# syzhang092218-source/dgppo

Hardware: AMD Instinct MI355X
Metric: env-steps/sec whole node, LidarSpread n=8 4096 envs, 1/2/4/8 GPUs (higher is better)
Workload: dtype f32

## Files before the change

dgppo_amd/_native.py:

```python
from __future__ import annotations

import ctypes as C
import os
from typing import Optional

import numpy as np
import torch

_HERE = os.path.dirname(os.path.abspath(__file__))
LIB_PATH = os.environ.get("DGPPO_HIP_LIB") or os.path.join(_HERE, "csrc", "libdgppo_hip.so")

ABI_VERSION = 3
OPT_STATE_FLOATS = 8 + 2 * 256

ENV_KINDS = {"LidarSpread": 0, "LidarTarget": 1, "LidarBicycleTarget": 2, "MPESpread": 3, "MPETarget": 4,
             "LidarLine": 5, "MPELine": 6, "MPEFormation": 7, "MPECorridor": 8, "MPEConnectSpread": 9,
             "VMASReverseTransport": 10}
VMAS_REVERSE_TRANSPORT = 10
GOALS_NODES, GOALS_LINE, GOALS_LINE_INTERIOR, GOALS_CIRCLE = range(4)
RECT_STRIDE = 16


class EnvCfg(C.Structure):
    _fields_ = [
        ("kind", C.c_int32), ("n_agents", C.c_int32), ("n_goals", C.c_int32), ("n_obs", C.c_int32),
        ("n_rays", C.c_int32), ("top_k", C.c_int32), ("state_dim", C.c_int32), ("node_dim", C.c_int32),
        ("area_size", C.c_float), ("dt", C.c_float), ("car_radius", C.c_float), ("comm_radius", C.c_float),
        ("obs_radius", C.c_float), ("dist2goal", C.c_float), ("two_car_radius", C.c_float),
        ("lidar_mask_radius", C.c_float), ("eye_offset", C.c_float), ("car_plus_obs", C.c_float),
        ("vel_limit", C.c_float), ("reset_min_dist", C.c_float),
        ("reward_goals", C.c_int32), ("n_cost", C.c_int32), ("obs_mask_radius", C.c_float), ("y_limit", C.c_float),
        ("connect_radius", C.c_float), ("reset_side_y", C.c_float), ("goal_shift_y", C.c_float), ("line_min_dist", C.c_float),
    ]

    @property
    def is_vmas(self):
        return self.kind == VMAS_REVERSE_TRANSPORT

    @property
    def is_lidar(self):
        return self.kind <= 2 or self.kind == 5

    @property
    def is_spread(self):
        return self.kind not in (1, 2, 4)

    @property
    def obs_nodes(self):
        if self.is_lidar:
            return self.n_agents * self.top_k if self.n_obs > 0 else 0
        return self.n_obs

    @property
    def obs_slots(self):
        if self.is_lidar:
            return self.top_k if self.n_obs > 0 else 0
        return self.n_obs

    @property
    def goal_slots(self):
        return self.n_goals if self.is_spread else 1

    @property
    def num_nodes(self):
        return self.n_agents + self.n_goals + self.obs_nodes + 1

    @property
    def num_edges(self):
        return self.n_agents * (self.n_agents + self.goal_slots + self.obs_slots)

    @property
    def fan_in(self):
        return self.n_agents + self.goal_slots + self.obs_slots

    @property
    def obst_stride(self):
        return RECT_STRIDE if self.is_lidar else self.state_dim


def make_env_cfg(kind: int, n_agents: int, n_obs: int, n_rays: int = 32, top_k: int = 8, area_size: float = None,
                 dt: float = 0.03, car_radius: float = 0.05, comm_radius: float = 0.5, obs_radius: float = None,
                 dist2goal: float = 0.01, connect_radius: float = 0.45, corridor_width: float = 0.2) -> EnvCfg:
    if kind == VMAS_REVERSE_TRANSPORT:
        return make_vmas_cfg(n_agents, dt)
    is_lidar = kind <= 2 or kind == 5
    corridor, connect = kind == 8, kind == 9
    if area_size is None:
        area_size = 1.0 if (corridor or connect) else 1.5
    if corridor:
        n_obs = 2
        obs_radius = (area_size - corridor_width) / 4
    elif connect:
        n_obs = 1
        obs_radius = 0.25 if obs_radius is None else obs_radius
    elif obs_radius is None:
        obs_radius = 0.05
    sd = 5 if kind == 2 else 4
    c = EnvCfg()
    c.kind, c.n_agents, c.n_obs = kind, n_agents, n_obs
    c.n_goals = 2 if kind in (5, 6) else (1 if kind == 7 else n_agents)
    c.n_rays, c.top_k = (n_rays, top_k) if is_lidar else (0, 0)
    c.state_dim, c.node_dim = sd, sd + 3
    c.area_size, c.dt, c.car_radius, c.comm_radius = area_size, dt, car_radius, comm_radius
    c.obs_radius, c.dist2goal = obs_radius, dist2goal
    c.two_car_radius = car_radius * 2
    c.lidar_mask_radius = comm_radius - 1e-1
    c.eye_offset = comm_radius + 1
    c.car_plus_obs = car_radius + obs_radius
    c.vel_limit = 0.5 if is_lidar else 1.0
    c.reset_min_dist = (2.2 * car_radius) if (is_lidar and kind != 5) else ((2.3 if connect else 2) * car_radius)
    c.reward_goals = {5: GOALS_LINE, 6: GOALS_LINE if n_agents > 3 else GOALS_LINE_INTERIOR, 7: GOALS_CIRCLE}.get(kind, GOALS_NODES)
    c.n_cost = 3 if connect else 2
    c.obs_mask_radius = comm_radius * 100 if (corridor or connect) else comm_radius
    c.y_limit = area_size * 2 if (corridor or connect) else area_size
    c.connect_radius = connect_radius
    c.reset_side_y = ((area_size - obs_radius * 2) / 2 - 1.5 * car_radius) if (corridor or connect) else area_size
    c.goal_shift_y = (area_size - (area_size - obs_radius * 2) / 2 + 1.5 * car_radius) if (corridor or connect) else 0.0
    if kind in (5, 6):
        c.line_min_dist = n_agents * 5 * car_radius if (kind == 6 and n_agents <= 3) else (n_agents - 2) * 6 * car_radius
    else:
        c.line_min_dist = 0.0
    return c


def make_vmas_cfg(n_agents: int, dt: float = 0.03) -> EnvCfg:
    c = EnvCfg()
    c.kind, c.n_agents, c.n_goals, c.n_obs, c.n_rays, c.top_k = VMAS_REVERSE_TRANSPORT, n_agents, 0, 0, 0, 0
    c.state_dim, c.node_dim = 4, 20
    c.area_size, c.dt, c.car_radius, c.comm_radius, c.obs_radius, c.dist2goal = 1.6, dt, 0.03, 0.4, 0.15, 0.01
    c.two_car_radius = 0.03 * 2
    c.vel_limit, c.reset_min_dist = 1.0, 0.03 * 2
    c.reward_goals, c.n_cost = GOALS_NODES, 2
    c.obs_mask_radius, c.y_limit = 0.4, 1.6
    return c


class GraphOut(C.Structure):
    _fields_ = [(k, C.c_void_p) for k in
                ("nodes", "edges", "states", "receivers", "senders", "node_type", "n_node", "n_edge")]


_lib: Optional[C.CDLL] = None


def lib() -> C.CDLL:
    global _lib
    if _lib is not None:
        return _lib
    if not os.path.exists(LIB_PATH):
        raise RuntimeError(
            f"dgppo_amd: HIP library not built: {LIB_PATH} is missing. "
            "Run `python -c 'import __graft_entry__ as g; g.build()'` (or `make -C dgppo_amd/csrc`). "
            "There is no CPU fallback.")
    l = C.CDLL(LIB_PATH)
    l.dgppo_abi_version.restype = C.c_int32
    l.dgppo_last_error.restype = C.c_char_p
    v = l.dgppo_abi_version()
    if v != ABI_VERSION:
        raise RuntimeError(f"dgppo_amd: ABI mismatch: library {v}, python {ABI_VERSION}")
    _lib = l
    return l


def check(rc: int, what: str):
    if rc != 0:
        msg = lib().dgppo_last_error().decode("utf-8", "replace")
        if rc > 0:
            raise RuntimeError(f"{what}: hipError {rc}: {msg}")
        raise ValueError(f"{what}: {msg}")


def ptr(t: Optional[torch.Tensor], dtype=torch.float32, name: str = "tensor") -> C.c_void_p:
    if t is None:
        return C.c_void_p(0)
    if not t.is_cuda:
        raise RuntimeError(f"{name} must live on the GPU (the HIP path has no CPU fallback)")
    if t.dtype != dtype:
        raise TypeError(f"{name} must be {dtype}, got {t.dtype}")
    if not t.is_contiguous():
        raise ValueError(f"{name} must be contiguous")
    return C.c_void_p(t.data_ptr())


_raw_stream = getattr(torch._C, "_cuda_getCurrentRawStream", None)
_raw_device = getattr(torch._C, "_cuda_getDevice", None)


def stream_ptr() -> C.c_void_p:
    if _raw_stream is not None and _raw_device is not None:
        return C.c_void_p(_raw_stream(_raw_device()))
    return C.c_void_p(torch.cuda.current_stream().cuda_stream)


def expect_shape(t: torch.Tensor, shape, name: str):
    if tuple(t.shape) != tuple(shape):
        raise ValueError(f"{name}: expected shape {tuple(shape)}, got {tuple(t.shape)}")
```

dgppo_amd/csrc/nn_elem.hip:

```cpp
#include "common.h"

using f32x4 = __attribute__((ext_vector_type(4))) float;

__device__ inline float wave_sum(float v) {
#pragma unroll
  for (int o = 32; o >= 1; o >>= 1) v += __shfl_xor(v, o);
  return v;
}
template <int NV>
__device__ inline void block_atomic_sums(const float (&v)[NV], float* dst) {
  __shared__ float s_red[4][NV];
  const int lane = threadIdx.x & 63, wave = threadIdx.x >> 6;
#pragma unroll
  for (int k = 0; k < NV; ++k) {
    const float w = wave_sum(v[k]);
    if (lane == 0) s_red[wave][k] = w;
  }
  __syncthreads();
  if (threadIdx.x < NV) {
    float t = 0.0f;
    for (int w = 0; w < (int)(blockDim.x >> 6); ++w) t += s_red[w][threadIdx.x];
    atomicAdd(dst + threadIdx.x, t);
  }
}

__device__ inline float row16_sum(float v) {
  v += __int_as_float(__builtin_amdgcn_update_dpp(0, __float_as_int(v), 0xB1, 0xf, 0xf, false));
  v += __int_as_float(__builtin_amdgcn_update_dpp(0, __float_as_int(v), 0x4E, 0xf, 0xf, false));
  v += __int_as_float(__builtin_amdgcn_update_dpp(0, __float_as_int(v), 0x141, 0xf, 0xf, false));
  v += __int_as_float(__builtin_amdgcn_update_dpp(0, __float_as_int(v), 0x140, 0xf, 0xf, false));
  return v;
}

__global__ void __launch_bounds__(256) ln_relu_fwd_kernel(const float* __restrict__ x, const float* __restrict__ gamma,
                                                          const float* __restrict__ beta, float* __restrict__ y,
                                                          float* __restrict__ stats, int M) {
  const int lane = threadIdx.x & 63, li = lane & 15, lq = lane >> 4;
  const int wave = (blockIdx.x * blockDim.x + threadIdx.x) >> 6;
  const int nw = (gridDim.x * blockDim.x) >> 6;
  const float4 g = reinterpret_cast<const float4*>(gamma)[li], b = reinterpret_cast<const float4*>(beta)[li];
  for (int row0 = wave * 4; row0 < M; row0 += nw * 4) {
    const int row = row0 + lq;
    const bool ok = row < M;
    const float4 v = reinterpret_cast<const float4*>(x)[(size_t)(ok ? row : M - 1) * 16 + li];
    const float mean = row16_sum((v.x + v.y) + (v.z + v.w)) * (1.0f / 64.0f);
    const float mean2 = row16_sum((v.x * v.x + v.y * v.y) + (v.z * v.z + v.w * v.w)) * (1.0f / 64.0f);
    const float var = fmaxf(mean2 - mean * mean, 0.0f);
    const float rstd = rsqrtf(var + 1e-6f);
    float4 o;
    o.x = fmaxf((v.x - mean) * rstd * g.x + b.x, 0.0f);
    o.y = fmaxf((v.y - mean) * rstd * g.y + b.y, 0.0f);
    o.z = fmaxf((v.z - mean) * rstd * g.z + b.z, 0.0f);
    o.w = fmaxf((v.w - mean) * rstd * g.w + b.w, 0.0f);
    if (ok) {
      reinterpret_cast<float4*>(y)[(size_t)row * 16 + li] = o;
      if (stats != nullptr && li == 0) reinterpret_cast<float2*>(stats)[row] = make_float2(mean, rstd);
    }
  }
}

__global__ void __launch_bounds__(256) ln_relu_bwd_kernel(const float* __restrict__ x, const float* __restrict__ y,
                                                          const float* __restrict__ stats, const float* __restrict__ gamma,
                                                          const float* __restrict__ dy, float* __restrict__ dx,
                                                          float* __restrict__ dgamma, float* __restrict__ dbeta, int M) {
  const int lane = threadIdx.x & 63, li = lane & 15, lq = lane >> 4;
  const int wave = (blockIdx.x * blockDim.x + threadIdx.x) >> 6;
  const int nw = (gridDim.x * blockDim.x) >> 6;
  const float4 g = reinterpret_cast<const float4*>(gamma)[li];
  float dg[4] = {0.f, 0.f, 0.f, 0.f}, db[4] = {0.f, 0.f, 0.f, 0.f};
  for (int row0 = wave * 4; row0 < M; row0 += nw * 4) {
    const int row = row0 + lq;
    const bool ok = row < M;
    const size_t o = (size_t)(ok ? row : M - 1) * 16 + li;
    const float4 xv = reinterpret_cast<const float4*>(x)[o], yv = reinterpret_cast<const float4*>(y)[o];
    const float4 dv = reinterpret_cast<const float4*>(dy)[o];
    const float2 st = reinterpret_cast<const float2*>(stats)[ok ? row : M - 1];
    const float mean = st.x, rstd = st.y;
    const float xh[4] = {(xv.x - mean) * rstd, (xv.y - mean) * rstd, (xv.z - mean) * rstd, (xv.w - mean) * rstd};
    const float dl[4] = {(ok && yv.x > 0.0f) ? dv.x : 0.0f, (ok && yv.y > 0.0f) ? dv.y : 0.0f,
                         (ok && yv.z > 0.0f) ? dv.z : 0.0f, (ok && yv.w > 0.0f) ? dv.w : 0.0f};
    const float gg[4] = {g.x, g.y, g.z, g.w};
    float dxh[4], s1 = 0.0f, s2 = 0.0f;
#pragma unroll
    for (int q = 0; q < 4; ++q) {
      dg[q] += dl[q] * xh[q];
      db[q] += dl[q];
      dxh[q] = dl[q] * gg[q];
      s1 += dxh[q];
      s2 += dxh[q] * xh[q];
    }
    const float m1 = row16_sum(s1) * (1.0f / 64.0f), m2 = row16_sum(s2) * (1.0f / 64.0f);
    if (ok)
      reinterpret_cast<float4*>(dx)[o] = make_float4(rstd * (dxh[0] - m1 - xh[0] * m2), rstd * (dxh[1] - m1 - xh[1] * m2),
                                                     rstd * (dxh[2] - m1 - xh[2] * m2), rstd * (dxh[3] - m1 - xh[3] * m2));
  }
  __shared__ float red[2][16][64];
  const int slot = (threadIdx.x >> 6) * 4 + lq;
#pragma unroll
  for (int q = 0; q < 4; ++q) { red[0][slot][li * 4 + q] = dg[q]; red[1][slot][li * 4 + q] = db[q]; }
  __syncthreads();
  if (threadIdx.x < 128) {
    const int which = threadIdx.x >> 6;
    float v = 0.0f;
#pragma unroll
    for (int sidx = 0; sidx < 16; ++sidx) v += red[which][sidx][lane];
    atomicAdd((which ? dbeta : dgamma) + lane, v);
  }
}

extern "C" int32_t dgppo_ln_relu_fwd(const float* x, const float* gamma, const float* beta, float* y, float* stats,
                                     int32_t M, void* stream) {
  DGPPO_REQUIRE(M >= 0, "ln_relu_fwd: M < 0");
  if (M == 0) return 0;
  DGPPO_REQUIRE(x && gamma && beta && y, "ln_relu_fwd: NULL operand");
  const int grid = min(cdiv(M, 16), 2048);
  hipLaunchKernelGGL(ln_relu_fwd_kernel, dim3(grid), dim3(256), 0, (hipStream_t)stream, x, gamma, beta, y, stats, M);
  DGPPO_LAUNCH_CHECK();
  return 0;
}

extern "C" int32_t dgppo_ln_relu_bwd(const float* x, const float* y, const float* stats, const float* gamma,
                                     const float* dy, float* dx, float* dgamma, float* dbeta, int32_t M, void* stream) {
  DGPPO_REQUIRE(M >= 0, "ln_relu_bwd: M < 0");
  if (M == 0) return 0;
  DGPPO_REQUIRE(x && y && stats && gamma && dy && dx && dgamma && dbeta, "ln_relu_bwd: NULL operand");
  const int grid = min(cdiv(M, 16), 256);
  hipLaunchKernelGGL(ln_relu_bwd_kernel, dim3(grid), dim3(256), 0, (hipStream_t)stream, x, y, stats, gamma, dy, dx, dgamma,
                     dbeta, M);
  DGPPO_LAUNCH_CHECK();
  return 0;
}

#define GRU_H 64
#define GRU_WL 194
#define GRU_HL 66

struct GruArgs {
  const float* gi;
  const float* Wh;
  const float* bhn;
  const float* h0;
  float* hs;
  float* hprev;
  float* gates;
  const float* dhs;
  float* dgi;
  float* dgh;
  float* dhn;
  int n_seq, T, n_inner;
};

__device__ inline size_t gru_row(const GruArgs& a, int s, int tau) {
  const int grp = s / a.n_inner, i = s - grp * a.n_inner;
  return ((size_t)grp * a.T + tau) * a.n_inner + i;
}
__device__ inline float sigmoidf_(float x) { return 1.0f / (1.0f + expf(-x)); }
__device__ inline float gate_sigmoid(float x) { return __builtin_amdgcn_rcpf(1.0f + __expf(-x)); }
__device__ inline float gate_tanh(float x) { return fmaf(2.0f, __builtin_amdgcn_rcpf(1.0f + __expf(-2.0f * x)), -1.0f); }


#define GRU_LDS_BARRIER() asm volatile("s_waitcnt lgkmcnt(0)\n\ts_barrier" ::: "memory")

template <int RTW>
__global__ void __launch_bounds__(256) gru_fwd_kernel(GruArgs a) {
  extern __shared__ float sm[];
  constexpr int RB = 16 * RTW;
  constexpr int HSLOT = RB * 16 / 256 > 0 ? RB * 16 / 256 : 1;
  const int tid = threadIdx.x, lane = tid & 63, w = tid >> 6, li = lane & 15, lq = lane >> 4;
  const int c = w * 16 + li;
  float breg[16][3];
#pragma unroll
  for (int kk = 0; kk < 16; ++kk)
#pragma unroll
    for (int t = 0; t < 3; ++t) breg[kk][t] = a.Wh[(size_t)(kk * 4 + lq) * 192 + t * 64 + c];
  const float bn = a.bhn[c];
  const int n_tiles = (a.n_seq + RB - 1) / RB;
  const float4 z4 = make_float4(0.f, 0.f, 0.f, 0.f);
  float hpf[HSLOT][4];
  auto fetch_h0 = [&](int tile) {
#pragma unroll
    for (int u = 0; u < HSLOT; ++u) {
      int idx = u * 256 + tid;
      idx = idx < RB * 16 ? idx : RB * 16 - 1;
      const int r = idx >> 4, q = idx & 15;
      int s = tile * RB + r;
      s = s < a.n_seq ? s : a.n_seq - 1;
      float4 v = z4;
      if (a.h0 != nullptr) v = reinterpret_cast<const float4*>(a.h0 + (size_t)s * GRU_H)[q];
      hpf[u][0] = v.x; hpf[u][1] = v.y; hpf[u][2] = v.z; hpf[u][3] = v.w;
    }
  };
  auto commit_h0 = [&](float* dst) {
#pragma unroll
    for (int u = 0; u < HSLOT; ++u) {
      const int idx = u * 256 + tid, r = idx >> 4, q = idx & 15;
      if (idx < RB * 16) { float* d = dst + r * GRU_HL + 4 * q; d[0] = hpf[u][0]; d[1] = hpf[u][1]; d[2] = hpf[u][2]; d[3] = hpf[u][3]; }
    }
  };
  int tile = blockIdx.x;
  if (tile < n_tiles) { fetch_h0(tile); commit_h0(sm); }
  __syncthreads();
  int cur = 0;
  for (; tile < n_tiles; tile += gridDim.x) {
    const int s0 = tile * RB;
    const int nxt = tile + gridDim.x;
    if (nxt < n_tiles) fetch_h0(nxt);
    int row0[RTW][4];
    bool ok[RTW][4];
#pragma unroll
    for (int rt = 0; rt < RTW; ++rt)
#pragma unroll
      for (int r = 0; r < 4; ++r) {
        int s = s0 + rt * 16 + lq * 4 + r;
        ok[rt][r] = s < a.n_seq;
        s = ok[rt][r] ? s : a.n_seq - 1;
        int rw = s;
        if (a.T != 1 && a.n_inner != 1) { const int grp = s / a.n_inner; rw = grp * a.T * a.n_inner + (s - grp * a.n_inner); }
        else if (a.T != 1) rw = s * a.T;
        row0[rt][r] = rw;
      }
    float gn[RTW][4][3];
    auto fetch_gi = [&](int tau) {
#pragma unroll
      for (int rt = 0; rt < RTW; ++rt)
#pragma unroll
        for (int r = 0; r < 4; ++r) {
          const float* gp = a.gi + (size_t)(row0[rt][r] + tau * a.n_inner) * 192 + c;
          gn[rt][r][0] = gp[0]; gn[rt][r][1] = gp[64]; gn[rt][r][2] = gp[128];
        }
    };
    fetch_gi(0);
    for (int tau = 0; tau < a.T; ++tau) {
      const float* hs_cur = sm + cur * (RB * GRU_HL);
      float* hs_nxt = sm + (cur ^ 1) * (RB * GRU_HL);
      float g[RTW][4][3];
#pragma unroll
      for (int rt = 0; rt < RTW; ++rt)
#pragma unroll
        for (int r = 0; r < 4; ++r) { g[rt][r][0] = gn[rt][r][0]; g[rt][r][1] = gn[rt][r][1]; g[rt][r][2] = gn[rt][r][2]; }
      if (tau + 1 < a.T) fetch_gi(tau + 1);
      __builtin_amdgcn_sched_barrier(0);
      float areg[RTW][16];
#pragma unroll
      for (int rt = 0; rt < RTW; ++rt)
#pragma unroll
        for (int kk = 0; kk < 16; ++kk) areg[rt][kk] = hs_cur[(rt * 16 + li) * GRU_HL + kk * 4 + lq];
      __builtin_amdgcn_sched_barrier(0);
      f32x4 acc[RTW][3];
#pragma unroll
      for (int rt = 0; rt < RTW; ++rt)
#pragma unroll
        for (int t = 0; t < 3; ++t) acc[rt][t] = f32x4{0.f, 0.f, 0.f, 0.f};
#pragma unroll
      for (int kk = 0; kk < 16; ++kk)
#pragma unroll
        for (int rt = 0; rt < RTW; ++rt)
#pragma unroll
          for (int t = 0; t < 3; ++t) acc[rt][t] = __builtin_amdgcn_mfma_f32_16x16x4f32(areg[rt][kk], breg[kk][t], acc[rt][t], 0, 0, 0);
#pragma unroll
      for (int rt = 0; rt < RTW; ++rt)
#pragma unroll
        for (int r = 0; r < 4; ++r) {
          const int rl = rt * 16 + lq * 4 + r;
          const float hp = hs_cur[rl * GRU_HL + c];
          const float rg = gate_sigmoid(g[rt][r][0] + acc[rt][0][r]);
          const float zg = gate_sigmoid(g[rt][r][1] + acc[rt][1][r]);
          const float hn = acc[rt][2][r] + bn;
          const float ng = gate_tanh(g[rt][r][2] + rg * hn);
          const float hnew = (1.0f - zg) * ng + zg * hp;
          hs_nxt[rl * GRU_HL + c] = hnew;
          if (ok[rt][r]) {
            const size_t row = (size_t)(row0[rt][r] + tau * a.n_inner);
            a.hs[row * GRU_H + c] = hnew;
            if (a.hprev != nullptr) a.hprev[row * GRU_H + c] = hp;
            if (a.gates != nullptr) {
              float* gs = a.gates + row * 256;
              gs[c] = rg; gs[64 + c] = zg; gs[128 + c] = ng; gs[192 + c] = hn;
            }
          }
        }
      GRU_LDS_BARRIER();
      cur ^= 1;
    }
    if (nxt < n_tiles) {
      commit_h0(sm + cur * (RB * GRU_HL));
      GRU_LDS_BARRIER();
    }
  }
}

template <int RTW, bool DHN_ONLY>
__global__ void __launch_bounds__(256) gru_bwd_kernel(GruArgs a) {
  extern __shared__ float sm[];
  constexpr int RB = 16 * RTW;
  const int tid = threadIdx.x, lane = tid & 63, w = tid >> 6, li = lane & 15, lq = lane >> 4;
  const int c = w * 16 + li;
  float breg[48];
#pragma unroll
  for (int kk = 0; kk < 48; ++kk) breg[kk] = a.Wh[(size_t)c * 192 + kk * 4 + lq];
  const int n_tiles = (a.n_seq + RB - 1) / RB;
  int cur = 0;
  for (int tile = blockIdx.x; tile < n_tiles; tile += gridDim.x) {
    const int s0 = tile * RB;
    int row0[RTW][4];
    bool ok[RTW][4];
#pragma unroll
    for (int rt = 0; rt < RTW; ++rt)
#pragma unroll
      for (int r = 0; r < 4; ++r) {
        int s = s0 + rt * 16 + lq * 4 + r;
        ok[rt][r] = s < a.n_seq;
        s = ok[rt][r] ? s : a.n_seq - 1;
        int rw = s;
        if (a.T != 1 && a.n_inner != 1) { const int grp = s / a.n_inner; rw = grp * a.T * a.n_inner + (s - grp * a.n_inner); }
        else if (a.T != 1) rw = s * a.T;
        row0[rt][r] = rw;
      }
    float rg[RTW][4], zg[RTW][4], ng[RTW][4], hn[RTW][4], hp[RTW][4], du[RTW][4], dh[RTW][4];
    auto fetch = [&](int tau) {
#pragma unroll
      for (int rt = 0; rt < RTW; ++rt)
#pragma unroll
        for (int r = 0; r < 4; ++r) {
          const size_t row = (size_t)(row0[rt][r] + tau * a.n_inner);
          const float* gs = a.gates + row * 256 + c;
          rg[rt][r] = gs[0]; zg[rt][r] = gs[64]; ng[rt][r] = gs[128]; hn[rt][r] = gs[192];
          hp[rt][r] = a.hprev[row * GRU_H + c];
          du[rt][r] = a.dhs[row * GRU_H + c];
        }
    };
#pragma unroll
    for (int rt = 0; rt < RTW; ++rt)
#pragma unroll
      for (int r = 0; r < 4; ++r) dh[rt][r] = 0.0f;
    fetch(a.T - 1);
    for (int tau = a.T - 1; tau >= 0; --tau) {
      float* s_g = sm + cur * (RB * GRU_WL);
#pragma unroll
      for (int rt = 0; rt < RTW; ++rt)
#pragma unroll
        for (int r = 0; r < 4; ++r) {
          const int rl = rt * 16 + lq * 4 + r;
          const float d = ok[rt][r] ? dh[rt][r] + du[rt][r] : 0.0f;
          const float dz = d * (hp[rt][r] - ng[rt][r]);
          const float dn = d * (1.0f - zg[rt][r]);
          const float dan = dn * (1.0f - ng[rt][r] * ng[rt][r]);
          const float dhn = dan * rg[rt][r];
          const float dar = dan * hn[rt][r] * rg[rt][r] * (1.0f - rg[rt][r]);
          const float daz = dz * zg[rt][r] * (1.0f - zg[rt][r]);
          dh[rt][r] = d * zg[rt][r];
          s_g[rl * GRU_WL + c] = dar;
          s_g[rl * GRU_WL + 64 + c] = daz;
          s_g[rl * GRU_WL + 128 + c] = dhn;
          if (ok[rt][r]) {
            const size_t row = (size_t)(row0[rt][r] + tau * a.n_inner);
            float* o = a.dgi + row * 192 + c;
            o[0] = dar; o[64] = daz; o[128] = dan;
            if (DHN_ONLY) {
              a.dhn[row * GRU_H + c] = dhn;
            } else {
              float* p = a.dgh + row * 192 + c;
              p[0] = dar; p[64] = daz; p[128] = dhn;
            }
          }
        }
      GRU_LDS_BARRIER();
      if (tau > 0) fetch(tau - 1);
      __builtin_amdgcn_sched_barrier(0);
      f32x4 acc[RTW];
#pragma unroll
      for (int rt = 0; rt < RTW; ++rt) acc[rt] = f32x4{0.f, 0.f, 0.f, 0.f};
#pragma unroll
      for (int k0 = 0; k0 < 48; k0 += 16) {
        float areg[RTW][16];
#pragma unroll
        for (int rt = 0; rt < RTW; ++rt)
#pragma unroll
          for (int u = 0; u < 16; ++u) areg[rt][u] = s_g[(rt * 16 + li) * GRU_WL + (k0 + u) * 4 + lq];
        __builtin_amdgcn_sched_barrier(0);
#pragma unroll
        for (int u = 0; u < 16; ++u)
#pragma unroll
          for (int rt = 0; rt < RTW; ++rt) acc[rt] = __builtin_amdgcn_mfma_f32_16x16x4f32(areg[rt][u], breg[k0 + u], acc[rt], 0, 0, 0);
      }
#pragma unroll
      for (int rt = 0; rt < RTW; ++rt)
#pragma unroll
        for (int r = 0; r < 4; ++r) dh[rt][r] += acc[rt][r];
      cur ^= 1;
    }
    GRU_LDS_BARRIER();
  }
}

static int gru_resident(const void* fn, size_t smem) {
  int per_cu = 0, dev = 0, cus = 256;
  if (hipOccupancyMaxActiveBlocksPerMultiprocessor(&per_cu, fn, 256, smem) != hipSuccess || per_cu < 1) per_cu = 1;
  if (hipGetDevice(&dev) != hipSuccess ||
      hipDeviceGetAttribute(&cus, hipDeviceAttributeMultiprocessorCount, dev) != hipSuccess || cus < 1) cus = 256;
  return per_cu * cus;
}

static int32_t gru_check(const GruArgs& a) {
  DGPPO_REQUIRE(a.n_seq >= 0 && a.T >= 1 && a.n_inner >= 1, "gru: bad sizes n_seq=%d T=%d n_inner=%d", a.n_seq, a.T, a.n_inner);
  DGPPO_REQUIRE(a.n_seq % a.n_inner == 0, "gru: n_seq must be a multiple of n_inner");
  return 0;
}

extern "C" int32_t dgppo_gru_fwd(const float* gi, const float* Wh, const float* bhn, const float* h0, float* hs,
                                 float* hprev, float* gates, int32_t n_seq, int32_t T, int32_t n_inner, void* stream) {
  GruArgs a{};
  a.gi = gi; a.Wh = Wh; a.bhn = bhn; a.h0 = h0; a.hs = hs; a.hprev = hprev; a.gates = gates;
  a.n_seq = n_seq; a.T = T; a.n_inner = n_inner;
  int32_t rc = gru_check(a);
  if (rc) return rc;
  if (n_seq == 0) return 0;
  DGPPO_REQUIRE(gi && Wh && bhn && hs, "gru_fwd: NULL operand");
  if (cdiv(n_seq, 32) >= 512) {
    const size_t smem = sizeof(float) * 2 * 32 * GRU_HL;
    static thread_local int cap = 0;
    if (cap == 0) cap = gru_resident(reinterpret_cast<const void*>(&gru_fwd_kernel<2>), smem);
    const int tiles = cdiv(n_seq, 32);
    hipLaunchKernelGGL(gru_fwd_kernel<2>, dim3(tiles < cap ? tiles : cap), dim3(256), smem, (hipStream_t)stream, a);
  } else {
    const size_t smem = sizeof(float) * 2 * 16 * GRU_HL;
    static thread_local int cap = 0;
    if (cap == 0) cap = gru_resident(reinterpret_cast<const void*>(&gru_fwd_kernel<1>), smem);
    const int tiles = cdiv(n_seq, 16);
    hipLaunchKernelGGL(gru_fwd_kernel<1>, dim3(tiles < cap ? tiles : cap), dim3(256), smem, (hipStream_t)stream, a);
  }
  DGPPO_LAUNCH_CHECK();
  return 0;
}

template <bool DHN_ONLY>
static int32_t gru_bwd_launch(GruArgs a, hipStream_t stream) {
  int32_t rc = gru_check(a);
  if (rc) return rc;
  if (a.n_seq == 0) return 0;
  DGPPO_REQUIRE(a.dhs && a.Wh && a.hprev && a.gates && a.dgi && (DHN_ONLY ? a.dhn : a.dgh), "gru_bwd: NULL operand");
  if (cdiv(a.n_seq, 32) >= 512) {
    const size_t smem = sizeof(float) * 2 * 32 * GRU_WL;
    static thread_local int cap = 0;
    if (cap == 0) cap = gru_resident(reinterpret_cast<const void*>(&gru_bwd_kernel<2, DHN_ONLY>), smem);
    const int tiles = cdiv(a.n_seq, 32);
    hipLaunchKernelGGL((gru_bwd_kernel<2, DHN_ONLY>), dim3(tiles < cap ? tiles : cap), dim3(256), smem, stream, a);
  } else {
    const size_t smem = sizeof(float) * 2 * 16 * GRU_WL;
    static thread_local int cap = 0;
    if (cap == 0) cap = gru_resident(reinterpret_cast<const void*>(&gru_bwd_kernel<1, DHN_ONLY>), smem);
    const int tiles = cdiv(a.n_seq, 16);
    hipLaunchKernelGGL((gru_bwd_kernel<1, DHN_ONLY>), dim3(tiles < cap ? tiles : cap), dim3(256), smem, stream, a);
  }
  DGPPO_LAUNCH_CHECK();
  return 0;
}

extern "C" int32_t dgppo_gru_bwd(const float* dhs, const float* Wh, const float* hprev, const float* gates, float* dgi,
                                 float* dgh, int32_t n_seq, int32_t T, int32_t n_inner, void* stream) {
  GruArgs a{};
  a.dhs = dhs; a.Wh = Wh; a.hprev = (float*)hprev; a.gates = (float*)gates; a.dgi = dgi; a.dgh = dgh;
  a.n_seq = n_seq; a.T = T; a.n_inner = n_inner;
  return gru_bwd_launch<false>(a, (hipStream_t)stream);
}

extern "C" int32_t dgppo_gru_bwd_dhn(const float* dhs, const float* Wh, const float* hprev, const float* gates, float* dgi,
                                     float* dhn, int32_t n_seq, int32_t T, int32_t n_inner, void* stream) {
  GruArgs a{};
  a.dhs = dhs; a.Wh = Wh; a.hprev = (float*)hprev; a.gates = (float*)gates; a.dgi = dgi; a.dhn = dhn;
  a.n_seq = n_seq; a.T = T; a.n_inner = n_inner;
  return gru_bwd_launch<true>(a, (hipStream_t)stream);
}

#define STD_INIT_INV (-0.43275212956718856f)
#define STD_MIN 1e-5f
#define THRESH 0.999f
#define INV_THRESH 3.8002011672502f
#define LOG_EPS (-6.907755278982137f)
#define HALF_LOG_2PI 0.9189385332046727f
#define LOG2_F 0.6931471805599453f

__device__ inline float softplusf_(float x) { return (x > 20.0f) ? x : log1pf(expf(x)); }
#define NDTR_SERIES_BELOW (-10.0f)
__device__ inline float ndtr_tail_series(float z2) { return 1.0f - 1.0f / z2 + 3.0f / (z2 * z2) - 15.0f / (z2 * z2 * z2); }
__device__ inline float log_ndtrf_(float z) {
  if (z > NDTR_SERIES_BELOW) return logf(0.5f * erfcf(-z * 0.70710678118654752f));
  const float z2 = z * z;
  return -0.5f * z2 - logf(-z) - HALF_LOG_2PI + logf(ndtr_tail_series(z2));
}
__device__ inline float dlog_ndtrf_(float z) {
  if (z > NDTR_SERIES_BELOW) return 0.3989422804014327f * expf(-0.5f * z * z) / (0.5f * erfcf(-z * 0.70710678118654752f));
  return -z / ndtr_tail_series(z * z);
}
__device__ inline float tanh_fldj(float x) { return 2.0f * (LOG2_F - x - softplusf_(-2.0f * x)); }

struct HeadArgs {
  const float* ms;
  const float* eps;
  const float* action_in;
  float* action;
  float* log_pi;
  float* entropy;
  int rows, n_agents, mode;
  const float* log_pi_old;
  const float* adv;
  float* dms;
  float* stats;
  float clip_eps, coef_ent, inv_count;
};

__device__ inline float tn_log_prob_dim(float act, float mu, float sd) {
  const float ac = fminf(fmaxf(act, -THRESH), THRESH);
  if (ac <= -THRESH) return log_ndtrf_((-INV_THRESH - mu) / sd) - LOG_EPS;
  if (ac >= THRESH) return log_ndtrf_(-(INV_THRESH - mu) / sd) - LOG_EPS;
  const float x = atanhf(ac);
  const float z = (x - mu) / sd;
  return -0.5f * z * z - logf(sd) - HALF_LOG_2PI - tanh_fldj(x);
}

__global__ void __launch_bounds__(256) policy_head_kernel(HeadArgs a) {
  float acc[4] = {0.0f, 0.0f, 0.0f, 0.0f};
  const int rows_pad = (a.rows + 255) & ~255;
  for (int row_raw = blockIdx.x * blockDim.x + threadIdx.x; row_raw < rows_pad; row_raw += gridDim.x * blockDim.x) {
  const bool valid = row_raw < a.rows;
  const int row = valid ? row_raw : a.rows - 1;
  const float4 m = reinterpret_cast<const float4*>(a.ms)[row];
  const float mu[2] = {m.x, m.y};
  const float st[2] = {m.z, m.w};
  float sd[2];
  for (int d = 0; d < 2; ++d) sd[d] = softplusf_(st[d] + STD_INIT_INV) + STD_MIN;
  if (a.mode == 1) {
    if (valid) {
      a.action[row * 2] = tanhf(mu[0]);
      a.action[row * 2 + 1] = tanhf(mu[1]);
    }
    continue;
  }
  float act[2];
  if (a.mode == 0) {
    for (int d = 0; d < 2; ++d) act[d] = tanhf(mu[d] + sd[d] * a.eps[row * 2 + d]);
    if (valid) {
      a.action[row * 2] = act[0];
      a.action[row * 2 + 1] = act[1];
      a.log_pi[row] = tn_log_prob_dim(act[0], mu[0], sd[0]) + tn_log_prob_dim(act[1], mu[1], sd[1]);
    }
    continue;
  }
  act[0] = a.action_in[row * 2];
  act[1] = a.action_in[row * 2 + 1];
  const int ag = row % a.n_agents;
  float lp = 0.0f, ent = 0.0f;
  float dlp_dmu[2], dlp_dsd[2], dent_dmu[2], dent_dsd[2];
  for (int d = 0; d < 2; ++d) {
    const float ac = fminf(fmaxf(act[d], -THRESH), THRESH);
    if (ac <= -THRESH) {
      const float u = (-INV_THRESH - mu[d]) / sd[d];
      lp += log_ndtrf_(u) - LOG_EPS;
      const float r = dlog_ndtrf_(u);
      dlp_dmu[d] = -r / sd[d];
      dlp_dsd[d] = -r * u / sd[d];
    } else if (ac >= THRESH) {
      const float u = (mu[d] - INV_THRESH) / sd[d];
      lp += log_ndtrf_(u) - LOG_EPS;
      const float r = dlog_ndtrf_(u);
      dlp_dmu[d] = r / sd[d];
      dlp_dsd[d] = -r * u / sd[d];
    } else {
      const float x = atanhf(ac);
      const float z = (x - mu[d]) / sd[d];
      lp += -0.5f * z * z - logf(sd[d]) - HALF_LOG_2PI - tanh_fldj(x);
      dlp_dmu[d] = z / sd[d];
      dlp_dsd[d] = (z * z - 1.0f) / sd[d];
    }
    const float eh = a.eps[ag * 2 + d];
    const float y = mu[d] + sd[d] * eh;
    ent += 0.5f + HALF_LOG_2PI + logf(sd[d]) + tanh_fldj(y);
    const float th = tanhf(y);
    dent_dmu[d] = -2.0f * th;
    dent_dsd[d] = 1.0f / sd[d] - 2.0f * th * eh;
  }
  if (valid) {
    a.log_pi[row] = lp;
    a.entropy[row] = ent;
  }
  if (a.dms == nullptr) continue;
  const float A = a.adv[row];
  const float rho = expf(lp - a.log_pi_old[row]);
  const float l1 = -rho * A;
  const float l2 = -fminf(fmaxf(rho, 1.0f - a.clip_eps), 1.0f + a.clip_eps) * A;
  const float lsel = fmaxf(l1, l2);
  const float dl_dlp = ((l2 > l1) ? 0.0f : -rho * A) * a.inv_count;
  const float dl_dent = -a.coef_ent * a.inv_count;
  if (valid) {
    float4 o;
    const float dsd0 = dl_dlp * dlp_dsd[0] + dl_dent * dent_dsd[0];
    const float dsd1 = dl_dlp * dlp_dsd[1] + dl_dent * dent_dsd[1];
    o.x = dl_dlp * dlp_dmu[0] + dl_dent * dent_dmu[0];
    o.y = dl_dlp * dlp_dmu[1] + dl_dent * dent_dmu[1];
    o.z = dsd0 * sigmoidf_(st[0] + STD_INIT_INV);
    o.w = dsd1 * sigmoidf_(st[1] + STD_INIT_INV);
    reinterpret_cast<float4*>(a.dms)[row] = o;
  }
  if (valid) {
    acc[0] += lsel; acc[1] += ent; acc[2] += (l2 > l1) ? 1.0f : 0.0f; acc[3] += fabsf(rho - 1.0f);
  }
  }
  if (a.mode == 2 && a.dms != nullptr) block_atomic_sums<4>(acc, a.stats);
}

extern "C" int32_t dgppo_policy_head(const float* ms, const float* eps, const float* action_in, float* action,
                                     float* log_pi, float* entropy, int32_t rows, int32_t n_agents, int32_t mode,
                                     const float* log_pi_old, const float* adv, float* dms, float* stats, float clip_eps,
                                     float coef_ent, void* stream) {
  DGPPO_REQUIRE(rows >= 0 && n_agents >= 1 && mode >= 0 && mode <= 2, "policy_head: bad arguments");
  if (rows == 0) return 0;
  DGPPO_REQUIRE(ms, "policy_head: ms is NULL");
  DGPPO_REQUIRE(((uintptr_t)ms & 15) == 0, "policy_head: ms must be 16-byte aligned");
  if (mode == 0) DGPPO_REQUIRE(eps && action && log_pi, "policy_head(sample): NULL operand");
  if (mode == 1) DGPPO_REQUIRE(action, "policy_head(mode): NULL operand");
  if (mode == 2) {
    DGPPO_REQUIRE(eps && action_in && log_pi && entropy, "policy_head(eval): NULL operand");
    if (dms) DGPPO_REQUIRE(log_pi_old && adv && stats && ((uintptr_t)dms & 15) == 0, "policy_head(eval+loss): NULL operand");
  }
  HeadArgs a{};
  a.ms = ms; a.eps = eps; a.action_in = action_in; a.action = action; a.log_pi = log_pi; a.entropy = entropy;
  a.rows = rows; a.n_agents = n_agents; a.mode = mode; a.log_pi_old = log_pi_old; a.adv = adv; a.dms = dms; a.stats = stats;
  a.clip_eps = clip_eps; a.coef_ent = coef_ent; a.inv_count = 1.0f / (float)rows;
  const int blocks = cdiv(rows, 256);
  hipLaunchKernelGGL(policy_head_kernel, dim3(blocks < 512 ? blocks : 512), dim3(256), 0, (hipStream_t)stream, a);
  DGPPO_LAUNCH_CHECK();
  return 0;
}

__global__ void __launch_bounds__(256) value_loss_kernel(const float* __restrict__ v, const float* __restrict__ target,
                                                         float* __restrict__ dv, float* __restrict__ stats, int count,
                                                         float count_f) {
  float l[1] = {0.0f};
  for (int i = blockIdx.x * blockDim.x + threadIdx.x; i < count; i += gridDim.x * blockDim.x) {
    const float d = v[i] - target[i];
    dv[i] = d / count_f;
    l[0] += 0.5f * d * d;
  }
  block_atomic_sums<1>(l, stats);
}

extern "C" int32_t dgppo_value_loss(const float* v, const float* target, float* dv, float* stats, int32_t count,
                                    void* stream) {
  DGPPO_REQUIRE(count >= 0, "value_loss: count < 0");
  if (count == 0) return 0;
  DGPPO_REQUIRE(v && target && dv && stats, "value_loss: NULL operand");
  const int blocks = cdiv(count, 256);
  hipLaunchKernelGGL(value_loss_kernel, dim3(blocks < 256 ? blocks : 256), dim3(256), 0, (hipStream_t)stream, v, target, dv,
                     stats, count, (float)count);
  DGPPO_LAUNCH_CHECK();
  return 0;
}

__global__ void mean_agents_kernel(const float* __restrict__ x, float* __restrict__ y, int G, int n, int D, int backward,
                                   const float* __restrict__ relu_mask) {
  const int idx = blockIdx.x * blockDim.x + threadIdx.x;
  if (backward) {
    if (idx >= G * n * D) return;
    const int d = idx % D, g = idx / (n * D);
    const float v = (backward == 2) ? y[idx] + x[(size_t)g * D + d] : x[(size_t)g * D + d] / (float)n;
    y[idx] = (relu_mask == nullptr || relu_mask[idx] > 0.0f) ? v : 0.0f;
  } else {
    if (idx >= G * D) return;
    const int d = idx % D, g = idx / D;
    float acc = 0.0f;
    for (int i = 0; i < n; ++i) acc += x[((size_t)g * n + i) * D + d];
    y[idx] = acc / (float)n;
  }
}

extern "C" int32_t dgppo_mean_agents(const float* x, float* y, int32_t G, int32_t n, int32_t D, int32_t backward,
                                     const float* relu_mask, void* stream) {
  DGPPO_REQUIRE(G >= 0 && n >= 1 && D >= 1, "mean_agents: bad sizes");
  DGPPO_REQUIRE(backward >= 0 && backward <= 2, "mean_agents: backward must be 0, 1 or 2");
  if (G == 0) return 0;
  DGPPO_REQUIRE(x && y, "mean_agents: NULL operand");
  const long total = backward ? (long)G * n * D : (long)G * D;
  hipLaunchKernelGGL(mean_agents_kernel, dim3(cdiv(total, 256)), dim3(256), 0, (hipStream_t)stream, x, y, G, n, D, backward,
                     backward ? relu_mask : nullptr);
  DGPPO_LAUNCH_CHECK();
  return 0;
}

__global__ void relu_bwd_kernel(float* __restrict__ dy, const float* __restrict__ y, long count) {
  const long i = (long)blockIdx.x * blockDim.x + threadIdx.x;
  if (i < count && !(y[i] > 0.0f)) dy[i] = 0.0f;
}

extern "C" int32_t dgppo_relu_bwd(float* dy, const float* y, int64_t count, void* stream) {
  DGPPO_REQUIRE(count >= 0, "relu_bwd: count < 0");
  if (count == 0) return 0;
  DGPPO_REQUIRE(dy && y, "relu_bwd: NULL operand");
  hipLaunchKernelGGL(relu_bwd_kernel, dim3(cdiv(count, 256)), dim3(256), 0, (hipStream_t)stream, dy, y, (long)count);
  DGPPO_LAUNCH_CHECK();
  return 0;
}
```

dgppo_amd/csrc/nn_fused.hip:

```cpp
#include "common.h"

using f32x4 = __attribute__((ext_vector_type(4))) float;
#define FZ_H 64
#define FZ_HL 66
#define FZ_RB 32
#define FZ_LDS_BARRIER() asm volatile("s_waitcnt lgkmcnt(0)\n\ts_barrier" ::: "memory")

__device__ inline float row16_sum(float v) {
  v += __int_as_float(__builtin_amdgcn_update_dpp(0, __float_as_int(v), 0xB1, 0xf, 0xf, false));
  v += __int_as_float(__builtin_amdgcn_update_dpp(0, __float_as_int(v), 0x4E, 0xf, 0xf, false));
  v += __int_as_float(__builtin_amdgcn_update_dpp(0, __float_as_int(v), 0x141, 0xf, 0xf, false));
  v += __int_as_float(__builtin_amdgcn_update_dpp(0, __float_as_int(v), 0x140, 0xf, 0xf, false));
  return v;
}

struct MlpGiArgs {
  const float* X; int ldx; int M;
  const float *W1, *b1, *g1, *be1, *W2, *b2, *g2, *be2, *Wi, *bi;
  float *p1, *y1, *st1, *p2, *y2, *st2;
  float* gi;
};

__global__ void __launch_bounds__(256) __attribute__((amdgpu_waves_per_eu(2, 8))) mlp_gi_fwd_kernel(MlpGiArgs a) {
  extern __shared__ float sm[];
  float* s_x = sm;
  float* s_y1 = s_x + FZ_RB * FZ_HL;
  float* s_y2 = s_y1 + FZ_RB * FZ_HL;
  float* s_red = s_y2 + FZ_RB * FZ_HL;
  const int tid = threadIdx.x, lane = tid & 63, w = tid >> 6, li = lane & 15, lq = lane >> 4;
  const int c = w * 16 + li;
  float w1[16], w2[16], wi[16][3];
#pragma unroll
  for (int kk = 0; kk < 16; ++kk) {
    const int k = kk * 4 + lq;
    w1[kk] = a.W1[k * FZ_H + c];
    w2[kk] = a.W2[k * FZ_H + c];
#pragma unroll
    for (int t = 0; t < 3; ++t) wi[kk][t] = a.Wi[k * 192 + t * 64 + c];
  }
  const float b1 = a.b1[c], g1 = a.g1[c], e1 = a.be1[c], b2 = a.b2[c], g2 = a.g2[c], e2 = a.be2[c];
  const float bi0 = a.bi[c], bi1 = a.bi[64 + c], bi2 = a.bi[128 + c];
  const int n_tiles = (a.M + FZ_RB - 1) / FZ_RB;
  const bool vec = ((a.ldx & 3) == 0) && ((reinterpret_cast<uintptr_t>(a.X) & 15) == 0);
  float xpf[2][4];
  auto fetch = [&](int tile) {
#pragma unroll
    for (int u = 0; u < 2; ++u) {
      const int idx = u * 256 + tid, r = idx >> 4, q = idx & 15;
      int row = tile * FZ_RB + r;
      row = row < a.M ? row : a.M - 1;
      const float* p = a.X + (size_t)row * a.ldx + 4 * q;
      if (vec) { const float4 v = *reinterpret_cast<const float4*>(p); xpf[u][0] = v.x; xpf[u][1] = v.y; xpf[u][2] = v.z; xpf[u][3] = v.w; }
      else { xpf[u][0] = p[0]; xpf[u][1] = p[1]; xpf[u][2] = p[2]; xpf[u][3] = p[3]; }
    }
  };
  auto commit = [&]() {
#pragma unroll
    for (int u = 0; u < 2; ++u) {
      const int idx = u * 256 + tid, r = idx >> 4, q = idx & 15;
      float* d = s_x + r * FZ_HL + 4 * q;
      d[0] = xpf[u][0]; d[1] = xpf[u][1]; d[2] = xpf[u][2]; d[3] = xpf[u][3];
    }
  };
  auto ln_relu = [&](float (&v)[2][4], float g, float e, float* s_out, float* y_out, float* st_out, int row0) {
#pragma unroll
    for (int rt = 0; rt < 2; ++rt)
#pragma unroll
      for (int r = 0; r < 4; ++r) {
        const float s = row16_sum(v[rt][r]), q = row16_sum(v[rt][r] * v[rt][r]);
        if (li == 0) { float* d = s_red + (rt * 16 + lq * 4 + r) * 8 + 2 * w; d[0] = s; d[1] = q; }
      }
    FZ_LDS_BARRIER();
    float4 pa[2][4], pb[2][4];
#pragma unroll
    for (int rt = 0; rt < 2; ++rt)
#pragma unroll
      for (int r = 0; r < 4; ++r) {
        const int rl = rt * 16 + lq * 4 + r;
        pa[rt][r] = *reinterpret_cast<const float4*>(s_red + rl * 8);
        pb[rt][r] = *reinterpret_cast<const float4*>(s_red + rl * 8 + 4);
      }
    __builtin_amdgcn_sched_barrier(0);
#pragma unroll
    for (int rt = 0; rt < 2; ++rt)
#pragma unroll
      for (int r = 0; r < 4; ++r) {
        const int rl = rt * 16 + lq * 4 + r;
        const float4 p0 = pa[rt][r], p1 = pb[rt][r];
        const float mean = ((p0.x + p0.z) + (p1.x + p1.z)) * (1.0f / 64.0f);
        const float mean2 = ((p0.y + p0.w) + (p1.y + p1.w)) * (1.0f / 64.0f);
        const float var = fmaxf(mean2 - mean * mean, 0.0f);
        const float rstd = rsqrtf(var + 1e-6f);
        const float y = fmaxf((v[rt][r] - mean) * rstd * g + e, 0.0f);
        s_out[rl * FZ_HL + c] = y;
        const int row = row0 + rl;
        if (y_out != nullptr && row < a.M) {
          y_out[(size_t)row * FZ_H + c] = y;
          if (c == 0) { st_out[(size_t)row * 2] = mean; st_out[(size_t)row * 2 + 1] = rstd; }
        }
      }
    FZ_LDS_BARRIER();
  };
  int tile = blockIdx.x;
  if (tile < n_tiles) { fetch(tile); commit(); }
  __syncthreads();
  for (; tile < n_tiles; tile += gridDim.x) {
    const int row0 = tile * FZ_RB;
    const int nxt = tile + gridDim.x;
    const bool more = nxt < n_tiles;
    if (more) fetch(nxt);
    __builtin_amdgcn_sched_barrier(0);
    float areg[2][16];
    f32x4 acc[2];
    float v[2][4];
#pragma unroll
    for (int rt = 0; rt < 2; ++rt)
#pragma unroll
      for (int kk = 0; kk < 16; ++kk) areg[rt][kk] = s_x[(rt * 16 + li) * FZ_HL + kk * 4 + lq];
    __builtin_amdgcn_sched_barrier(0);
    acc[0] = acc[1] = f32x4{0.f, 0.f, 0.f, 0.f};
#pragma unroll
    for (int kk = 0; kk < 16; ++kk)
#pragma unroll
      for (int rt = 0; rt < 2; ++rt) acc[rt] = __builtin_amdgcn_mfma_f32_16x16x4f32(areg[rt][kk], w1[kk], acc[rt], 0, 0, 0);
#pragma unroll
    for (int rt = 0; rt < 2; ++rt)
#pragma unroll
      for (int r = 0; r < 4; ++r) {
        v[rt][r] = acc[rt][r] + b1;
        const int row = row0 + rt * 16 + lq * 4 + r;
        if (a.p1 != nullptr && row < a.M) a.p1[(size_t)row * FZ_H + c] = v[rt][r];
      }
    ln_relu(v, g1, e1, s_y1, a.y1, a.st1, row0);
    if (more) commit();
#pragma unroll
    for (int rt = 0; rt < 2; ++rt)
#pragma unroll
      for (int kk = 0; kk < 16; ++kk) areg[rt][kk] = s_y1[(rt * 16 + li) * FZ_HL + kk * 4 + lq];
    __builtin_amdgcn_sched_barrier(0);
    acc[0] = acc[1] = f32x4{0.f, 0.f, 0.f, 0.f};
#pragma unroll
    for (int kk = 0; kk < 16; ++kk)
#pragma unroll
      for (int rt = 0; rt < 2; ++rt) acc[rt] = __builtin_amdgcn_mfma_f32_16x16x4f32(areg[rt][kk], w2[kk], acc[rt], 0, 0, 0);
#pragma unroll
    for (int rt = 0; rt < 2; ++rt)
#pragma unroll
      for (int r = 0; r < 4; ++r) {
        v[rt][r] = acc[rt][r] + b2;
        const int row = row0 + rt * 16 + lq * 4 + r;
        if (a.p2 != nullptr && row < a.M) a.p2[(size_t)row * FZ_H + c] = v[rt][r];
      }
    ln_relu(v, g2, e2, s_y2, a.y2, a.st2, row0);
#pragma unroll
    for (int rt = 0; rt < 2; ++rt)
#pragma unroll
      for (int kk = 0; kk < 16; ++kk) areg[rt][kk] = s_y2[(rt * 16 + li) * FZ_HL + kk * 4 + lq];
    __builtin_amdgcn_sched_barrier(0);
    f32x4 ag[2][3];
#pragma unroll
    for (int rt = 0; rt < 2; ++rt)
#pragma unroll
      for (int t = 0; t < 3; ++t) ag[rt][t] = f32x4{0.f, 0.f, 0.f, 0.f};
#pragma unroll
    for (int kk = 0; kk < 16; ++kk)
#pragma unroll
      for (int rt = 0; rt < 2; ++rt)
#pragma unroll
        for (int t = 0; t < 3; ++t) ag[rt][t] = __builtin_amdgcn_mfma_f32_16x16x4f32(areg[rt][kk], wi[kk][t], ag[rt][t], 0, 0, 0);
#pragma unroll
    for (int rt = 0; rt < 2; ++rt)
#pragma unroll
      for (int r = 0; r < 4; ++r) {
        const int row = row0 + rt * 16 + lq * 4 + r;
        if (row < a.M) {
          float* o = a.gi + (size_t)row * 192 + c;
          o[0] = ag[rt][0][r] + bi0; o[64] = ag[rt][1][r] + bi1; o[128] = ag[rt][2][r] + bi2;
        }
      }
  }
}

#define RW_WL 65
#define RW_WIL 193
#define RW_YL 68
#define RW_WAVES 16
__global__ void __launch_bounds__(64 * RW_WAVES) mlp_gi_fwd_rw_kernel(MlpGiArgs a) {
  extern __shared__ float sm[];
  float* sW1 = sm;
  float* sW2 = sW1 + 64 * RW_WL;
  float* sWi = sW2 + 64 * RW_WL;
  float* sP = sWi + 64 * RW_WIL;
  const int tid = threadIdx.x, lane = tid & 63, w = tid >> 6, li = lane & 15, lq = lane >> 4;
  float* sY = sP + 576 + w * (16 * RW_YL);
  {
    static_assert(RW_WAVES == 16, "the staging below assumes 1024 threads");
    const float4 v1 = reinterpret_cast<const float4*>(a.W1)[tid], v2 = reinterpret_cast<const float4*>(a.W2)[tid];
    float4 vi[3];
#pragma unroll
    for (int j = 0; j < 3; ++j) vi[j] = reinterpret_cast<const float4*>(a.Wi)[j * 1024 + tid];
    {
      const int k = tid >> 4, c = (tid & 15) * 4;
      float* d1 = sW1 + k * RW_WL + c; float* d2 = sW2 + k * RW_WL + c;
      d1[0] = v1.x; d1[1] = v1.y; d1[2] = v1.z; d1[3] = v1.w;
      d2[0] = v2.x; d2[1] = v2.y; d2[2] = v2.z; d2[3] = v2.w;
    }
#pragma unroll
    for (int j = 0; j < 3; ++j) {
      const int q = j * 1024 + tid, k = q / 48, c = (q - k * 48) * 4;
      float* d = sWi + k * RW_WIL + c;
      d[0] = vi[j].x; d[1] = vi[j].y; d[2] = vi[j].z; d[3] = vi[j].w;
    }
  }
  if (tid < 64) {
    sP[tid] = a.b1[tid]; sP[64 + tid] = a.g1[tid]; sP[128 + tid] = a.be1[tid];
    sP[192 + tid] = a.b2[tid]; sP[256 + tid] = a.g2[tid]; sP[320 + tid] = a.be2[tid];
  }
  if (tid < 192) sP[384 + tid] = a.bi[tid];
  __syncthreads();
  const int n_tiles = (a.M + 15) >> 4;
  const bool save = a.p1 != nullptr;
  float A[16];
  auto fetch = [&](int tile) {
    int row = tile * 16 + li;
    row = row < a.M ? row : a.M - 1;
    const float4* p = reinterpret_cast<const float4*>(a.X + (size_t)row * a.ldx + lq * 16);
#pragma unroll
    for (int j = 0; j < 4; ++j) { const float4 v = p[j]; A[4 * j] = v.x; A[4 * j + 1] = v.y; A[4 * j + 2] = v.z; A[4 * j + 3] = v.w; }
  };
  auto layer = [&](const float* sW, const float* par, float* p_out, float* y_out, float* st_out, int row0) {
    f32x4 acc[4];
#pragma unroll
    for (int ct = 0; ct < 4; ++ct) acc[ct] = f32x4{0.f, 0.f, 0.f, 0.f};
    float bw[2][4][4];
    auto ldw = [&](int buf, int g) {
#pragma unroll
      for (int kk = 0; kk < 4; ++kk) {
        const float* wr = sW + (lq * 16 + g * 4 + kk) * RW_WL + li;
#pragma unroll
        for (int ct = 0; ct < 4; ++ct) bw[buf][kk][ct] = wr[ct * 16];
      }
    };
    ldw(0, 0);
#pragma unroll
    for (int g = 0; g < 4; ++g) {
      if (g + 1 < 4) ldw((g + 1) & 1, g + 1);
      __builtin_amdgcn_sched_barrier(0);
#pragma unroll
      for (int kk = 0; kk < 4; ++kk)
#pragma unroll
        for (int ct = 0; ct < 4; ++ct) acc[ct] = __builtin_amdgcn_mfma_f32_16x16x4f32(A[g * 4 + kk], bw[g & 1][kk][ct], acc[ct], 0, 0, 0);
      __builtin_amdgcn_sched_barrier(0);
    }
    float s[4] = {0.f, 0.f, 0.f, 0.f}, q[4] = {0.f, 0.f, 0.f, 0.f};
#pragma unroll
    for (int ct = 0; ct < 4; ++ct) {
      const float b = par[ct * 16 + li];
#pragma unroll
      for (int r = 0; r < 4; ++r) {
        acc[ct][r] += b;
        s[r] += acc[ct][r];
        q[r] = fmaf(acc[ct][r], acc[ct][r], q[r]);
        const int row = row0 + lq * 4 + r;
        if (save && row < a.M) p_out[(size_t)row * FZ_H + ct * 16 + li] = acc[ct][r];
      }
    }
    float mean[4], rstd[4];
#pragma unroll
    for (int r = 0; r < 4; ++r) {
      mean[r] = row16_sum(s[r]) * (1.0f / 64.0f);
      const float m2 = row16_sum(q[r]) * (1.0f / 64.0f);
      rstd[r] = rsqrtf(fmaxf(m2 - mean[r] * mean[r], 0.0f) + 1e-6f);
      const int row = row0 + lq * 4 + r;
      if (save && li == 0 && row < a.M) { st_out[(size_t)row * 2] = mean[r]; st_out[(size_t)row * 2 + 1] = rstd[r]; }
    }
#pragma unroll
    for (int ct = 0; ct < 4; ++ct) {
      const float g = par[64 + ct * 16 + li], e = par[128 + ct * 16 + li];
#pragma unroll
      for (int r = 0; r < 4; ++r) {
        const float y = fmaxf((acc[ct][r] - mean[r]) * rstd[r] * g + e, 0.0f);
        sY[(lq * 4 + r) * RW_YL + ct * 16 + li] = y;
        const int row = row0 + lq * 4 + r;
        if (save && row < a.M) y_out[(size_t)row * FZ_H + ct * 16 + li] = y;
      }
    }
#pragma unroll
    for (int j = 0; j < 4; ++j) {
      const float4 v = *reinterpret_cast<const float4*>(sY + li * RW_YL + lq * 16 + 4 * j);
      A[4 * j] = v.x; A[4 * j + 1] = v.y; A[4 * j + 2] = v.z; A[4 * j + 3] = v.w;
    }
  };
  for (int tile = w * gridDim.x + blockIdx.x; tile < n_tiles; tile += gridDim.x * RW_WAVES) {
    const int row0 = tile * 16;
    fetch(tile);
    layer(sW1, sP, a.p1, a.y1, a.st1, row0);
    layer(sW2, sP + 192, a.p2, a.y2, a.st2, row0);
#pragma unroll
    for (int half = 0; half < 2; ++half) {
      f32x4 ag[6];
#pragma unroll
      for (int t = 0; t < 6; ++t) ag[t] = f32x4{0.f, 0.f, 0.f, 0.f};
      float bg[2][2][6];
      auto ldg = [&](int buf, int g) {
#pragma unroll
        for (int kk = 0; kk < 2; ++kk) {
          const float* wr = sWi + (lq * 16 + g * 2 + kk) * RW_WIL + half * 96 + li;
#pragma unroll
          for (int t = 0; t < 6; ++t) bg[buf][kk][t] = wr[t * 16];
        }
      };
      ldg(0, 0);
#pragma unroll
      for (int g = 0; g < 8; ++g) {
        if (g + 1 < 8) ldg((g + 1) & 1, g + 1);
        __builtin_amdgcn_sched_barrier(0);
#pragma unroll
        for (int kk = 0; kk < 2; ++kk)
#pragma unroll
          for (int t = 0; t < 6; ++t) ag[t] = __builtin_amdgcn_mfma_f32_16x16x4f32(A[g * 2 + kk], bg[g & 1][kk][t], ag[t], 0, 0, 0);
        __builtin_amdgcn_sched_barrier(0);
      }
#pragma unroll
      for (int t = 0; t < 6; ++t) {
        const int col = half * 96 + t * 16 + li;
        const float b = sP[384 + col];
#pragma unroll
        for (int r = 0; r < 4; ++r) {
          const int row = row0 + lq * 4 + r;
          if (row < a.M) a.gi[(size_t)row * 192 + col] = ag[t][r] + b;
        }
      }
    }
  }
}

struct MlpGiBwdArgs {
  const float* dgi; int M;
  const float *Wi, *W2, *W1, *g2, *g1;
  const float *p2, *y2, *st2, *p1, *y1, *st1;
  const float* mask; int ldm;
  float *dpre2, *dpre1, *dx; int lddx;
  float *dg2, *db2, *dg1, *db1;
};
#define FZ_GL 194
#ifndef FZ_BWD_RT
#define FZ_BWD_RT 1
#endif
#ifndef FZ_BWD_WPE
#define FZ_BWD_WPE 2
#endif

__global__ void __launch_bounds__(256) __attribute__((amdgpu_waves_per_eu(FZ_BWD_WPE, 8))) mlp_gi_bwd_kernel(MlpGiBwdArgs a) {
  constexpr int BRT = FZ_BWD_RT, BRB = 16 * BRT;
  extern __shared__ float sm[];
  float* s_g = sm;
  float* s_d2 = s_g + BRB * FZ_GL;
  float* s_d1 = s_d2 + BRB * FZ_HL;
  float* s_red = s_d1 + BRB * FZ_HL;
  const int tid = threadIdx.x, lane = tid & 63, w = tid >> 6, li = lane & 15, lq = lane >> 4;
  const int c = w * 16 + li;
  float wi[48], w2[16], w1[16];
#pragma unroll
  for (int kk = 0; kk < 48; ++kk) wi[kk] = a.Wi[c * 192 + kk * 4 + lq];
#pragma unroll
  for (int kk = 0; kk < 16; ++kk) { w2[kk] = a.W2[c * FZ_H + kk * 4 + lq]; w1[kk] = a.W1[c * FZ_H + kk * 4 + lq]; }
  const float g2 = a.g2[c], g1 = a.g1[c];
  float dgs[2] = {0.f, 0.f}, dbs[2] = {0.f, 0.f};
  const int n_tiles = (a.M + BRB - 1) / BRB;
  constexpr int GSL = BRB * 48 / 256;
  float4 gpf[GSL];
  auto fetch = [&](int tile) {
#pragma unroll
    for (int u = 0; u < GSL; ++u) {
      const int idx = u * 256 + tid, r = idx / 48, q = idx - r * 48;
      int row = tile * BRB + r;
      row = row < a.M ? row : a.M - 1;
      gpf[u] = *reinterpret_cast<const float4*>(a.dgi + (size_t)row * 192 + 4 * q);
    }
  };
  auto commit = [&]() {
#pragma unroll
    for (int u = 0; u < GSL; ++u) {
      const int idx = u * 256 + tid, r = idx / 48, q = idx - r * 48;
      float2* d = reinterpret_cast<float2*>(s_g + r * FZ_GL + 4 * q);
      d[0] = make_float2(gpf[u].x, gpf[u].y); d[1] = make_float2(gpf[u].z, gpf[u].w);
    }
  };
  auto ln_relu_bwd = [&](float (&v)[BRT][4], const float (&pv)[BRT][4], const float (&yv)[BRT][4], const float2 (&st)[BRT][4], float g,
                         float& dg_acc, float& db_acc, float* s_out, float* d_out, int row0) {
    float xh[BRT][4], dxh[BRT][4];
#pragma unroll
    for (int rt = 0; rt < BRT; ++rt)
#pragma unroll
      for (int r = 0; r < 4; ++r) {
        const int rl = rt * 16 + lq * 4 + r;
        int row = row0 + rl;
        const bool ok = row < a.M;
        row = ok ? row : a.M - 1;
        const float2 ms = st[rt][r];
        xh[rt][r] = (pv[rt][r] - ms.x) * ms.y;
        const float dl = (ok && yv[rt][r] > 0.0f) ? v[rt][r] : 0.0f;
        dg_acc += dl * xh[rt][r];
        db_acc += dl;
        dxh[rt][r] = dl * g;
        const float s1 = row16_sum(dxh[rt][r]), s2 = row16_sum(dxh[rt][r] * xh[rt][r]);
        if (li == 0) { float* d = s_red + rl * 8 + 2 * w; d[0] = s1; d[1] = s2; }
        v[rt][r] = ms.y;
      }
    FZ_LDS_BARRIER();
#pragma unroll
    for (int rt = 0; rt < BRT; ++rt)
#pragma unroll
      for (int r = 0; r < 4; ++r) {
        const int rl = rt * 16 + lq * 4 + r;
        const float4 p0 = *reinterpret_cast<const float4*>(s_red + rl * 8), p1 = *reinterpret_cast<const float4*>(s_red + rl * 8 + 4);
        const float m1 = ((p0.x + p0.z) + (p1.x + p1.z)) * (1.0f / 64.0f);
        const float m2 = ((p0.y + p0.w) + (p1.y + p1.w)) * (1.0f / 64.0f);
        const float dp = v[rt][r] * (dxh[rt][r] - m1 - xh[rt][r] * m2);
        v[rt][r] = dp;
        s_out[rl * FZ_HL + c] = dp;
        const int row = row0 + rl;
        if (row < a.M) d_out[(size_t)row * FZ_H + c] = dp;
      }
    FZ_LDS_BARRIER();
  };
  auto load_st = [&](const float* src, int row0, float2 (&o)[BRT][4]) {
#pragma unroll
    for (int rt = 0; rt < BRT; ++rt)
#pragma unroll
      for (int r = 0; r < 4; ++r) {
        int row = row0 + rt * 16 + lq * 4 + r;
        row = row < a.M ? row : a.M - 1;
        o[rt][r] = reinterpret_cast<const float2*>(src)[row];
      }
  };
  auto load8 = [&](const float* src, int ld, int row0, float (&o)[BRT][4]) {
#pragma unroll
    for (int rt = 0; rt < BRT; ++rt)
#pragma unroll
      for (int r = 0; r < 4; ++r) {
        int row = row0 + rt * 16 + lq * 4 + r;
        row = row < a.M ? row : a.M - 1;
        o[rt][r] = src[(size_t)row * ld + c];
      }
  };
  int tile = blockIdx.x;
  if (tile < n_tiles) { fetch(tile); commit(); }
  __syncthreads();
  for (; tile < n_tiles; tile += gridDim.x) {
    const int row0 = tile * BRB;
    const int nxt = tile + gridDim.x;
    const bool more = nxt < n_tiles;
    if (more) fetch(nxt);
    float pv2[BRT][4], yv2[BRT][4], pv1[BRT][4], yv1[BRT][4], mk[BRT][4];
    float2 sv2[BRT][4], sv1[BRT][4];
    load8(a.p2, FZ_H, row0, pv2); load8(a.y2, FZ_H, row0, yv2); load_st(a.st2, row0, sv2);
    load8(a.p1, FZ_H, row0, pv1); load8(a.y1, FZ_H, row0, yv1); load_st(a.st1, row0, sv1);
    if (a.mask != nullptr) load8(a.mask, a.ldm, row0, mk);
    __builtin_amdgcn_sched_barrier(0);
    f32x4 acc[BRT];
    float v[BRT][4];
    for (int rt = 0; rt < BRT; ++rt) acc[rt] = f32x4{0.f, 0.f, 0.f, 0.f};
#pragma unroll
    for (int c0 = 0; c0 < 48; c0 += 8) {
      float areg[BRT][8];
#pragma unroll
      for (int rt = 0; rt < BRT; ++rt)
#pragma unroll
        for (int kk = 0; kk < 8; ++kk) areg[rt][kk] = s_g[(rt * 16 + li) * FZ_GL + (c0 + kk) * 4 + lq];
      __builtin_amdgcn_sched_barrier(0);
#pragma unroll
      for (int kk = 0; kk < 8; ++kk)
#pragma unroll
        for (int rt = 0; rt < BRT; ++rt) acc[rt] = __builtin_amdgcn_mfma_f32_16x16x4f32(areg[rt][kk], wi[c0 + kk], acc[rt], 0, 0, 0);
      __builtin_amdgcn_sched_barrier(0);
    }
#pragma unroll
    for (int rt = 0; rt < BRT; ++rt)
#pragma unroll
      for (int r = 0; r < 4; ++r) v[rt][r] = acc[rt][r];
    ln_relu_bwd(v, pv2, yv2, sv2, g2, dgs[0], dbs[0], s_d2, a.dpre2, row0);
    if (more) commit();
    {
      float areg[BRT][16];
#pragma unroll
      for (int rt = 0; rt < BRT; ++rt)
#pragma unroll
        for (int kk = 0; kk < 16; ++kk) areg[rt][kk] = s_d2[(rt * 16 + li) * FZ_HL + kk * 4 + lq];
      __builtin_amdgcn_sched_barrier(0);
      for (int rt = 0; rt < BRT; ++rt) acc[rt] = f32x4{0.f, 0.f, 0.f, 0.f};
#pragma unroll
      for (int kk = 0; kk < 16; ++kk)
#pragma unroll
        for (int rt = 0; rt < BRT; ++rt) acc[rt] = __builtin_amdgcn_mfma_f32_16x16x4f32(areg[rt][kk], w2[kk], acc[rt], 0, 0, 0);
    }
#pragma unroll
    for (int rt = 0; rt < BRT; ++rt)
#pragma unroll
      for (int r = 0; r < 4; ++r) v[rt][r] = acc[rt][r];
    ln_relu_bwd(v, pv1, yv1, sv1, g1, dgs[1], dbs[1], s_d1, a.dpre1, row0);
    {
      float areg[BRT][16];
#pragma unroll
      for (int rt = 0; rt < BRT; ++rt)
#pragma unroll
        for (int kk = 0; kk < 16; ++kk) areg[rt][kk] = s_d1[(rt * 16 + li) * FZ_HL + kk * 4 + lq];
      __builtin_amdgcn_sched_barrier(0);
      for (int rt = 0; rt < BRT; ++rt) acc[rt] = f32x4{0.f, 0.f, 0.f, 0.f};
#pragma unroll
      for (int kk = 0; kk < 16; ++kk)
#pragma unroll
        for (int rt = 0; rt < BRT; ++rt) acc[rt] = __builtin_amdgcn_mfma_f32_16x16x4f32(areg[rt][kk], w1[kk], acc[rt], 0, 0, 0);
    }
#pragma unroll
    for (int rt = 0; rt < BRT; ++rt)
#pragma unroll
      for (int r = 0; r < 4; ++r) {
        const int row = row0 + rt * 16 + lq * 4 + r;
        float o = acc[rt][r];
        if (a.mask != nullptr) o = (mk[rt][r] > 0.0f) ? o : 0.0f;
        if (row < a.M) a.dx[(size_t)row * a.lddx + c] = o;
      }
  }
  __syncthreads();
  float* red = sm;
  red[(0 * 4 + lq) * 64 + c] = dgs[0]; red[(1 * 4 + lq) * 64 + c] = dbs[0];
  red[(2 * 4 + lq) * 64 + c] = dgs[1]; red[(3 * 4 + lq) * 64 + c] = dbs[1];
  __syncthreads();
  {
    const int which = tid >> 6, col = tid & 63;
    const float tot = (red[(which * 4 + 0) * 64 + col] + red[(which * 4 + 1) * 64 + col]) +
                      (red[(which * 4 + 2) * 64 + col] + red[(which * 4 + 3) * 64 + col]);
    float* dst = which == 0 ? a.dg2 : (which == 1 ? a.db2 : (which == 2 ? a.dg1 : a.db1));
    atomicAdd(dst + col, tot);
  }
}

extern "C" int32_t dgppo_mlp_gi_bwd(const float* dgi, const float* Wi, const float* W2, const float* W1, const float* g2,
                                    const float* g1, const float* p2, const float* y2, const float* st2, const float* p1,
                                    const float* y1, const float* st1, const float* relu_mask, int32_t ldm, float* dpre2,
                                    float* dpre1, float* dx, int32_t lddx, float* dg2, float* db2, float* dg1, float* db1,
                                    int32_t M, void* stream) {
  DGPPO_REQUIRE(M >= 0 && lddx >= FZ_H && (relu_mask == nullptr || ldm >= FZ_H), "mlp_gi_bwd: bad shape M=%d lddx=%d ldm=%d", M, lddx, ldm);
  DGPPO_REQUIRE(dgi && Wi && W2 && W1 && g2 && g1 && p2 && y2 && st2 && p1 && y1 && st1 && dpre2 && dpre1 && dx && dg2 && db2 &&
                dg1 && db1, "mlp_gi_bwd: NULL operand");
  DGPPO_REQUIRE((reinterpret_cast<uintptr_t>(dgi) & 15) == 0, "mlp_gi_bwd: dgi must be 16-byte aligned");
  if (M == 0) return 0;
  MlpGiBwdArgs a{dgi, M, Wi, W2, W1, g2, g1, p2, y2, st2, p1, y1, st1, relu_mask, ldm, dpre2, dpre1, dx, lddx, dg2, db2, dg1, db1};
  constexpr int BRB = 16 * FZ_BWD_RT;
  const size_t smem_t = sizeof(float) * (BRB * FZ_GL + 2 * BRB * FZ_HL + BRB * 8), smem_r = sizeof(float) * 16 * 64;
  const size_t smem = smem_t > smem_r ? smem_t : smem_r;
  static thread_local int cap = 0;
  if (cap == 0) {
    int per_cu = 0, dev = 0, cus = 256;
    if (hipOccupancyMaxActiveBlocksPerMultiprocessor(&per_cu, reinterpret_cast<const void*>(&mlp_gi_bwd_kernel), 256, smem) !=
            hipSuccess || per_cu < 1) per_cu = 1;
    if (hipGetDevice(&dev) != hipSuccess ||
        hipDeviceGetAttribute(&cus, hipDeviceAttributeMultiprocessorCount, dev) != hipSuccess || cus < 1) cus = 256;
    cap = per_cu * cus;
  }
  const int tiles = (M + BRB - 1) / BRB;
  hipLaunchKernelGGL(mlp_gi_bwd_kernel, dim3(tiles < cap ? tiles : cap), dim3(256), smem, (hipStream_t)stream, a);
  DGPPO_LAUNCH_CHECK();
  return 0;
}

extern "C" int32_t dgppo_mlp_gi_fwd(const float* X, int32_t ldx, const float* W1, const float* b1, const float* g1,
                                    const float* be1, const float* W2, const float* b2, const float* g2, const float* be2,
                                    const float* Wi, const float* bi, float* p1, float* y1, float* st1, float* p2, float* y2,
                                    float* st2, float* gi, int32_t M, void* stream) {
  DGPPO_REQUIRE(M >= 0 && ldx >= FZ_H, "mlp_gi_fwd: bad shape M=%d ldx=%d", M, ldx);
  DGPPO_REQUIRE(X && W1 && b1 && g1 && be1 && W2 && b2 && g2 && be2 && Wi && bi && gi, "mlp_gi_fwd: NULL operand");
  const bool save = p1 || y1 || st1 || p2 || y2 || st2;
  DGPPO_REQUIRE(!save || (p1 && y1 && st1 && p2 && y2 && st2), "mlp_gi_fwd: the saved activations are all-or-none");
  if (M == 0) return 0;
  MlpGiArgs a{X, ldx, M, W1, b1, g1, be1, W2, b2, g2, be2, Wi, bi, p1, y1, st1, p2, y2, st2, gi};
  if ((ldx & 3) == 0 && ((reinterpret_cast<uintptr_t>(X) | reinterpret_cast<uintptr_t>(W1) | reinterpret_cast<uintptr_t>(W2) |
                          reinterpret_cast<uintptr_t>(Wi)) & 15) == 0) {
    static thread_local int cus = 0;
    if (cus == 0) {
      int dev = 0;
      if (hipGetDevice(&dev) != hipSuccess ||
          hipDeviceGetAttribute(&cus, hipDeviceAttributeMultiprocessorCount, dev) != hipSuccess || cus < 1) cus = 256;
    }
    const size_t smem_rw = sizeof(float) * (2 * 64 * RW_WL + 64 * RW_WIL + 576 + RW_WAVES * 16 * RW_YL);
    static thread_local bool attr = false;
    if (!attr) {
      const hipError_t e = hipFuncSetAttribute(reinterpret_cast<const void*>(&mlp_gi_fwd_rw_kernel),
                                               hipFuncAttributeMaxDynamicSharedMemorySize, (int)smem_rw);
      DGPPO_REQUIRE(e == hipSuccess, "mlp_gi_fwd: cannot reserve %zu bytes of LDS per workgroup: %s", smem_rw, hipGetErrorString(e));
      attr = true;
    }
    const int tiles16 = (M + 15) / 16;
    hipLaunchKernelGGL(mlp_gi_fwd_rw_kernel, dim3(tiles16 < cus ? tiles16 : cus), dim3(64 * RW_WAVES), smem_rw, (hipStream_t)stream, a);
    DGPPO_LAUNCH_CHECK();
    return 0;
  }
  const size_t smem = sizeof(float) * (3 * FZ_RB * FZ_HL + FZ_RB * 8);
  static thread_local int cap = 0;
  if (cap == 0) {
    int per_cu = 0, dev = 0, cus = 256;
    if (hipOccupancyMaxActiveBlocksPerMultiprocessor(&per_cu, reinterpret_cast<const void*>(&mlp_gi_fwd_kernel), 256, smem) !=
            hipSuccess || per_cu < 1) per_cu = 1;
    if (hipGetDevice(&dev) != hipSuccess ||
        hipDeviceGetAttribute(&cus, hipDeviceAttributeMultiprocessorCount, dev) != hipSuccess || cus < 1) cus = 256;
    cap = per_cu * cus;
  }
  const int tiles = (M + FZ_RB - 1) / FZ_RB;
  hipLaunchKernelGGL(mlp_gi_fwd_kernel, dim3(tiles < cap ? tiles : cap), dim3(256), smem, (hipStream_t)stream, a);
  DGPPO_LAUNCH_CHECK();
  return 0;
}

struct GruHeadArgs {
  const float *gi, *Wh, *bhn, *h0;
  const float *W1, *b1, *W2, *b2;
  float *hs, *hprev, *gates, *u, *out;
  int M, n_out;
};
__device__ inline float gate_sigmoid(float x) { return __builtin_amdgcn_rcpf(1.0f + __expf(-x)); }
__device__ inline float gate_tanh(float x) { return fmaf(2.0f, __builtin_amdgcn_rcpf(1.0f + __expf(-2.0f * x)), -1.0f); }


template <bool TWO>
__global__ void __launch_bounds__(256) __attribute__((amdgpu_waves_per_eu(2, 8))) gru1_head_fwd_kernel(GruHeadArgs a) {
  extern __shared__ float sm[];
  float* s_h = sm;
  float* s_n = s_h + FZ_RB * FZ_HL;
  float* s_u = s_n + FZ_RB * FZ_HL;
  const int tid = threadIdx.x, lane = tid & 63, w = tid >> 6, li = lane & 15, lq = lane >> 4;
  const int c = w * 16 + li;
  float wh[16][3], w1[16], w2[16];
#pragma unroll
  for (int kk = 0; kk < 16; ++kk) {
    const int k = kk * 4 + lq;
#pragma unroll
    for (int t = 0; t < 3; ++t) wh[kk][t] = a.Wh[k * 192 + t * 64 + c];
    if (TWO) {
      w1[kk] = a.W1[k * FZ_H + c];
      w2[kk] = (li < a.n_out) ? a.W2[k * a.n_out + li] : 0.0f;
    } else {
      w1[kk] = (li < a.n_out) ? a.W1[k * a.n_out + li] : 0.0f;
      w2[kk] = 0.0f;
    }
  }
  const float bn = a.bhn[c];
  const float b1 = TWO ? a.b1[c] : ((li < a.n_out) ? a.b1[li] : 0.0f);
  const float b2 = (TWO && li < a.n_out) ? a.b2[li] : 0.0f;
  const int n_tiles = (a.M + FZ_RB - 1) / FZ_RB;
  float hpf[2][4];
  auto fetch_h0 = [&](int tile) {
#pragma unroll
    for (int u = 0; u < 2; ++u) {
      const int idx = u * 256 + tid, r = idx >> 4, q = idx & 15;
      int row = tile * FZ_RB + r;
      row = row < a.M ? row : a.M - 1;
      float4 v = make_float4(0.f, 0.f, 0.f, 0.f);
      if (a.h0 != nullptr) v = reinterpret_cast<const float4*>(a.h0 + (size_t)row * FZ_H)[q];
      hpf[u][0] = v.x; hpf[u][1] = v.y; hpf[u][2] = v.z; hpf[u][3] = v.w;
    }
  };
  auto commit_h0 = [&]() {
#pragma unroll
    for (int u = 0; u < 2; ++u) {
      const int idx = u * 256 + tid, r = idx >> 4, q = idx & 15;
      float* d = s_h + r * FZ_HL + 4 * q;
      d[0] = hpf[u][0]; d[1] = hpf[u][1]; d[2] = hpf[u][2]; d[3] = hpf[u][3];
    }
  };
  int tile = blockIdx.x;
  if (tile < n_tiles) { fetch_h0(tile); commit_h0(); }
  __syncthreads();
  for (; tile < n_tiles; tile += gridDim.x) {
    const int row0 = tile * FZ_RB;
    const int nxt = tile + gridDim.x;
    const bool more = nxt < n_tiles;
    float g[2][4][3];
#pragma unroll
    for (int rt = 0; rt < 2; ++rt)
#pragma unroll
      for (int r = 0; r < 4; ++r) {
        int row = row0 + rt * 16 + lq * 4 + r;
        row = row < a.M ? row : a.M - 1;
        const float* gp = a.gi + (size_t)row * 192 + c;
        g[rt][r][0] = gp[0]; g[rt][r][1] = gp[64]; g[rt][r][2] = gp[128];
      }
    if (more) fetch_h0(nxt);
    __builtin_amdgcn_sched_barrier(0);
    float areg[2][16];
#pragma unroll
    for (int rt = 0; rt < 2; ++rt)
#pragma unroll
      for (int kk = 0; kk < 16; ++kk) areg[rt][kk] = s_h[(rt * 16 + li) * FZ_HL + kk * 4 + lq];
    __builtin_amdgcn_sched_barrier(0);
    f32x4 acc[2][3];
#pragma unroll
    for (int rt = 0; rt < 2; ++rt)
#pragma unroll
      for (int t = 0; t < 3; ++t) acc[rt][t] = f32x4{0.f, 0.f, 0.f, 0.f};
#pragma unroll
    for (int kk = 0; kk < 16; ++kk)
#pragma unroll
      for (int rt = 0; rt < 2; ++rt)
#pragma unroll
        for (int t = 0; t < 3; ++t) acc[rt][t] = __builtin_amdgcn_mfma_f32_16x16x4f32(areg[rt][kk], wh[kk][t], acc[rt][t], 0, 0, 0);
#pragma unroll
    for (int rt = 0; rt < 2; ++rt)
#pragma unroll
      for (int r = 0; r < 4; ++r) {
        const int rl = rt * 16 + lq * 4 + r, row = row0 + rl;
        const float hp = s_h[rl * FZ_HL + c];
        const float rg = gate_sigmoid(g[rt][r][0] + acc[rt][0][r]);
        const float zg = gate_sigmoid(g[rt][r][1] + acc[rt][1][r]);
        const float hn = acc[rt][2][r] + bn;
        const float ng = gate_tanh(g[rt][r][2] + rg * hn);
        const float hnew = (1.0f - zg) * ng + zg * hp;
        s_n[rl * FZ_HL + c] = hnew;
        if (row < a.M) {
          a.hs[(size_t)row * FZ_H + c] = hnew;
          if (a.hprev != nullptr) a.hprev[(size_t)row * FZ_H + c] = hp;
          if (a.gates != nullptr) {
            float* gs = a.gates + (size_t)row * 256;
            gs[c] = rg; gs[64 + c] = zg; gs[128 + c] = ng; gs[192 + c] = hn;
          }
        }
      }
    FZ_LDS_BARRIER();
    if (more) commit_h0();
#pragma unroll
    for (int rt = 0; rt < 2; ++rt)
#pragma unroll
      for (int kk = 0; kk < 16; ++kk) areg[rt][kk] = s_n[(rt * 16 + li) * FZ_HL + kk * 4 + lq];
    __builtin_amdgcn_sched_barrier(0);
    if (TWO) {
      f32x4 au[2] = {f32x4{0.f, 0.f, 0.f, 0.f}, f32x4{0.f, 0.f, 0.f, 0.f}};
#pragma unroll
      for (int kk = 0; kk < 16; ++kk)
#pragma unroll
        for (int rt = 0; rt < 2; ++rt) au[rt] = __builtin_amdgcn_mfma_f32_16x16x4f32(areg[rt][kk], w1[kk], au[rt], 0, 0, 0);
#pragma unroll
      for (int rt = 0; rt < 2; ++rt)
#pragma unroll
        for (int r = 0; r < 4; ++r) {
          const int rl = rt * 16 + lq * 4 + r, row = row0 + rl;
          const float uv = au[rt][r] + b1;
          s_u[rl * FZ_HL + c] = uv;
          if (a.u != nullptr && row < a.M) a.u[(size_t)row * FZ_H + c] = uv;
        }
      FZ_LDS_BARRIER();
      if (w < 2) {
        float ar[16];
#pragma unroll
        for (int kk = 0; kk < 16; ++kk) ar[kk] = s_u[(w * 16 + li) * FZ_HL + kk * 4 + lq];
        f32x4 ao = f32x4{0.f, 0.f, 0.f, 0.f};
#pragma unroll
        for (int kk = 0; kk < 16; ++kk) ao = __builtin_amdgcn_mfma_f32_16x16x4f32(ar[kk], w2[kk], ao, 0, 0, 0);
#pragma unroll
        for (int r = 0; r < 4; ++r) {
          const int row = row0 + w * 16 + lq * 4 + r;
          if (row < a.M && li < a.n_out) a.out[(size_t)row * a.n_out + li] = ao[r] + b2;
        }
      }
    } else if (w < 2) {
      f32x4 ao = f32x4{0.f, 0.f, 0.f, 0.f};
#pragma unroll
      for (int kk = 0; kk < 16; ++kk) ao = __builtin_amdgcn_mfma_f32_16x16x4f32(areg[w][kk], w1[kk], ao, 0, 0, 0);
#pragma unroll
      for (int r = 0; r < 4; ++r) {
        const int row = row0 + w * 16 + lq * 4 + r;
        if (row < a.M && li < a.n_out) a.out[(size_t)row * a.n_out + li] = ao[r] + b1;
      }
    }
    FZ_LDS_BARRIER();
  }
}

#define RWH_W1L 65
template <bool TWO>
__global__ void __launch_bounds__(64 * RW_WAVES) gru1_head_fwd_rw_kernel(GruHeadArgs a) {
  extern __shared__ float sm[];
  float* sWh = sm;
  float* sW1 = sWh + 64 * RW_WIL;
  float* sW2 = sW1 + 64 * RWH_W1L;
  float* sB = sW2 + 64 * 17;
  const int tid = threadIdx.x, lane = tid & 63, w = tid >> 6, li = lane & 15, lq = lane >> 4;
  float* sY = sB + 144 + w * (16 * RW_YL);
  {
    static_assert(RW_WAVES == 16, "the staging below assumes 1024 threads");
    float4 vh[3];
#pragma unroll
    for (int j = 0; j < 3; ++j) vh[j] = reinterpret_cast<const float4*>(a.Wh)[j * 1024 + tid];
    float w1v[4] = {0.f, 0.f, 0.f, 0.f};
    float w2v = 0.0f;
    if (TWO) {
      const float4 v = reinterpret_cast<const float4*>(a.W1)[tid];
      w1v[0] = v.x; w1v[1] = v.y; w1v[2] = v.z; w1v[3] = v.w;
      { const int k = tid >> 4, c = tid & 15; w2v = (c < a.n_out) ? a.W2[k * a.n_out + c] : 0.0f; }
    } else {
      const int k = tid >> 4, c = tid & 15;
      w1v[0] = (c < a.n_out) ? a.W1[k * a.n_out + c] : 0.0f;
    }
#pragma unroll
    for (int j = 0; j < 3; ++j) {
      const int q = j * 1024 + tid, k = q / 48, c = (q - k * 48) * 4;
      float* d = sWh + k * RW_WIL + c;
      d[0] = vh[j].x; d[1] = vh[j].y; d[2] = vh[j].z; d[3] = vh[j].w;
    }
    if (TWO) {
      const int k = tid >> 4, c = (tid & 15) * 4;
      float* d = sW1 + k * RWH_W1L + c;
      d[0] = w1v[0]; d[1] = w1v[1]; d[2] = w1v[2]; d[3] = w1v[3];
      sW2[(tid >> 4) * 17 + (tid & 15)] = w2v;
    } else {
      sW1[(tid >> 4) * RWH_W1L + (tid & 15)] = w1v[0];
    }
    if (tid < 64) { sB[tid] = a.bhn[tid]; sB[64 + tid] = TWO ? a.b1[tid] : ((tid < a.n_out) ? a.b1[tid] : 0.0f); }
    if (tid < 16) sB[128 + tid] = (TWO && tid < a.n_out) ? a.b2[tid] : 0.0f;
  }
  __syncthreads();
  const int n_tiles = (a.M + 15) >> 4;
  for (int tile = w * gridDim.x + blockIdx.x; tile < n_tiles; tile += gridDim.x * RW_WAVES) {
    const int row0 = tile * 16;
    float A[16];
    {
      int row = row0 + li;
      row = row < a.M ? row : a.M - 1;
      if (a.h0 != nullptr) {
        const float4* p = reinterpret_cast<const float4*>(a.h0 + (size_t)row * FZ_H + lq * 16);
#pragma unroll
        for (int j = 0; j < 4; ++j) { const float4 v = p[j]; A[4 * j] = v.x; A[4 * j + 1] = v.y; A[4 * j + 2] = v.z; A[4 * j + 3] = v.w; }
      } else {
#pragma unroll
        for (int j = 0; j < 16; ++j) A[j] = 0.0f;
      }
    }
    float hp[4][4];
#pragma unroll
    for (int ct = 0; ct < 4; ++ct)
#pragma unroll
      for (int r = 0; r < 4; ++r) {
        int row = row0 + lq * 4 + r;
        row = row < a.M ? row : a.M - 1;
        hp[ct][r] = (a.h0 != nullptr) ? a.h0[(size_t)row * FZ_H + ct * 16 + li] : 0.0f;
      }
#pragma unroll
    for (int ct = 0; ct < 4; ++ct) {
      f32x4 ar, az, an = f32x4{0.f, 0.f, 0.f, 0.f};
      float gn[4];
#pragma unroll
      for (int r = 0; r < 4; ++r) {
        int row = row0 + lq * 4 + r;
        row = row < a.M ? row : a.M - 1;
        const float* gp = a.gi + (size_t)row * 192 + ct * 16 + li;
        ar[r] = gp[0]; az[r] = gp[64]; gn[r] = gp[128];
      }
#pragma unroll
      for (int kk = 0; kk < 16; ++kk) {
        const float* wr = sWh + (lq * 16 + kk) * RW_WIL + ct * 16 + li;
        ar = __builtin_amdgcn_mfma_f32_16x16x4f32(A[kk], wr[0], ar, 0, 0, 0);
        az = __builtin_amdgcn_mfma_f32_16x16x4f32(A[kk], wr[64], az, 0, 0, 0);
        an = __builtin_amdgcn_mfma_f32_16x16x4f32(A[kk], wr[128], an, 0, 0, 0);
      }
      const float bn = sB[ct * 16 + li];
#pragma unroll
      for (int r = 0; r < 4; ++r) {
        const float rg = gate_sigmoid(ar[r]);
        const float zg = gate_sigmoid(az[r]);
        const float ng = gate_tanh(gn[r] + rg * (an[r] + bn));
        const float hnew = (1.0f - zg) * ng + zg * hp[ct][r];
        sY[(lq * 4 + r) * RW_YL + ct * 16 + li] = hnew;
        const int row = row0 + lq * 4 + r;
        if (row < a.M) a.hs[(size_t)row * FZ_H + ct * 16 + li] = hnew;
      }
    }
#pragma unroll
    for (int j = 0; j < 4; ++j) {
      const float4 v = *reinterpret_cast<const float4*>(sY + li * RW_YL + lq * 16 + 4 * j);
      A[4 * j] = v.x; A[4 * j + 1] = v.y; A[4 * j + 2] = v.z; A[4 * j + 3] = v.w;
    }
    if (TWO) {
      f32x4 au[4];
#pragma unroll
      for (int ct = 0; ct < 4; ++ct) au[ct] = f32x4{0.f, 0.f, 0.f, 0.f};
#pragma unroll
      for (int kk = 0; kk < 16; ++kk) {
        const float* wr = sW1 + (lq * 16 + kk) * RWH_W1L + li;
#pragma unroll
        for (int ct = 0; ct < 4; ++ct) au[ct] = __builtin_amdgcn_mfma_f32_16x16x4f32(A[kk], wr[ct * 16], au[ct], 0, 0, 0);
      }
#pragma unroll
      for (int ct = 0; ct < 4; ++ct) {
        const float b = sB[64 + ct * 16 + li];
#pragma unroll
        for (int r = 0; r < 4; ++r) sY[(lq * 4 + r) * RW_YL + ct * 16 + li] = au[ct][r] + b;
      }
#pragma unroll
      for (int j = 0; j < 4; ++j) {
        const float4 v = *reinterpret_cast<const float4*>(sY + li * RW_YL + lq * 16 + 4 * j);
        A[4 * j] = v.x; A[4 * j + 1] = v.y; A[4 * j + 2] = v.z; A[4 * j + 3] = v.w;
      }
    }
    {
      f32x4 ao = f32x4{0.f, 0.f, 0.f, 0.f};
      const float* sWo = TWO ? sW2 : sW1;
      const int ld = TWO ? 17 : RWH_W1L;
#pragma unroll
      for (int kk = 0; kk < 16; ++kk) ao = __builtin_amdgcn_mfma_f32_16x16x4f32(A[kk], sWo[(lq * 16 + kk) * ld + li], ao, 0, 0, 0);
      const float b = TWO ? sB[128 + li] : sB[64 + li];
#pragma unroll
      for (int r = 0; r < 4; ++r) {
        const int row = row0 + lq * 4 + r;
        if (row < a.M && li < a.n_out) a.out[(size_t)row * a.n_out + li] = ao[r] + b;
      }
    }
  }
}

extern "C" int32_t dgppo_gru1_head_fwd(const float* gi, const float* Wh, const float* bhn, const float* h0, const float* W1,
                                       const float* b1, const float* W2, const float* b2, float* hs, float* hprev,
                                       float* gates, float* u, float* out, int32_t M, int32_t n_out, void* stream) {
  DGPPO_REQUIRE(M >= 0 && n_out >= 1 && n_out <= 16, "gru1_head_fwd: bad shape M=%d n_out=%d", M, n_out);
  DGPPO_REQUIRE(gi && Wh && bhn && W1 && b1 && hs && out, "gru1_head_fwd: NULL operand");
  const bool two = W2 != nullptr;
  DGPPO_REQUIRE(!two || b2, "gru1_head_fwd: W2 without b2");
  DGPPO_REQUIRE(two || !u, "gru1_head_fwd: u is only produced by the two-layer head");
  if (M == 0) return 0;
  GruHeadArgs a{gi, Wh, bhn, h0, W1, b1, W2, b2, hs, hprev, gates, u, out, M, n_out};
  if (!hprev && !gates && !u && ((reinterpret_cast<uintptr_t>(Wh) | reinterpret_cast<uintptr_t>(W1) | reinterpret_cast<uintptr_t>(h0)) & 15) == 0) {
    static thread_local int cus = 0;
    if (cus == 0) {
      int dev = 0;
      if (hipGetDevice(&dev) != hipSuccess ||
          hipDeviceGetAttribute(&cus, hipDeviceAttributeMultiprocessorCount, dev) != hipSuccess || cus < 1) cus = 256;
    }
    const size_t smem_rw = sizeof(float) * (64 * RW_WIL + 64 * RWH_W1L + 64 * 17 + 144 + RW_WAVES * 16 * RW_YL);
    static thread_local bool attr[2] = {false, false};
    if (!attr[two]) {
      const void* f = two ? reinterpret_cast<const void*>(&gru1_head_fwd_rw_kernel<true>)
                          : reinterpret_cast<const void*>(&gru1_head_fwd_rw_kernel<false>);
      const hipError_t e = hipFuncSetAttribute(f, hipFuncAttributeMaxDynamicSharedMemorySize, (int)smem_rw);
      DGPPO_REQUIRE(e == hipSuccess, "gru1_head_fwd: cannot reserve %zu bytes of LDS per workgroup: %s", smem_rw, hipGetErrorString(e));
      attr[two] = true;
    }
    const int tiles16 = (M + 15) / 16, grid_rw = tiles16 < cus ? tiles16 : cus;
    if (two) hipLaunchKernelGGL(gru1_head_fwd_rw_kernel<true>, dim3(grid_rw), dim3(64 * RW_WAVES), smem_rw, (hipStream_t)stream, a);
    else hipLaunchKernelGGL(gru1_head_fwd_rw_kernel<false>, dim3(grid_rw), dim3(64 * RW_WAVES), smem_rw, (hipStream_t)stream, a);
    DGPPO_LAUNCH_CHECK();
    return 0;
  }
  const size_t smem = sizeof(float) * 3 * FZ_RB * FZ_HL;
  const void* fn = two ? reinterpret_cast<const void*>(&gru1_head_fwd_kernel<true>)
                       : reinterpret_cast<const void*>(&gru1_head_fwd_kernel<false>);
  static thread_local int cap[2] = {0, 0};
  if (cap[two] == 0) {
    int per_cu = 0, dev = 0, cus = 256;
    if (hipOccupancyMaxActiveBlocksPerMultiprocessor(&per_cu, fn, 256, smem) != hipSuccess || per_cu < 1) per_cu = 1;
    if (hipGetDevice(&dev) != hipSuccess ||
        hipDeviceGetAttribute(&cus, hipDeviceAttributeMultiprocessorCount, dev) != hipSuccess || cus < 1) cus = 256;
    cap[two] = per_cu * cus;
  }
  const int tiles = (M + FZ_RB - 1) / FZ_RB;
  const int grid = tiles < cap[two] ? tiles : cap[two];
  if (two) hipLaunchKernelGGL(gru1_head_fwd_kernel<true>, dim3(grid), dim3(256), smem, (hipStream_t)stream, a);
  else hipLaunchKernelGGL(gru1_head_fwd_kernel<false>, dim3(grid), dim3(256), smem, (hipStream_t)stream, a);
  DGPPO_LAUNCH_CHECK();
  return 0;
}
```

dgppo_amd/nets.py:

```python
from __future__ import annotations

import math
from typing import Dict, List, Optional, Tuple

import numpy as np
import torch

from . import _native as N
from . import ops_nn as K

H_HEADS = 3
MSG_DIM = 32
OUT_DIM = 64
HID = 64


def _ceil4(x):
    return (x + 3) // 4 * 4


class Layout:
    def __init__(self):
        self.entries: Dict[str, Tuple[int, Tuple[int, ...]]] = {}
        self.size = 0

    def add(self, name, *shape):
        n = int(np.prod(shape))
        self.size = (self.size + 3) // 4 * 4
        self.entries[name] = (self.size, tuple(shape))
        self.size += n

    def view(self, flat: torch.Tensor, name: str) -> torch.Tensor:
        off, shape = self.entries[name]
        return flat[off:off + math.prod(shape)].view(shape)


def make_layout(kind: str, node_dim: int, gnn_layers: int, n_out: int, rnn: str = "gru", rnn_layers: int = 1) -> Layout:
    L = Layout()
    f = node_dim
    for l in range(gnn_layers):
        d = OUT_DIM if l == gnn_layers - 1 else MSG_DIM
        hd = H_HEADS * d
        for nm, shp in (("Wq", (f, hd)), ("bq", (hd,)), ("Wk", (f, hd)), ("bk", (hd,)), ("Wv", (f, hd)), ("bv", (hd,)),
                        ("We", (4, hd)), ("Wu", (f, d)), ("bu", (d,))):
            L.add(f"gnn{l}.{nm}", *shp)
        f = d
    for i in (1, 2):
        L.add(f"mlp.W{i}", 2 * HID if (kind == "Vhg" and i == 1) else HID, HID)
        L.add(f"mlp.b{i}", HID)
        L.add(f"mlp.g{i}", HID)
        L.add(f"mlp.be{i}", HID)
    assert rnn in ("gru", "lstm", "none"), rnn
    for l in range(rnn_layers if rnn == "lstm" else 0):
        L.add(f"lstm{l}.Wi", HID, 4 * HID)
        L.add(f"lstm{l}.Wh", HID, 4 * HID)
        L.add(f"lstm{l}.bh", 4 * HID)
    for l in range(rnn_layers if rnn == "gru" else 0):
        pre = "gru" if l == 0 else f"gru{l}"
        L.add(f"{pre}.Wi", HID, 3 * HID)
        L.add(f"{pre}.bi", 3 * HID)
        L.add(f"{pre}.Wh", HID, 3 * HID)
        L.add(f"{pre}.bhn", HID)
    if kind == "policy":
        L.add("head.Ws", HID, HID)
        L.add("head.bs", HID)
        L.add("head.Wms", HID, 2 * n_out)
        L.add("head.bms", 2 * n_out)
    else:
        L.add("head.Wo", HID, n_out)
        L.add("head.bo", n_out)
    return L


class Arena:

    def __init__(self, device):
        self.device = device
        self.bufs: Dict[str, torch.Tensor] = {}
        self.generation = 0

    def get(self, name: str, *shape, dtype=torch.float32, zero=False) -> torch.Tensor:
        n = math.prod(shape)
        b = self.bufs.get(name)
        if b is None or b.numel() < n or b.dtype != dtype:
            if b is not None:
                self.generation += 1
            b = torch.empty(max(n, 1), dtype=dtype, device=self.device)
            self.bufs[name] = b
        v = b[:n].view(shape)
        if zero:
            v.zero_()
        return v


class GraphFeats:

    def __init__(self, cfg: N.EnvCfg, G: int, arena: Arena, tag: str):
        self.cfg, self.G = cfg, G
        n, S = cfg.n_agents, cfg.fan_in
        self.n_other = cfg.num_nodes - 1 - n
        self.Fp = input_width(cfg)
        self.Xa = arena.get(f"{tag}.Xa0", G * n, self.Fp)
        self.Xo = arena.get(f"{tag}.Xo0", max(G * self.n_other, 1), self.Fp)[:G * self.n_other]
        self.efeat = arena.get(f"{tag}.efeat", G * n, S, 4)
        self.emask = arena.get(f"{tag}.emask", G * n, S)

    def compute(self, agent, agent_se, agent_st, goal, obst, hits, hits_se, hits_st, env_ids, n_env, n_time):
        assert n_env * n_time == self.G
        K.graph_feats(self.cfg, agent, agent_se, agent_st, goal, obst, hits, hits_se, hits_st, env_ids, n_env, n_time,
                      self.Xa, self.Xo if self.n_other > 0 else None, self.efeat, self.emask, self.Fp)
        return self

    def compute_record(self, step, slots: int, env, env_ids, n_env, n_time):
        cfg, n = self.cfg, self.cfg.n_agents
        se, st = slots, int(slots > 1)
        if cfg.is_vmas:
            return self.compute_vmas(step["agent"], se * n * 4, st * n * 4, step["body"], se * 4, st * 4, env["scene"], env_ids,
                                     n_env, n_time)
        ia, ih = n * cfg.state_dim, n * cfg.top_k * 2
        return self.compute(step["agent"], se * ia, st * ia, env["goal"], env.get("obst"), step.get("hits"), se * ih, st * ih,
                            env_ids, n_env, n_time)

    def compute_vmas(self, agent, agent_se, agent_st, body, body_se, body_st, scene, env_ids, n_env, n_time):
        assert n_env * n_time == self.G
        K.vmas_graph_feats(self.cfg, agent, agent_se, agent_st, body, body_se, body_st, scene, env_ids, n_env, n_time,
                           self.Xa, self.efeat, self.emask, self.Fp)
        return self


def input_width(cfg: N.EnvCfg) -> int:
    return _ceil4(cfg.node_dim) if cfg.is_vmas else 8


class Net:

    def __init__(self, kind: str, cfg: N.EnvCfg, gnn_layers: int, n_out: int, device, grads: Optional[torch.Tensor] = None,
                 rnn: str = "gru", rnn_layers: int = 1):
        assert kind in ("policy", "Vl", "Vh", "Vhg")
        self.kind, self.cfg, self.gnn_layers, self.n_out, self.device = kind, cfg, gnn_layers, n_out, device
        self.rnn, self.rnn_layers = rnn, (rnn_layers if rnn != "none" else 0)
        self.carry_dim = HID * max(self.rnn_layers, 1) * (2 if rnn == "lstm" else 1)
        self.layout = make_layout(kind, cfg.node_dim, gnn_layers, n_out, rnn, rnn_layers)
        self.params = torch.zeros(self.layout.size, device=device)
        if grads is None:
            grads = torch.zeros(self.layout.size, device=device)
        assert grads.shape == (self.layout.size,) and grads.is_contiguous() and grads.data_ptr() % 16 == 0
        self.grads = grads
        self.arena = Arena(device)
        self.ws_arena = Arena(device)
        self._views: Dict[tuple, torch.Tensor] = {}
        self.dims = []
        f = cfg.node_dim
        for l in range(gnn_layers):
            d = OUT_DIM if l == gnn_layers - 1 else MSG_DIM
            fp = input_width(cfg) if l == 0 else f
            kp = _ceil4(fp + H_HEADS * (fp + 4) + 1)
            self.dims.append((f, fp, d, kp))
            f = d
        self.prep_layout = Layout()
        for l, (f, fp, d, kp) in enumerate(self.dims):
            self.prep_layout.add(f"gnn{l}.Mcat", fp, H_HEADS * fp)
            self.prep_layout.add(f"gnn{l}.cvec", H_HEADS * fp)
            self.prep_layout.add(f"gnn{l}.Wout", kp, d)
        self.prep = torch.zeros(self.prep_layout.size, device=device)
        self.prep_grads = torch.zeros(self.prep_layout.size, device=device)

    def _cached(self, kind: str, layout, flat, name):
        key = (kind, name)
        v = self._views.get(key)
        if v is None:
            v = self._views[key] = layout.view(flat, name)
        return v

    def p(self, name):
        return self._cached("p", self.layout, self.params, name)

    def g(self, name):
        return self._cached("g", self.layout, self.grads, name)

    def pp(self, name):
        return self._cached("pp", self.prep_layout, self.prep, name)

    def pg(self, name):
        return self._cached("pg", self.prep_layout, self.prep_grads, name)

    def prepare(self):
        for l, (f, fp, d, kp) in enumerate(self.dims):
            q = lambda nm: self.p(f"gnn{l}.{nm}")
            K.gnn_prep(q("Wq"), q("bq"), q("Wk"), q("Wv"), q("bv"), q("We"), q("Wu"), self.pp(f"gnn{l}.Mcat"),
                       self.pp(f"gnn{l}.cvec"), self.pp(f"gnn{l}.Wout"), f, fp, d, H_HEADS, kp)

    def _xo_fusable(self, l: int) -> bool:
        if l != 0 or self.gnn_layers != 2:
            return False
        key = "_xo_ok"
        if not hasattr(self, key):
            f1, fp1, d1, kp1 = self.dims[1]
            setattr(self, key, self.dims[0][1] == 8 and self.dims[0][2] == 32 and fp1 == 32 and
                    K.attn_xo_supported(self.cfg, fp1, H_HEADS, kp1))
        return getattr(self, key)

    def zero_grads(self):
        self.grads.zero_()

    def forward(self, feats: GraphFeats, n_seq: int, T: int, h0: Optional[torch.Tensor], tag: str = "f",
                hs_out: Optional[torch.Tensor] = None, train: bool = True):
        cfg, G, A = self.cfg, feats.G, self.arena
        n = cfg.n_agents
        R = G * n
        Ro = G * feats.n_other
        act = {"feats": feats, "G": G, "n_seq": n_seq, "T": T}
        Xa, Xo = feats.Xa, feats.Xo
        xo_fused = None
        for l, (f, fp, d, kp) in enumerate(self.dims):
            qt = A.get(f"{tag}.qt{l}", R, H_HEADS * fp)
            K.dense_fwd(Xa, self.pp(f"gnn{l}.Mcat"), self.pp(f"gnn{l}.cvec"), qt)
            zcat = A.get(f"{tag}.zcat{l}", R, kp)
            attn = A.get(f"{tag}.attn{l}", R, cfg.fan_in, H_HEADS) if train else None
            if xo_fused is not None:
                K.attn_fwd_xo(cfg, fp, H_HEADS, kp, qt, Xa, xo_fused[0], xo_fused[1], xo_fused[2], feats.efeat, feats.emask, zcat, attn, G)
            else:
                K.attn_fwd(cfg, fp, H_HEADS, kp, qt, Xa, Xo if Ro > 0 else None, feats.efeat, feats.emask, zcat, attn, G)
            act[f"xo_fused{l}"] = xo_fused
            xo_fused = None
            Xa_n = A.get(f"{tag}.Xa{l + 1}", R, d)
            K.dense_fwd(zcat, self.pp(f"gnn{l}.Wout"), self.p(f"gnn{l}.bu"), Xa_n, act=1)
            act[f"Xa{l}"], act[f"Xo{l}"], act[f"qt{l}"], act[f"zcat{l}"], act[f"attn{l}"] = Xa, Xo, qt, zcat, attn
            if l < self.gnn_layers - 1 and Ro > 0:
                if self._xo_fusable(l):
                    xo_fused = (Xo, self.pp(f"gnn{l}.Wout")[:fp], self.p(f"gnn{l}.bu"))
                    Xo = None
                else:
                    Xo_n = A.get(f"{tag}.Xo{l + 1}", Ro, d)
                    K.dense_fwd(Xo, self.pp(f"gnn{l}.Wout")[:fp], self.p(f"gnn{l}.bu"), Xo_n, act=1)
                    Xo = Xo_n
            Xa = Xa_n
        act[f"Xa{self.gnn_layers}"] = Xa
        if self.kind == "Vl":
            pooled = A.get(f"{tag}.pool", G, OUT_DIM)
            K.mean_agents(Xa, pooled, G, n, OUT_DIM)
            x, Rh, n_inner = pooled, G, 1
        else:
            x, Rh, n_inner = Xa, R, n
        if self.kind == "Vhg":
            pooled = A.get(f"{tag}.pool", G, OUT_DIM)
            K.mean_agents(Xa, pooled, G, n, OUT_DIM)
            xcat = A.get(f"{tag}.xcat", R, 2 * OUT_DIM)
            xcat[:, :OUT_DIM].copy_(Xa)
            xcat.view(G, n, 2 * OUT_DIM)[:, :, OUT_DIM:].copy_(pooled.view(G, 1, OUT_DIM).expand(G, n, OUT_DIM))
            x = xcat
        act["Rh"], act["n_inner"], act["mlp_in"] = Rh, n_inner, x
        gi = A.get(f"{tag}.gi", Rh, 3 * HID)
        if self.kind == "Vhg" or self.rnn != "gru":
            sv = {nm: A.get(f"{tag}.{nm}", Rh, w) for nm, w in (("p1", HID), ("y1", HID), ("st1", 2), ("p2", HID), ("y2", HID), ("st2", 2))}
            K.dense_fwd(x, self.p("mlp.W1"), self.p("mlp.b1"), sv["p1"])
            K.ln_relu_fwd(sv["p1"], self.p("mlp.g1"), self.p("mlp.be1"), sv["y1"], sv["st1"])
            K.dense_fwd(sv["y1"], self.p("mlp.W2"), self.p("mlp.b2"), sv["p2"])
            K.ln_relu_fwd(sv["p2"], self.p("mlp.g2"), self.p("mlp.be2"), sv["y2"], sv["st2"])
            if self.rnn == "gru":
                K.dense_fwd(sv["y2"], self.p("gru.Wi"), self.p("gru.bi"), gi)
            act.update(sv)
        else:
            saves = None
            if train:
                saves = tuple(A.get(f"{tag}.{nm}{i}", Rh, w) for i in (1, 2) for nm, w in (("p", HID), ("y", HID), ("st", 2)))
                for i in (1, 2):
                    act[f"p{i}"], act[f"y{i}"], act[f"st{i}"] = saves[3 * (i - 1):3 * i]
            K.mlp_gi_fwd(x, self.p("mlp.W1"), self.p("mlp.b1"), self.p("mlp.g1"), self.p("mlp.be1"), self.p("mlp.W2"),
                         self.p("mlp.b2"), self.p("mlp.g2"), self.p("mlp.be2"), self.p("gru.Wi"), self.p("gru.bi"), gi, saves)
        assert n_seq * T == Rh, (n_seq, T, Rh)
        L, CD = self.rnn_layers, self.carry_dim
        if h0 is not None:
            assert tuple(h0.shape) == (n_seq, CD), (tuple(h0.shape), n_seq, CD)
        if hs_out is not None:
            assert tuple(hs_out.shape) == (Rh, CD), (tuple(hs_out.shape), Rh, CD)
        act["gi"] = gi
        simple = (self.rnn == "gru" and L == 1)
        if simple:
            hs = hs_out if hs_out is not None else A.get(f"{tag}.hs", Rh, HID)
            hprev_is_h0 = train and T == 1 and h0 is not None and self.kind != "policy"
            hprev = A.get(f"{tag}.hprev", Rh, HID) if (train and not hprev_is_h0) else None
            gates = A.get(f"{tag}.gates", Rh, 4 * HID) if train else None
            feat = hs
            act["hs"], act["hprev"], act["gates"] = hs, hprev, gates
        fused_tail = (simple and T == 1 and self.kind == "policy")
        if simple and not fused_tail:
            K.gru_fwd(gi, self.p("gru.Wh"), self.p("gru.bhn"), h0, hs, hprev, gates, n_seq, T, n_inner)
            if hprev_is_h0:
                act["hprev"] = h0
        if self.rnn == "none":
            feat = act["y2"]
            if hs_out is not None:
                if h0 is not None and T == 1:
                    hs_out.copy_(h0)
                else:
                    hs_out.zero_()
        elif self.rnn == "lstm":
            x_l = act["y2"]
            act["stack"] = []
            for l in range(L):
                zi = A.get(f"{tag}.zi{l}", Rh, 4 * HID)
                for half in (slice(0, 2 * HID), slice(2 * HID, 4 * HID)):
                    K.dense_fwd(x_l, self.p(f"lstm{l}.Wi")[:, half], None, zi[:, half])
                c0_l = h0_l = None
                if h0 is not None:
                    c0_l, h0_l = A.get(f"{tag}.c0_{l}", n_seq, HID), A.get(f"{tag}.h0_{l}", n_seq, HID)
                    c0_l.copy_(h0[:, (2 * l) * HID:(2 * l + 1) * HID])
                    h0_l.copy_(h0[:, (2 * l + 1) * HID:(2 * l + 2) * HID])
                cs_l, hs_l = A.get(f"{tag}.cs{l}", Rh, HID), A.get(f"{tag}.hs{l}", Rh, HID)
                cprev_l = A.get(f"{tag}.cprev{l}", Rh, HID) if train else None
                hprev_l = A.get(f"{tag}.hprev{l}", Rh, HID) if train else None
                gates_l = A.get(f"{tag}.gates{l}", Rh, 4 * HID) if train else None
                K.lstm_fwd(zi, self.p(f"lstm{l}.Wh"), self.p(f"lstm{l}.bh"), c0_l, h0_l, cs_l, hs_l, cprev_l, hprev_l, gates_l,
                           n_seq, T, n_inner)
                if hs_out is not None:
                    hs_out[:, (2 * l) * HID:(2 * l + 1) * HID].copy_(cs_l)
                    hs_out[:, (2 * l + 1) * HID:(2 * l + 2) * HID].copy_(hs_l)
                act["stack"].append(dict(x=x_l, hs=hs_l, cprev=cprev_l, hprev=hprev_l, gates=gates_l))
                x_l = hs_l
            feat = x_l
        elif not simple:
            x_l = None
            act["stack"] = []
            for l in range(L):
                pre = "gru" if l == 0 else f"gru{l}"
                gi_l = gi if l == 0 else A.get(f"{tag}.gi{l}", Rh, 3 * HID)
                if l > 0:
                    K.dense_fwd(x_l, self.p(f"{pre}.Wi"), self.p(f"{pre}.bi"), gi_l)
                h0_l = None
                if h0 is not None:
                    h0_l = A.get(f"{tag}.h0_{l}", n_seq, HID)
                    h0_l.copy_(h0[:, l * HID:(l + 1) * HID])
                hs_l = A.get(f"{tag}.hs{l}", Rh, HID)
                hprev_l = A.get(f"{tag}.hprev{l}", Rh, HID) if train else None
                gates_l = A.get(f"{tag}.gates{l}", Rh, 4 * HID) if train else None
                K.gru_fwd(gi_l, self.p(f"{pre}.Wh"), self.p(f"{pre}.bhn"), h0_l, hs_l, hprev_l, gates_l, n_seq, T, n_inner)
                if hs_out is not None:
                    hs_out[:, l * HID:(l + 1) * HID].copy_(hs_l)
                act["stack"].append(dict(x=x_l, gi=gi_l, hs=hs_l, hprev=hprev_l, gates=gates_l))
                x_l = hs_l
            feat = x_l
        act["feat"] = feat
        if self.kind == "policy":
            u = A.get(f"{tag}.u", Rh, HID) if (train or not fused_tail) else None
            ms = A.get(f"{tag}.ms", Rh, 4)
            if fused_tail:
                K.gru1_head_fwd(gi, self.p("gru.Wh"), self.p("gru.bhn"), h0, self.p("head.Ws"), self.p("head.bs"),
                                self.p("head.Wms"), self.p("head.bms"), hs, hprev, gates, u, ms)
            else:
                K.dense_fwd(feat, self.p("head.Ws"), self.p("head.bs"), u)
                K.dense_fwd(u, self.p("head.Wms"), self.p("head.bms"), ms)
            act["u"], act["ms"] = u, ms
        else:
            v = A.get(f"{tag}.v", Rh, self.n_out)
            K.dense_fwd(feat, self.p("head.Wo"), self.p("head.bo"), v)
            act["v"] = v
        return act

    def backward(self, act, dout: torch.Tensor, tag: str = "b"):
        A = self.arena
        ws_floats = getattr(self, "_bwdw_floats", 16 << 20)

        def _alloc(n_floats):
            self._bwdw_floats = max(ws_floats, n_floats)
            return self.ws_arena.get(f"{tag}.bwdw_ws", self._bwdw_floats)
        batch = K.BwdWBatch(self.device, _alloc) if dout.is_cuda else None
        if batch is not None:
            batch.__enter__()
        try:
            self._backward_body(act, dout, tag)
        except BaseException:
            if batch is not None:
                batch.__exit__(RuntimeError, None, None)
            raise
        if batch is not None:
            batch.__exit__(None, None, None)
        for l, (f, fp, d, kp) in enumerate(self.dims):
            q = lambda nm: self.p(f"gnn{l}.{nm}")
            gq = lambda nm: self.g(f"gnn{l}.{nm}")
            K.gnn_unprep(self.pg(f"gnn{l}.Mcat"), self.pg(f"gnn{l}.cvec"), self.pg(f"gnn{l}.Wout"), q("Wq"), q("bq"), q("Wk"),
                         gq("Wq"), gq("bq"), gq("Wk"), gq("Wv"), gq("bv"), gq("We"), gq("Wu"), f, fp, d, H_HEADS, kp)
        self.prep_grads.zero_()

    def _backward_body(self, act, dout: torch.Tensor, tag: str):
        cfg, A = self.cfg, self.arena
        G, Rh, n_inner, n_seq, T = act["G"], act["Rh"], act["n_inner"], act["n_seq"], act["T"]
        n = cfg.n_agents
        R = G * n
        feats: GraphFeats = act["feats"]
        Ro = G * feats.n_other
        feat = act["feat"]
        fused_trunk = self.rnn == "gru" and self.rnn_layers == 1 and self.kind != "Vhg" and dout.is_cuda
        dgi0 = None
        dhs = A.get(f"{tag}.dhs", Rh, HID)
        if self.kind == "policy":
            K.dense_bwd_w(act["u"], dout, self.g("head.Wms"), self.g("head.bms"))
            du = A.get(f"{tag}.du", Rh, HID)
            K.dense_fwd(dout, self.p("head.Wms"), None, du, trans_w=True)
            K.dense_bwd_w(feat, du, self.g("head.Ws"), self.g("head.bs"))
            K.dense_fwd(du, self.p("head.Ws"), None, dhs, trans_w=True)
        else:
            K.dense_bwd_w(feat, dout, self.g("head.Wo"), self.g("head.bo"))
            K.dense_fwd(dout, self.p("head.Wo"), None, dhs, trans_w=True)
        if self.rnn == "none":
            dy = dhs
        elif self.rnn == "lstm":
            stack = act["stack"]
            for l in range(len(stack) - 1, -1, -1):
                st = stack[l]
                dz = A.get(f"{tag}.dz_lstm{l}", Rh, 4 * HID)
                K.lstm_bwd(dhs, self.p(f"lstm{l}.Wh"), st["cprev"], st["gates"], dz, n_seq, T, n_inner)
                for half in (slice(0, 2 * HID), slice(2 * HID, 4 * HID)):
                    K.dense_bwd_w(st["hprev"], dz[:, half], self.g(f"lstm{l}.Wh")[:, half], self.g(f"lstm{l}.bh")[half])
                    K.dense_bwd_w(st["x"], dz[:, half], self.g(f"lstm{l}.Wi")[:, half], None)
                dx = A.get(f"{tag}.dy" if l == 0 else f"{tag}.dx{l}", Rh, HID)
                K.dense_fwd(dz, self.p(f"lstm{l}.Wi"), None, dx, trans_w=True)
                dhs = dx
            dy = dhs
        else:
            stack = act.get("stack") or [dict(x=None, gi=act["gi"], hs=act["hs"], hprev=act["hprev"], gates=act["gates"])]
            if act.get("stack") is None and dout.is_cuda:
                st = stack[0]
                dgi = A.get(f"{tag}.dgi0", Rh, 3 * HID)
                dhn = A.get(f"{tag}.dhn0", Rh, HID)
                K.gru_bwd_dhn(dhs, self.p("gru.Wh"), st["hprev"], st["gates"], dgi, dhn, n_seq, T, n_inner)
                K.gru_bwd_w(act["y2"], st["hprev"], dgi, dhn, self.g("gru.Wi"), self.g("gru.bi"), self.g("gru.Wh"), self.g("gru.bhn"))
                if fused_trunk:
                    dgi0 = dgi
                else:
                    dhs = A.get(f"{tag}.dy", Rh, HID)
                    K.dense_fwd(dgi, self.p("gru.Wi"), None, dhs, trans_w=True)
                stack = []
            for l in range(len(stack) - 1, -1, -1):
                st = stack[l]
                pre = "gru" if l == 0 else f"gru{l}"
                dgi = A.get(f"{tag}.dgi{l}", Rh, 3 * HID)
                dgh = A.get(f"{tag}.dgh{l}", Rh, 3 * HID)
                K.gru_bwd(dhs, self.p(f"{pre}.Wh"), st["hprev"], st["gates"], dgi, dgh, n_seq, T, n_inner)
                K.dense_bwd_w(st["hprev"], dgh[:, :2 * HID], self.g(f"{pre}.Wh")[:, :2 * HID], None)
                K.dense_bwd_w(st["hprev"], dgh[:, 2 * HID:], self.g(f"{pre}.Wh")[:, 2 * HID:], self.g(f"{pre}.bhn"))
                x_l = act["y2"] if l == 0 else st["x"]
                K.dense_bwd_w(x_l, dgi, self.g(f"{pre}.Wi"), self.g(f"{pre}.bi"))
                if l == 0 and fused_trunk:
                    dgi0 = dgi
                    break
                dx = A.get(f"{tag}.dy" if l == 0 else f"{tag}.dx{l}", Rh, HID)
                K.dense_fwd(dgi, self.p(f"{pre}.Wi"), None, dx, trans_w=True)
                dhs = dx
            dy = dhs
        x_in = {1: act["mlp_in"], 2: act["y1"]}
        top = act[f"Xa{self.gnn_layers}"]
        if fused_trunk:
            dpre2, dpre1 = A.get(f"{tag}.dpre2", Rh, HID), A.get(f"{tag}.dpre1", Rh, HID)
            dy = A.get(f"{tag}.dyy1", Rh, HID)
            K.mlp_gi_bwd(dgi0, self.p("gru.Wi"), self.p("mlp.W2"), self.p("mlp.W1"), self.p("mlp.g2"), self.p("mlp.g1"),
                         act["p2"], act["y2"], act["st2"], act["p1"], act["y1"], act["st1"],
                         top if self.kind in ("policy", "Vh") else None, dpre2, dpre1, dy,
                         self.g("mlp.g2"), self.g("mlp.be2"), self.g("mlp.g1"), self.g("mlp.be1"))
            K.dense_bwd_w(x_in[2], dpre2, self.g("mlp.W2"), self.g("mlp.b2"))
            K.dense_bwd_w(x_in[1], dpre1, self.g("mlp.W1"), self.g("mlp.b1"))
        for i in (() if fused_trunk else (2, 1)):
            dpre = A.get(f"{tag}.dpre{i}", Rh, HID)
            K.ln_relu_bwd(act[f"p{i}"], act[f"y{i}"], act[f"st{i}"], self.p(f"mlp.g{i}"), dy, dpre, self.g(f"mlp.g{i}"),
                          self.g(f"mlp.be{i}"))
            K.dense_bwd_w(x_in[i], dpre, self.g(f"mlp.W{i}"), self.g(f"mlp.b{i}"))
            dy = A.get(f"{tag}.dyy{i}", Rh, HID if not (self.kind == "Vhg" and i == 1) else 2 * HID)
            K.dense_fwd(dpre, self.p(f"mlp.W{i}"), None, dy, trans_w=True,
                        relu_mask=top if (i == 1 and self.kind in ("policy", "Vh")) else None)
        if self.kind == "Vl":
            dXa = A.get(f"{tag}.dXaL", R, OUT_DIM)
            K.mean_agents(dy, dXa, G, n, OUT_DIM, backward=True, relu_mask=top)
        elif self.kind == "Vhg":
            dXa = A.get(f"{tag}.dXaL", R, OUT_DIM)
            dXa.copy_(dy[:, :OUT_DIM])
            dglob = A.get(f"{tag}.dglob", R, OUT_DIM)
            dglob.copy_(dy[:, OUT_DIM:])
            dpool = A.get(f"{tag}.dpool", G, OUT_DIM)
            K.mean_agents(dglob, dpool, G, n, OUT_DIM)
            K.mean_agents(dpool, dXa, G, n, OUT_DIM, backward=2, relu_mask=top)
        else:
            dXa = dy
        dXo = None
        for l in range(self.gnn_layers - 1, -1, -1):
            f, fp, d, kp = self.dims[l]
            K.dense_bwd_w(act[f"zcat{l}"], dXa, self.pg(f"gnn{l}.Wout"), self.g(f"gnn{l}.bu"))
            dz = A.get(f"{tag}.dz{l}", R, kp)
            K.dense_fwd(dXa, self.pp(f"gnn{l}.Wout"), None, dz, trans_w=True)
            if dXo is not None:
                K.dense_bwd_w(act[f"Xo{l}"], dXo, self.pg(f"gnn{l}.Wout")[:fp], self.g(f"gnn{l}.bu"))
            dqt = A.get(f"{tag}.dqt{l}", R, H_HEADS * fp)
            need_dx = l > 0
            dXa_l = A.get(f"{tag}.dXa{l}", R, fp) if need_dx else None
            dXo_prev = dXo
            dXo_l = A.get(f"{tag}.dXo{l}", Ro, fp) if (need_dx and Ro > 0) else None
            more_dXo = dXo_prev is not None and dXo_l is not None
            xf = act.get(f"xo_fused{l}")
            if xf is not None and dXa_l is not None and not more_dXo:
                ws = A.get(f"{tag}.xo_ws", K.attn_xo_workspace_floats(G), 1).view(-1)
                K.attn_bwd_xo_dw(cfg, fp, H_HEADS, kp, dz, act[f"attn{l}"], act[f"qt{l}"], act[f"Xa{l}"], xf[0], xf[1], xf[2],
                                 feats.efeat, dqt, dXa_l, self.pg(f"gnn{l - 1}.Wout")[:self.dims[l - 1][1]], self.g(f"gnn{l - 1}.bu"), ws, G)
                dXo_l = None
            elif xf is not None:
                K.attn_bwd_xo(cfg, fp, H_HEADS, kp, dz, act[f"attn{l}"], act[f"qt{l}"], act[f"Xa{l}"], xf[0], xf[1], xf[2],
                              feats.efeat, dqt, dXa_l, dXo_l, G, relu_xo=(dXo_l is not None and not more_dXo))
            else:
                K.attn_bwd(cfg, fp, H_HEADS, kp, dz, act[f"attn{l}"], act[f"qt{l}"], act[f"Xa{l}"],
                           act[f"Xo{l}"] if Ro > 0 else None, feats.efeat, dqt, dXa_l, dXo_l, G,
                           relu_xo=(dXo_l is not None and not more_dXo))
            K.dense_bwd_w(act[f"Xa{l}"], dqt, self.pg(f"gnn{l}.Mcat"), self.pg(f"gnn{l}.cvec"))
            if need_dx:
                K.dense_fwd(dqt, self.pp(f"gnn{l}.Mcat"), None, dXa_l, accumulate=True, trans_w=True, relu_mask=act[f"Xa{l}"])
                if more_dXo:
                    K.dense_fwd(dXo_prev, self.pp(f"gnn{l}.Wout")[:fp], None, dXo_l, accumulate=True, trans_w=True,
                                relu_mask=act[f"Xo{l}"])
            dXa, dXo = dXa_l, dXo_l

    def load_tree(self, tree: dict):
        t = tree["params"]
        to = lambda x: torch.as_tensor(np.asarray(x), dtype=torch.float32).to(self.device)
        if self.kind == "policy":
            base, gnn, head_name = t["PolicyNet_0"], t["PolicyNet_0"]["GraphTransformerGNN_0"], "PolicyGNNHead"
        else:
            base, gnn, head_name = t, t["GraphTransformerGNN_0"], "ValueGNNHead"
        for l in range(self.gnn_layers):
            gl = gnn[f"GraphTransformer_{l}"]
            for nm, dn, key in (("Wq", "Dense_0", "kernel"), ("bq", "Dense_0", "bias"), ("Wk", "Dense_1", "kernel"),
                                ("bk", "Dense_1", "bias"), ("Wv", "Dense_2", "kernel"), ("bv", "Dense_2", "bias"),
                                ("We", "Dense_3", "kernel"), ("Wu", "Dense_4", "kernel"), ("bu", "Dense_4", "bias")):
                self.p(f"gnn{l}.{nm}").copy_(to(gl[dn][key]))
        hd = base[head_name]
        for i in (1, 2):
            self.p(f"mlp.W{i}").copy_(to(hd[f"Dense_{i - 1}"]["kernel"]))
            self.p(f"mlp.b{i}").copy_(to(hd[f"Dense_{i - 1}"]["bias"]))
            self.p(f"mlp.g{i}").copy_(to(hd[f"LayerNorm_{i - 1}"]["scale"]))
            self.p(f"mlp.be{i}").copy_(to(hd[f"LayerNorm_{i - 1}"]["bias"]))
        for l in range(self.rnn_layers if self.rnn == "lstm" else 0):
            lc = base["RNN_0"][f"LSTMCell_{3 * l + 2}"]
            self.p(f"lstm{l}.Wi").copy_(torch.cat([to(lc[k]["kernel"]) for k in ("ii", "if", "ig", "io")], dim=1))
            self.p(f"lstm{l}.Wh").copy_(torch.cat([to(lc[k]["kernel"]) for k in ("hi", "hf", "hg", "ho")], dim=1))
            self.p(f"lstm{l}.bh").copy_(torch.cat([to(lc[k]["bias"]) for k in ("hi", "hf", "hg", "ho")]))
        for l in range(self.rnn_layers if self.rnn == "gru" else 0):
            pre = "gru" if l == 0 else f"gru{l}"
            gr = base["RNN_0"][f"GRUCell_{2 * l + 1}"]
            self.p(f"{pre}.Wi").copy_(torch.cat([to(gr[k]["kernel"]) for k in ("ir", "iz", "in")], dim=1))
            self.p(f"{pre}.bi").copy_(torch.cat([to(gr[k]["bias"]) for k in ("ir", "iz", "in")]))
            self.p(f"{pre}.Wh").copy_(torch.cat([to(gr[k]["kernel"]) for k in ("hr", "hz", "hn")], dim=1))
            self.p(f"{pre}.bhn").copy_(to(gr["hn"]["bias"]))
        if self.kind == "policy":
            self.p("head.Ws").copy_(to(t["ScaleHid"]["kernel"]))
            self.p("head.bs").copy_(to(t["ScaleHid"]["bias"]))
            self.p("head.Wms").copy_(torch.cat([to(t["OutputDenseMean"]["kernel"]), to(t["OutputDenseStdTrans"]["kernel"])], 1))
            self.p("head.bms").copy_(torch.cat([to(t["OutputDenseMean"]["bias"]), to(t["OutputDenseStdTrans"]["bias"])]))
        else:
            self.p("head.Wo").copy_(to(t["Dense_0"]["kernel"]))
            self.p("head.bo").copy_(to(t["Dense_0"]["bias"]))
        self.prepare()

    def to_tree(self, flat: Optional[torch.Tensor] = None) -> dict:
        flat = self.params if flat is None else flat
        v = lambda nm: self.layout.view(flat, nm).detach().cpu().numpy().copy()
        gnn = {}
        for l in range(self.gnn_layers):
            gnn[f"GraphTransformer_{l}"] = {
                "Dense_0": {"kernel": v(f"gnn{l}.Wq"), "bias": v(f"gnn{l}.bq")},
                "Dense_1": {"kernel": v(f"gnn{l}.Wk"), "bias": v(f"gnn{l}.bk")},
                "Dense_2": {"kernel": v(f"gnn{l}.Wv"), "bias": v(f"gnn{l}.bv")},
                "Dense_3": {"kernel": v(f"gnn{l}.We")},
                "Dense_4": {"kernel": v(f"gnn{l}.Wu"), "bias": v(f"gnn{l}.bu")},
            }
        head = {}
        for i in (1, 2):
            head[f"Dense_{i - 1}"] = {"kernel": v(f"mlp.W{i}"), "bias": v(f"mlp.b{i}")}
            head[f"LayerNorm_{i - 1}"] = {"scale": v(f"mlp.g{i}"), "bias": v(f"mlp.be{i}")}
        rnn = {}
        for l in range(self.rnn_layers if self.rnn == "lstm" else 0):
            Wi, Wh, bh = v(f"lstm{l}.Wi"), v(f"lstm{l}.Wh"), v(f"lstm{l}.bh")
            cell = {}
            for q, g_ in enumerate("ifgo"):
                cell["i" + g_] = {"kernel": Wi[:, q * 64:(q + 1) * 64]}
                cell["h" + g_] = {"kernel": Wh[:, q * 64:(q + 1) * 64], "bias": bh[q * 64:(q + 1) * 64]}
            rnn[f"LSTMCell_{3 * l + 2}"] = cell
        for l in range(self.rnn_layers if self.rnn == "gru" else 0):
            pre = "gru" if l == 0 else f"gru{l}"
            Wi, bi, Wh = v(f"{pre}.Wi"), v(f"{pre}.bi"), v(f"{pre}.Wh")
            rnn[f"GRUCell_{2 * l + 1}"] = {
                "ir": {"kernel": Wi[:, :64], "bias": bi[:64]}, "iz": {"kernel": Wi[:, 64:128], "bias": bi[64:128]},
                "in": {"kernel": Wi[:, 128:], "bias": bi[128:]}, "hr": {"kernel": Wh[:, :64]}, "hz": {"kernel": Wh[:, 64:128]},
                "hn": {"kernel": Wh[:, 128:], "bias": v(f"{pre}.bhn")}}
        if self.kind == "policy":
            Wms, bms = v("head.Wms"), v("head.bms")
            k = self.n_out
            return {"params": {
                "PolicyNet_0": dict({"GraphTransformerGNN_0": gnn, "PolicyGNNHead": head}, **({"RNN_0": rnn} if rnn else {})),
                "ScaleHid": {"kernel": v("head.Ws"), "bias": v("head.bs")},
                "OutputDenseMean": {"kernel": Wms[:, :k], "bias": bms[:k]},
                "OutputDenseStdTrans": {"kernel": Wms[:, k:], "bias": bms[k:]}}}
        return {"params": dict({"GraphTransformerGNN_0": gnn, "ValueGNNHead": head, "Dense_0": {"kernel": v("head.Wo"), "bias": v("head.bo")}},
                               **({"RNN_0": rnn} if rnn else {}))}
```

dgppo_amd/ops_nn.py:

```python
from __future__ import annotations

import ctypes as C
from typing import Optional

import torch

from . import _native as N

FLOPS = [0.0]


def _mat(t: torch.Tensor, name: str):
    if t.dim() != 2:
        raise ValueError(f"{name} must be 2-D, got {tuple(t.shape)}")
    if not t.is_cuda:
        raise RuntimeError(f"{name} must live on the GPU (the HIP path has no CPU fallback)")
    if t.dtype != torch.float32:
        raise TypeError(f"{name} must be float32")
    if t.shape[1] > 1 and t.stride(1) != 1:
        raise ValueError(f"{name} must have unit inner stride")
    ld = t.stride(0) if t.shape[0] > 1 else max(t.shape[1], t.stride(0))
    return C.c_void_p(t.data_ptr()), int(ld), int(t.shape[0]), int(t.shape[1])


def _p(t: Optional[torch.Tensor], name="tensor", dtype=torch.float32):
    return N.ptr(t, dtype, name)


def dense_fwd(X, W, bias, Y, act: int = 0, accumulate: bool = False, trans_w: bool = False, relu_mask=None):
    xp, ldx, M, K = _mat(X, "X")
    wp, ldw, wr, wc = _mat(W, "W")
    yp, ldy, My, Ncol = _mat(Y, "Y")
    Kw, Nw = (wc, wr) if trans_w else (wr, wc)
    if Kw != K or Nw != Ncol or My != M:
        raise ValueError(f"dense_fwd: shape mismatch X{tuple(X.shape)} W{tuple(W.shape)} trans={trans_w} Y{tuple(Y.shape)}")
    if bias is not None:
        N.expect_shape(bias, (Ncol,), "bias")
    mp, ldm = C.c_void_p(0), 0
    if relu_mask is not None:
        mp, ldm, Mm, Nm = _mat(relu_mask, "relu_mask")
        if (Mm, Nm) != (M, Ncol):
            raise ValueError(f"dense_fwd: relu_mask {tuple(relu_mask.shape)} does not match Y {tuple(Y.shape)}")
    FLOPS[0] += 2.0 * M * K * Ncol
    rc = N.lib().dgppo_dense_fwd(xp, ldx, wp, ldw, _p(bias, "bias"), yp, ldy, M, K, Ncol, int(act), int(accumulate),
                                 int(trans_w), mp, ldm, N.stream_ptr())
    N.check(rc, "dgppo_dense_fwd")


def mlp_gi_fwd(X, W1, b1, g1, be1, W2, b2, g2, be2, Wi, bi, gi, saves=None):
    xp, ldx, M, K = _mat(X, "X")
    if K != 64:
        raise ValueError(f"mlp_gi_fwd: X must be [M, 64], got {tuple(X.shape)}")
    for t, shp, nm in ((W1, (64, 64), "W1"), (W2, (64, 64), "W2"), (Wi, (64, 192), "Wi"), (b1, (64,), "b1"), (g1, (64,), "g1"),
                       (be1, (64,), "be1"), (b2, (64,), "b2"), (g2, (64,), "g2"), (be2, (64,), "be2"), (bi, (192,), "bi"),
                       (gi, (M, 192), "gi")):
        N.expect_shape(t, shp, nm)
    sv = [None] * 6
    if saves is not None:
        for t, shp, nm in zip(saves, ((M, 64), (M, 64), (M, 2), (M, 64), (M, 64), (M, 2)), ("p1", "y1", "st1", "p2", "y2", "st2")):
            N.expect_shape(t, shp, nm)
        sv = list(saves)
    FLOPS[0] += 2.0 * M * (64 * 64 * 2 + 64 * 192)
    rc = N.lib().dgppo_mlp_gi_fwd(xp, ldx, _p(W1), _p(b1), _p(g1), _p(be1), _p(W2), _p(b2), _p(g2), _p(be2), _p(Wi), _p(bi),
                                  *[_p(t) for t in sv], _p(gi), M, N.stream_ptr())
    N.check(rc, "dgppo_mlp_gi_fwd")


def mlp_gi_bwd(dgi, Wi, W2, W1, g2, g1, p2, y2, st2, p1, y1, st1, relu_mask, dpre2, dpre1, dx, dg2, db2, dg1, db1):
    M = dgi.shape[0]
    N.expect_shape(dgi, (M, 192), "dgi")
    for t, shp, nm in ((Wi, (64, 192), "Wi"), (W2, (64, 64), "W2"), (W1, (64, 64), "W1"), (g2, (64,), "g2"), (g1, (64,), "g1"),
                       (p2, (M, 64), "p2"), (y2, (M, 64), "y2"), (st2, (M, 2), "st2"), (p1, (M, 64), "p1"), (y1, (M, 64), "y1"),
                       (st1, (M, 2), "st1"), (dpre2, (M, 64), "dpre2"), (dpre1, (M, 64), "dpre1"), (dx, (M, 64), "dx"),
                       (dg2, (64,), "dg2"), (db2, (64,), "db2"), (dg1, (64,), "dg1"), (db1, (64,), "db1")):
        N.expect_shape(t, shp, nm)
    mp, ldm = (None, 0)
    if relu_mask is not None:
        mp, ldm, Mm, Km = _mat(relu_mask, "relu_mask")
        if (Mm, Km) != (M, 64):
            raise ValueError(f"mlp_gi_bwd: relu_mask must be [M, 64], got {tuple(relu_mask.shape)}")
    FLOPS[0] += 2.0 * M * (64 * 64 * 2 + 64 * 192)
    rc = N.lib().dgppo_mlp_gi_bwd(_p(dgi), _p(Wi), _p(W2), _p(W1), _p(g2), _p(g1), _p(p2), _p(y2), _p(st2), _p(p1), _p(y1), _p(st1),
                                  mp if mp is not None else C.c_void_p(0), ldm, _p(dpre2), _p(dpre1), _p(dx), 64,
                                  _p(dg2), _p(db2), _p(dg1), _p(db1), M, N.stream_ptr())
    N.check(rc, "dgppo_mlp_gi_bwd")


def gru1_head_fwd(gi, Wh, bhn, h0, W1, b1, W2, b2, hs, hprev, gates, u, out):
    M = gi.shape[0]
    n_out = out.shape[1]
    N.expect_shape(gi, (M, 192), "gi"); N.expect_shape(Wh, (64, 192), "Wh"); N.expect_shape(bhn, (64,), "bhn")
    N.expect_shape(hs, (M, 64), "hs"); N.expect_shape(out, (M, n_out), "out")
    if h0 is not None:
        N.expect_shape(h0, (M, 64), "h0")
    if W2 is not None:
        N.expect_shape(W1, (64, 64), "W1"); N.expect_shape(b1, (64,), "b1")
        N.expect_shape(W2, (64, n_out), "W2"); N.expect_shape(b2, (n_out,), "b2")
    else:
        N.expect_shape(W1, (64, n_out), "W1"); N.expect_shape(b1, (n_out,), "b1")
    for t, shp, nm in ((hprev, (M, 64), "hprev"), (gates, (M, 256), "gates"), (u, (M, 64), "u")):
        if t is not None:
            N.expect_shape(t, shp, nm)
    FLOPS[0] += 2.0 * M * (64 * 192 + (64 * 64 + 64 * n_out if W2 is not None else 64 * n_out))
    rc = N.lib().dgppo_gru1_head_fwd(_p(gi), _p(Wh), _p(bhn), _p(h0), _p(W1), _p(b1), _p(W2), _p(b2), _p(hs), _p(hprev),
                                     _p(gates), _p(u), _p(out), M, n_out, N.stream_ptr())
    N.check(rc, "dgppo_gru1_head_fwd")


_WS: dict = {}


def _bwd_w_workspace(device, K: int, Ncol: int) -> torch.Tensor:
    lib = N.lib()
    lib.dgppo_dense_bwd_w_workspace_bytes.restype = C.c_int64
    need = int(lib.dgppo_dense_bwd_w_workspace_bytes(C.c_int32(K), C.c_int32(Ncol)))
    need = min(need, 64 << 20)
    key = (device.index, torch.cuda.current_stream(device).cuda_stream)
    ws = _WS.get(key)
    if ws is None or ws.numel() * 4 < need:
        ws = torch.empty(need // 4, dtype=torch.float32, device=device)
        _WS[key] = ws
    return ws


class ReduceDesc(C.Structure):
    _fields_ = [("part", C.c_void_p), ("dW", C.c_void_p), ("db", C.c_void_p), ("part_stride", C.c_int32), ("slabs", C.c_int32),
                ("ldw", C.c_int32), ("K", C.c_int32), ("N", C.c_int32), ("pending", C.c_int32)]


class BwdWBatch:
    _active = {}

    def __init__(self, device, alloc):
        self.device, self.alloc = device, alloc
        self.key = None
        self.descs = []
        self.offset = 0
        self.ws = None

    def __enter__(self):
        self.key = (self.device.index, torch.cuda.current_stream(self.device).cuda_stream)
        if self.key in BwdWBatch._active:
            raise RuntimeError("BwdWBatch: nested batches on one stream")
        BwdWBatch._active[self.key] = self
        return self

    def region(self, nbytes: int):
        nbytes = (nbytes + 255) & ~255
        if self.ws is None or self.ws.numel() * 4 < self.offset + nbytes:
            if self.descs:
                self.flush()
            self.ws = self.alloc(max(self.offset + nbytes, 2 * (self.ws.numel() * 4 if self.ws is not None else 0)) // 4)
        view = self.ws[self.offset // 4:(self.offset + nbytes) // 4]
        self.offset += nbytes
        return view

    def flush(self):
        if self.descs:
            arr = (ReduceDesc * len(self.descs))(*self.descs)
            N.check(N.lib().dgppo_dense_bwd_w_reduce_batch(arr, C.c_int32(len(self.descs)), N.stream_ptr()),
                    "dgppo_dense_bwd_w_reduce_batch")
        self.descs = []
        self.offset = 0

    def __exit__(self, *exc):
        try:
            if exc[0] is None:
                self.flush()
        finally:
            BwdWBatch._active.pop(self.key, None)
        return False


def dense_bwd_w(X, dY, dW, db=None):
    xp, ldx, M, K = _mat(X, "X")
    yp, ldy, My, Ncol = _mat(dY, "dY")
    wp, ldw, Kw, Nw = _mat(dW, "dW")
    if My != M or Kw != K or Nw != Ncol:
        raise ValueError(f"dense_bwd_w: shape mismatch X{tuple(X.shape)} dY{tuple(dY.shape)} dW{tuple(dW.shape)}")
    if db is not None:
        N.expect_shape(db, (Ncol,), "db")
    FLOPS[0] += 2.0 * M * K * Ncol
    batch = BwdWBatch._active.get((X.device.index, torch.cuda.current_stream(X.device).cuda_stream)) if X.is_cuda else None
    if batch is not None:
        lib = N.lib()
        lib.dgppo_dense_bwd_w_workspace_bytes.restype = C.c_int64
        need = min(int(lib.dgppo_dense_bwd_w_workspace_bytes(C.c_int32(K), C.c_int32(Ncol))), 64 << 20)
        ws = batch.region(need)
        d = ReduceDesc()
        rc = lib.dgppo_dense_bwd_w_deferred(xp, ldx, yp, ldy, wp, ldw, _p(db, "db"), M, K, Ncol, _p(ws, "workspace"),
                                            C.c_int64(ws.numel() * 4), C.byref(d), N.stream_ptr())
        N.check(rc, "dgppo_dense_bwd_w_deferred")
        if d.pending:
            batch.descs.append(d)
        return
    ws = _bwd_w_workspace(X.device, K, Ncol)
    rc = N.lib().dgppo_dense_bwd_w(xp, ldx, yp, ldy, wp, ldw, _p(db, "db"), M, K, Ncol, _p(ws, "workspace"),
                                   C.c_int64(ws.numel() * 4), N.stream_ptr())
    N.check(rc, "dgppo_dense_bwd_w")


def _check_strided(fn: str, name: str, t_, se: int, st: int, inner: tuple, env_ids, n_env: int, n_time: int):
    if not (t_.is_cuda and t_.dtype == torch.float32):
        raise ValueError(f"{fn}: {name} must be a float32 CUDA tensor")
    want, acc = [], 1
    for d in reversed(inner):
        want.append(acc)
        acc *= d
    if tuple(t_.shape[-len(inner):]) != tuple(inner) or list(t_.stride()[-len(inner):]) != want[::-1]:
        raise ValueError(f"{fn}: the trailing {inner} block of {name} must be dense (got shape {tuple(t_.shape)}, "
                         f"strides {t_.stride()})")
    avail = t_.untyped_storage().nbytes() // 4 - t_.storage_offset()
    if env_ids is None and (n_env - 1) * se + (n_time - 1) * st + acc > avail:
        raise ValueError(f"{fn}: {name}: the strides reach beyond its storage")


def graph_feats(cfg: N.EnvCfg, agent, agent_se, agent_st, goal, obst, hits, hits_se, hits_st, env_ids, n_env, n_time,
                Xa, Xo, efeat, emask, Fp):
    G = n_env * n_time
    n, S = cfg.n_agents, cfg.fan_in
    n_other = cfg.num_nodes - 1 - n
    N.expect_shape(Xa, (G * n, Fp), "Xa")
    if n_other > 0:
        N.expect_shape(Xo, (G * n_other, Fp), "Xo")
    N.expect_shape(efeat, (G * n, S, 4), "efeat")
    N.expect_shape(emask, (G * n, S), "emask")
    _check_strided("graph_feats", "agent", agent, agent_se, agent_st, (n, cfg.state_dim), env_ids, n_env, n_time)
    if hits is not None:
        _check_strided("graph_feats", "hits", hits, hits_se, hits_st, (n, cfg.top_k, 2), env_ids, n_env, n_time)
    rc = N.lib().dgppo_graph_feats(
        C.byref(cfg), C.c_void_p(agent.data_ptr()), C.c_int64(agent_se), C.c_int64(agent_st), _p(goal, "goal"),
        _p(obst, "obst") if (obst is not None and not cfg.is_lidar) else C.c_void_p(0),
        C.c_void_p(hits.data_ptr()) if hits is not None else C.c_void_p(0), C.c_int64(hits_se), C.c_int64(hits_st),
        _p(env_ids, "env_ids", torch.int32), C.c_int32(n_env), C.c_int32(n_time), _p(Xa, "Xa"), _p(Xo, "Xo"),
        _p(efeat, "efeat"), _p(emask, "emask"), C.c_int32(Fp), N.stream_ptr())
    N.check(rc, "dgppo_graph_feats")


def vmas_graph_feats(cfg: N.EnvCfg, agent, agent_se, agent_st, body, body_se, body_st, scene, env_ids, n_env, n_time,
                     Xa, efeat, emask, Fp):
    G = n_env * n_time
    n = cfg.n_agents
    N.expect_shape(Xa, (G * n, Fp), "Xa")
    N.expect_shape(efeat, (G * n, n, 4), "efeat")
    N.expect_shape(emask, (G * n, n), "emask")
    _check_strided("vmas_graph_feats", "agent", agent, agent_se, agent_st, (n, 4), env_ids, n_env, n_time)
    _check_strided("vmas_graph_feats", "body", body, body_se, body_st, (4,), env_ids, n_env, n_time)
    rc = N.lib().dgppo_vmas_graph_feats(
        C.byref(cfg), C.c_void_p(agent.data_ptr()), C.c_int64(agent_se), C.c_int64(agent_st), C.c_void_p(body.data_ptr()),
        C.c_int64(body_se), C.c_int64(body_st), _p(scene, "scene"), _p(env_ids, "env_ids", torch.int32), C.c_int32(n_env),
        C.c_int32(n_time), _p(Xa, "Xa"), _p(efeat, "efeat"), _p(emask, "emask"), C.c_int32(Fp), N.stream_ptr())
    N.check(rc, "dgppo_vmas_graph_feats")


def attn_fwd(cfg, F, H, Kp, qt, Xa, Xo, efeat, emask, zcat, attn, G):
    n, S = cfg.n_agents, cfg.fan_in
    N.expect_shape(qt, (G * n, H * F), "qt")
    N.expect_shape(Xa, (G * n, F), "Xa")
    N.expect_shape(zcat, (G * n, Kp), "zcat")
    if attn is not None:
        N.expect_shape(attn, (G * n, S, H), "attn")
    FLOPS[0] += 2.0 * G * n * H * S * (2 * F + 4)
    rc = N.lib().dgppo_attn_fwd(C.byref(cfg), F, H, Kp, _p(qt), _p(Xa), _p(Xo), _p(efeat), _p(emask), _p(zcat), _p(attn),
                                G, N.stream_ptr())
    N.check(rc, "dgppo_attn_fwd")


def attn_bwd(cfg, F, H, Kp, dzcat, attn, qt, Xa, Xo, efeat, dqt, dXa, dXo, G, relu_xo: bool = False):
    n = cfg.n_agents
    N.expect_shape(dzcat, (G * n, Kp), "dzcat")
    N.expect_shape(dqt, (G * n, H * F), "dqt")
    if dXa is not None:
        N.expect_shape(dXa, (G * n, F), "dXa")
    FLOPS[0] += 4.0 * G * n * H * cfg.fan_in * (2 * F + 4)
    rc = N.lib().dgppo_attn_bwd(C.byref(cfg), F, H, Kp, _p(dzcat), _p(attn), _p(qt), _p(Xa), _p(Xo), _p(efeat), _p(dqt),
                                _p(dXa), _p(dXo), int(relu_xo), G, N.stream_ptr())
    N.check(rc, "dgppo_attn_bwd")


def attn_xo_supported(cfg, F, H, Kp) -> bool:
    return bool(N.lib().dgppo_attn_xo_supported(C.byref(cfg), F, H, Kp))


def _wo_ptr(Wo):
    if not Wo.is_cuda or Wo.dtype != torch.float32:
        raise TypeError("Wo must be a float32 GPU tensor")
    return C.c_void_p(Wo.data_ptr())


def _wo_ld(Wo):
    if Wo.dim() != 2 or Wo.shape[0] != 8 or Wo.shape[1] < 32 or Wo.stride(1) != 1:
        raise ValueError(f"Wo must be [8, >= 32] with contiguous rows, got {tuple(Wo.shape)} strides {Wo.stride()}")
    return int(Wo.stride(0))


def attn_fwd_xo(cfg, F, H, Kp, qt, Xa, Xo_raw, Wo, bo, efeat, emask, zcat, attn, G):
    n, S = cfg.n_agents, cfg.fan_in
    N.expect_shape(qt, (G * n, H * F), "qt")
    N.expect_shape(Xa, (G * n, F), "Xa")
    N.expect_shape(zcat, (G * n, Kp), "zcat")
    N.expect_shape(Xo_raw, (G * (cfg.num_nodes - 1 - n), 8), "Xo_raw")
    N.expect_shape(bo, (32,), "bo")
    if attn is not None:
        N.expect_shape(attn, (G * n, S, H), "attn")
    FLOPS[0] += 2.0 * G * n * H * S * (2 * F + 4) + 2.0 * G * (cfg.num_nodes - 1 - n) * 8 * 32
    rc = N.lib().dgppo_attn_fwd_xo(C.byref(cfg), F, H, Kp, _p(qt), _p(Xa), _p(Xo_raw), _wo_ptr(Wo),
                                   _wo_ld(Wo), _p(bo), _p(efeat), _p(emask), _p(zcat), _p(attn), G, N.stream_ptr())
    N.check(rc, "dgppo_attn_fwd_xo")


def attn_bwd_xo(cfg, F, H, Kp, dzcat, attn, qt, Xa, Xo_raw, Wo, bo, efeat, dqt, dXa, dXo, G, relu_xo: bool = False):
    n = cfg.n_agents
    N.expect_shape(dzcat, (G * n, Kp), "dzcat")
    N.expect_shape(dqt, (G * n, H * F), "dqt")
    N.expect_shape(Xo_raw, (G * (cfg.num_nodes - 1 - n), 8), "Xo_raw")
    if dXa is not None:
        N.expect_shape(dXa, (G * n, F), "dXa")
    FLOPS[0] += 4.0 * G * n * H * cfg.fan_in * (2 * F + 4) + 2.0 * G * (cfg.num_nodes - 1 - n) * 8 * 32
    rc = N.lib().dgppo_attn_bwd_xo(C.byref(cfg), F, H, Kp, _p(dzcat), _p(attn), _p(qt), _p(Xa), _p(Xo_raw),
                                   _wo_ptr(Wo), _wo_ld(Wo), _p(bo), _p(efeat), _p(dqt), _p(dXa), _p(dXo),
                                   int(relu_xo), G, N.stream_ptr())
    N.check(rc, "dgppo_attn_bwd_xo")


def attn_xo_workspace_floats(G: int) -> int:
    return int(N.lib().dgppo_attn_xo_workspace_bytes(int(G))) // 4


def attn_bwd_xo_dw(cfg, F, H, Kp, dzcat, attn, qt, Xa, Xo_raw, Wo, bo, efeat, dqt, dXa, dWo, dbo, workspace, G):
    n = cfg.n_agents
    N.expect_shape(dzcat, (G * n, Kp), "dzcat")
    N.expect_shape(dqt, (G * n, H * F), "dqt")
    N.expect_shape(dXa, (G * n, F), "dXa")
    N.expect_shape(Xo_raw, (G * (cfg.num_nodes - 1 - n), 8), "Xo_raw")
    N.expect_shape(dbo, (32,), "dbo")
    FLOPS[0] += 4.0 * G * n * H * cfg.fan_in * (2 * F + 4) + 4.0 * G * (cfg.num_nodes - 1 - n) * 8 * 32
    rc = N.lib().dgppo_attn_bwd_xo_dw(C.byref(cfg), F, H, Kp, _p(dzcat), _p(attn), _p(qt), _p(Xa), _p(Xo_raw), _wo_ptr(Wo), _wo_ld(Wo),
                                      _p(bo), _p(efeat), _p(dqt), _p(dXa), _wo_ptr(dWo), _wo_ld(dWo), _p(dbo), _p(workspace),
                                      C.c_int64(workspace.numel() * 4), G, N.stream_ptr())
    N.check(rc, "dgppo_attn_bwd_xo_dw")


def gnn_prep(Wq, bq, Wk, Wv, bv, We, Wu, Mcat, cvec, Wout, F, Fp, D, H, Kp):
    rc = N.lib().dgppo_gnn_prep(_p(Wq), _p(bq), _p(Wk), _p(Wv), _p(bv), _p(We), _p(Wu), _p(Mcat), _p(cvec), _p(Wout),
                                F, Fp, D, H, Kp, N.stream_ptr())
    N.check(rc, "dgppo_gnn_prep")


def gnn_unprep(dMcat, dcvec, dWout, Wq, bq, Wk, dWq, dbq, dWk, dWv, dbv, dWe, dWu, F, Fp, D, H, Kp):
    rc = N.lib().dgppo_gnn_unprep(_p(dMcat), _p(dcvec), _p(dWout), _p(Wq), _p(bq), _p(Wk), _p(dWq), _p(dbq), _p(dWk),
                                  _p(dWv), _p(dbv), _p(dWe), _p(dWu), F, Fp, D, H, Kp, N.stream_ptr())
    N.check(rc, "dgppo_gnn_unprep")


def ln_relu_fwd(x, gamma, beta, y, stats):
    M = x.shape[0]
    N.expect_shape(x, (M, 64), "x")
    N.expect_shape(y, (M, 64), "y")
    rc = N.lib().dgppo_ln_relu_fwd(_p(x), _p(gamma), _p(beta), _p(y), _p(stats), M, N.stream_ptr())
    N.check(rc, "dgppo_ln_relu_fwd")


def ln_relu_bwd(x, y, stats, gamma, dy, dx, dgamma, dbeta):
    M = x.shape[0]
    rc = N.lib().dgppo_ln_relu_bwd(_p(x), _p(y), _p(stats), _p(gamma), _p(dy), _p(dx), _p(dgamma), _p(dbeta), M,
                                   N.stream_ptr())
    N.check(rc, "dgppo_ln_relu_bwd")


def gru_fwd(gi, Wh, bhn, h0, hs, hprev, gates, n_seq, T, n_inner):
    rows = n_seq * T
    N.expect_shape(gi, (rows, 192), "gi")
    N.expect_shape(hs, (rows, 64), "hs")
    N.expect_shape(Wh, (64, 192), "Wh")
    if h0 is not None:
        N.expect_shape(h0, (n_seq, 64), "h0")
    FLOPS[0] += 2.0 * rows * 64 * 192
    rc = N.lib().dgppo_gru_fwd(_p(gi), _p(Wh), _p(bhn), _p(h0), _p(hs), _p(hprev), _p(gates), n_seq, T, n_inner,
                               N.stream_ptr())
    N.check(rc, "dgppo_gru_fwd")


def gru_bwd(dhs, Wh, hprev, gates, dgi, dgh, n_seq, T, n_inner):
    rows = n_seq * T
    N.expect_shape(dhs, (rows, 64), "dhs")
    N.expect_shape(dgi, (rows, 192), "dgi")
    N.expect_shape(dgh, (rows, 192), "dgh")
    FLOPS[0] += 2.0 * rows * 64 * 192
    rc = N.lib().dgppo_gru_bwd(_p(dhs), _p(Wh), _p(hprev), _p(gates), _p(dgi), _p(dgh), n_seq, T, n_inner, N.stream_ptr())
    N.check(rc, "dgppo_gru_bwd")


def gru_bwd_dhn(dhs, Wh, hprev, gates, dgi, dhn, n_seq, T, n_inner):
    rows = n_seq * T
    N.expect_shape(dhs, (rows, 64), "dhs")
    N.expect_shape(dgi, (rows, 192), "dgi")
    N.expect_shape(dhn, (rows, 64), "dhn")
    FLOPS[0] += 2.0 * rows * 64 * 192
    rc = N.lib().dgppo_gru_bwd_dhn(_p(dhs), _p(Wh), _p(hprev), _p(gates), _p(dgi), _p(dhn), n_seq, T, n_inner, N.stream_ptr())
    N.check(rc, "dgppo_gru_bwd_dhn")


def gru_bwd_w(x, hprev, dgi, dhn, dWi, dbi, dWh, dbhn):
    xp, ldx, M, Kx = _mat(x, "x")
    hp, ldh, Mh, Kh = _mat(hprev, "hprev")
    wip, ldwi, _, _ = _mat(dWi, "dWi")
    whp, ldwh, _, _ = _mat(dWh, "dWh")
    if Kx != 64 or (Mh, Kh) != (M, 64) or tuple(dWi.shape) != (64, 192) or tuple(dWh.shape) != (64, 192):
        raise ValueError(f"gru_bwd_w: shape mismatch x{tuple(x.shape)} hprev{tuple(hprev.shape)} dWi{tuple(dWi.shape)} "
                         f"dWh{tuple(dWh.shape)}")
    N.expect_shape(dgi, (M, 192), "dgi"); N.expect_shape(dhn, (M, 64), "dhn")
    N.expect_shape(dbi, (192,), "dbi"); N.expect_shape(dbhn, (64,), "dbhn")
    FLOPS[0] += 2.0 * M * 64 * (128 + 64 + 192)
    lib = N.lib()
    lib.dgppo_gru_bwd_w_workspace_bytes.restype = C.c_int64
    need = int(lib.dgppo_gru_bwd_w_workspace_bytes())
    batch = BwdWBatch._active.get((x.device.index, torch.cuda.current_stream(x.device).cuda_stream)) if x.is_cuda else None
    if batch is not None:
        ws = batch.region(need)
        d = (ReduceDesc * 3)()
        pend = d
    else:
        key = (x.device.index, torch.cuda.current_stream(x.device).cuda_stream, "gru")
        ws = _WS.get(key)
        if ws is None or ws.numel() * 4 < need:
            ws = _WS[key] = torch.empty(need // 4, dtype=torch.float32, device=x.device)
        pend = None
    rc = lib.dgppo_gru_bwd_w(xp, ldx, hp, ldh, _p(dgi, "dgi"), _p(dhn, "dhn"), wip, ldwi, _p(dbi, "dbi"), whp, ldwh,
                             _p(dbhn, "dbhn"), M, _p(ws, "workspace"), C.c_int64(ws.numel() * 4), pend, N.stream_ptr())
    N.check(rc, "dgppo_gru_bwd_w")
    if batch is not None:
        for i in range(3):
            if d[i].pending:
                batch.descs.append(ReduceDesc.from_buffer_copy(d[i]))


def policy_head(ms, eps, action_in, action, log_pi, entropy, n_agents, mode, log_pi_old=None, adv=None, dms=None,
                stats=None, clip_eps=0.25, coef_ent=0.01):
    rows = ms.shape[0]
    N.expect_shape(ms, (rows, 4), "ms")
    rc = N.lib().dgppo_policy_head(_p(ms), _p(eps), _p(action_in), _p(action), _p(log_pi), _p(entropy), rows, n_agents,
                                   mode, _p(log_pi_old), _p(adv), _p(dms), _p(stats), C.c_float(clip_eps),
                                   C.c_float(coef_ent), N.stream_ptr())
    N.check(rc, "dgppo_policy_head")


def value_loss(v, target, dv, stats):
    rc = N.lib().dgppo_value_loss(_p(v), _p(target), _p(dv), _p(stats), v.numel(), N.stream_ptr())
    N.check(rc, "dgppo_value_loss")


def mean_agents(x, y, G, n, D, backward=False, relu_mask=None):
    rc = N.lib().dgppo_mean_agents(_p(x), _p(y), G, n, D, int(backward), _p(relu_mask), N.stream_ptr())
    N.check(rc, "dgppo_mean_agents")


def relu_bwd(dy, y):
    rc = N.lib().dgppo_relu_bwd(_p(dy), _p(y), C.c_int64(dy.numel()), N.stream_ptr())
    N.check(rc, "dgppo_relu_bwd")


def lstm_fwd(zi, Wh, bh, c0, h0, cs, hs, cprev, hprev, gates, n_seq, T, n_inner):
    rows = n_seq * T
    N.expect_shape(zi, (rows, 256), "zi"); N.expect_shape(Wh, (64, 256), "Wh"); N.expect_shape(bh, (256,), "bh")
    N.expect_shape(cs, (rows, 64), "cs"); N.expect_shape(hs, (rows, 64), "hs")
    for t, nm in ((c0, "c0"), (h0, "h0")):
        if t is not None:
            N.expect_shape(t, (n_seq, 64), nm)
    FLOPS[0] += 2.0 * rows * 64 * 256
    rc = N.lib().dgppo_lstm_fwd(_p(zi), _p(Wh), _p(bh), _p(c0), _p(h0), _p(cs), _p(hs), _p(cprev), _p(hprev), _p(gates),
                                n_seq, T, n_inner, N.stream_ptr())
    N.check(rc, "dgppo_lstm_fwd")


def lstm_bwd(dhs, Wh, cprev, gates, dz, n_seq, T, n_inner):
    rows = n_seq * T
    N.expect_shape(dhs, (rows, 64), "dhs"); N.expect_shape(dz, (rows, 256), "dz")
    FLOPS[0] += 2.0 * rows * 64 * 256
    rc = N.lib().dgppo_lstm_bwd(_p(dhs), _p(Wh), _p(cprev), _p(gates), _p(dz), n_seq, T, n_inner, N.stream_ptr())
    N.check(rc, "dgppo_lstm_bwd")
```

include/dgppo_hip.h:

```cpp
#ifndef DGPPO_HIP_H
#define DGPPO_HIP_H

#include <stdint.h>

#ifdef __cplusplus
extern "C" {
#endif

#define DGPPO_ABI_VERSION 3

enum {
  DGPPO_ENV_LIDAR_SPREAD = 0,
  DGPPO_ENV_LIDAR_TARGET = 1,
  DGPPO_ENV_LIDAR_BICYCLE_TARGET = 2,
  DGPPO_ENV_MPE_SPREAD = 3,
  DGPPO_ENV_MPE_TARGET = 4,
  DGPPO_ENV_LIDAR_LINE = 5,
  DGPPO_ENV_MPE_LINE = 6,
  DGPPO_ENV_MPE_FORMATION = 7,
  DGPPO_ENV_MPE_CORRIDOR = 8,
  DGPPO_ENV_MPE_CONNECT_SPREAD = 9,
  DGPPO_ENV_VMAS_REVERSE_TRANSPORT = 10
};
enum {
  DGPPO_GOALS_NODES = 0,
  DGPPO_GOALS_LINE = 1,
  DGPPO_GOALS_LINE_INTERIOR = 2,
  DGPPO_GOALS_CIRCLE = 3
};

#define DGPPO_RECT_STRIDE 16

typedef struct dgppo_env_cfg {
  int32_t kind;
  int32_t n_agents;
  int32_t n_goals;
  int32_t n_obs;
  int32_t n_rays;
  int32_t top_k;
  int32_t state_dim;
  int32_t node_dim;
  float area_size;
  float dt;
  float car_radius;
  float comm_radius;
  float obs_radius;
  float dist2goal;
  float two_car_radius;
  float lidar_mask_radius;
  float eye_offset;
  float car_plus_obs;
  float vel_limit;
  float reset_min_dist;
  int32_t reward_goals;
  int32_t n_cost;
  float obs_mask_radius;
  float y_limit;
  float connect_radius;
  float reset_side_y;
  float goal_shift_y;
  float line_min_dist;
} dgppo_env_cfg;

typedef struct dgppo_graph_out {
  float*   nodes;
  float*   edges;
  float*   states;
  int32_t* receivers;
  int32_t* senders;
  int32_t* node_type;
  int32_t* n_node;
  int32_t* n_edge;
} dgppo_graph_out;

int32_t     dgppo_abi_version(void);
const char* dgppo_last_error(void);

int32_t dgppo_env_num_nodes(const dgppo_env_cfg* cfg);
int32_t dgppo_env_num_edges(const dgppo_env_cfg* cfg);


int32_t dgppo_env_step(const dgppo_env_cfg* cfg,
                       const float* agent, const float* action, const float* goal,
                       const float* obst, const float* hits,
                       const float* ray_cos, const float* ray_sin,
                       float* next_agent, float* next_hits, float* reward, float* cost,
                       const dgppo_graph_out* gout, int32_t B, void* stream);

int32_t dgppo_graph_materialize(const dgppo_env_cfg* cfg,
                                const float* agent, const float* goal,
                                const float* obst, const float* hits,
                                const dgppo_graph_out* gout, int32_t B, void* stream);

int32_t dgppo_env_reset(const dgppo_env_cfg* cfg, const uint64_t* seeds,
                        float* agent, float* goal, float* obst, int32_t B, void* stream);
int32_t dgppo_env_reset_checked(const dgppo_env_cfg* cfg, const uint64_t* seeds, float* agent, float* goal, float* obst,
                                int32_t* n_failed, int32_t B, void* stream);


int32_t dgppo_vmas_reset_checked(const dgppo_env_cfg* cfg, const uint64_t* seeds, float* agent, float* body, float* scene,
                                 int32_t* n_failed, int32_t B, void* stream);
int32_t dgppo_vmas_step(const dgppo_env_cfg* cfg, const float* agent, const float* body, const float* scene,
                        const float* action, float* next_agent, float* next_body, float* reward, float* cost,
                        const dgppo_graph_out* gout, int32_t B, void* stream);
int32_t dgppo_vmas_graph_materialize(const dgppo_env_cfg* cfg, const float* agent, const float* body, const float* scene,
                                     const dgppo_graph_out* gout, int32_t B, void* stream);
int32_t dgppo_vmas_graph_feats(const dgppo_env_cfg* cfg, const float* agent, int64_t agent_se, int64_t agent_st,
                               const float* body, int64_t body_se, int64_t body_st, const float* scene,
                               const int32_t* env_ids, int32_t n_env, int32_t n_time, float* Xa, float* efeat, float* emask,
                               int32_t Fp, void* stream);

int32_t dgppo_randn(uint64_t seed, uint64_t offset, float* out, int64_t n_elem, void* stream);
int32_t dgppo_randn_rows(uint64_t seed, float* out, int64_t rows, int64_t row_len, int64_t global_row_len,
                         int64_t col_offset, void* stream);


int32_t dgppo_dense_fwd(const float* X, int32_t ldx, const float* W, int32_t ldw, const float* bias, float* Y,
                        int32_t ldy, int32_t M, int32_t K, int32_t N, int32_t act, int32_t accumulate,
                        int32_t trans_w, const float* relu_mask, int32_t ldm, void* stream);
int32_t dgppo_dense_bwd_w(const float* X, int32_t ldx, const float* dY, int32_t ldy, float* dW, int32_t ldw,
                          float* db, int32_t M, int32_t K, int32_t N, float* workspace, int64_t workspace_bytes,
                          void* stream);
int32_t dgppo_mlp_gi_fwd(const float* X, int32_t ldx, const float* W1, const float* b1, const float* g1, const float* be1,
                         const float* W2, const float* b2, const float* g2, const float* be2, const float* Wi,
                         const float* bi, float* p1, float* y1, float* st1, float* p2, float* y2, float* st2, float* gi,
                         int32_t M, void* stream);
int32_t dgppo_mlp_gi_bwd(const float* dgi, const float* Wi, const float* W2, const float* W1, const float* g2,
                         const float* g1, const float* p2, const float* y2, const float* st2, const float* p1,
                         const float* y1, const float* st1, const float* relu_mask, int32_t ldm, float* dpre2, float* dpre1,
                         float* dx, int32_t lddx, float* dg2, float* db2, float* dg1, float* db1, int32_t M, void* stream);
#define DGPPO_REDUCE_BATCH 16
typedef struct dgppo_reduce_desc {
  const float* part;
  float* dW;
  float* db;
  int32_t part_stride, slabs, ldw, K, N;
  int32_t pending;
} dgppo_reduce_desc;
int32_t dgppo_dense_bwd_w_deferred(const float* X, int32_t ldx, const float* dY, int32_t ldy, float* dW, int32_t ldw,
                                   float* db, int32_t M, int32_t K, int32_t N, float* workspace, int64_t workspace_bytes,
                                   dgppo_reduce_desc* pending, void* stream);
int32_t dgppo_dense_bwd_w_reduce_batch(const dgppo_reduce_desc* descs, int32_t n, void* stream);
int32_t dgppo_gru1_head_fwd(const float* gi, const float* Wh, const float* bhn, const float* h0, const float* W1,
                            const float* b1, const float* W2, const float* b2, float* hs, float* hprev, float* gates,
                            float* u, float* out, int32_t M, int32_t n_out, void* stream);
int64_t dgppo_dense_bwd_w_workspace_bytes(int32_t K, int32_t N);

int32_t dgppo_graph_feats(const dgppo_env_cfg* cfg, const float* agent, int64_t agent_se, int64_t agent_st,
                          const float* goal, const float* obst, const float* hits, int64_t hits_se, int64_t hits_st,
                          const int32_t* env_ids, int32_t n_env, int32_t n_time, float* Xa, float* Xo, float* efeat,
                          float* emask, int32_t Fp, void* stream);

int32_t dgppo_attn_fwd(const dgppo_env_cfg* cfg, int32_t F, int32_t H, int32_t Kp, const float* qt, const float* Xa,
                       const float* Xo, const float* efeat, const float* emask, float* zcat, float* attn, int32_t G,
                       void* stream);
int32_t dgppo_attn_bwd(const dgppo_env_cfg* cfg, int32_t F, int32_t H, int32_t Kp, const float* dzcat,
                       const float* attn, const float* qt, const float* Xa, const float* Xo, const float* efeat,
                       float* dqt, float* dXa, float* dXo, int32_t relu_xo, int32_t G, void* stream);
int32_t dgppo_attn_xo_supported(const dgppo_env_cfg* cfg, int32_t F, int32_t H, int32_t Kp);
int32_t dgppo_attn_fwd_xo(const dgppo_env_cfg* cfg, int32_t F, int32_t H, int32_t Kp, const float* qt, const float* Xa,
                          const float* Xo_raw, const float* Wo, int32_t ldwo, const float* bo, const float* efeat,
                          const float* emask, float* zcat, float* attn, int32_t G, void* stream);
int32_t dgppo_attn_bwd_xo(const dgppo_env_cfg* cfg, int32_t F, int32_t H, int32_t Kp, const float* dzcat,
                          const float* attn, const float* qt, const float* Xa, const float* Xo_raw, const float* Wo,
                          int32_t ldwo, const float* bo, const float* efeat, float* dqt, float* dXa, float* dXo,
                          int32_t relu_xo, int32_t G, void* stream);
int64_t dgppo_attn_xo_workspace_bytes(int32_t G);
int32_t dgppo_attn_bwd_xo_dw(const dgppo_env_cfg* cfg, int32_t F, int32_t H, int32_t Kp, const float* dzcat,
                             const float* attn, const float* qt, const float* Xa, const float* Xo_raw, const float* Wo,
                             int32_t ldwo, const float* bo, const float* efeat, float* dqt, float* dXa, float* dWo,
                             int32_t lddwo, float* dbo, float* workspace, int64_t workspace_bytes, int32_t G, void* stream);

int32_t dgppo_gnn_prep(const float* Wq, const float* bq, const float* Wk, const float* Wv, const float* bv,
                       const float* We, const float* Wu, float* Mcat, float* cvec, float* Wout, int32_t F, int32_t Fp,
                       int32_t D, int32_t H, int32_t Kp, void* stream);
int32_t dgppo_gnn_unprep(const float* dMcat, const float* dcvec, const float* dWout, const float* Wq, const float* bq,
                         const float* Wk, float* dWq, float* dbq, float* dWk, float* dWv, float* dbv, float* dWe,
                         float* dWu, int32_t F, int32_t Fp, int32_t D, int32_t H, int32_t Kp, void* stream);

int32_t dgppo_ln_relu_fwd(const float* x, const float* gamma, const float* beta, float* y, float* stats, int32_t M,
                          void* stream);
int32_t dgppo_ln_relu_bwd(const float* x, const float* y, const float* stats, const float* gamma, const float* dy,
                          float* dx, float* dgamma, float* dbeta, int32_t M, void* stream);

int32_t dgppo_gru_fwd(const float* gi, const float* Wh, const float* bhn, const float* h0, float* hs, float* hprev,
                      float* gates, int32_t n_seq, int32_t T, int32_t n_inner, void* stream);
int32_t dgppo_gru_bwd(const float* dhs, const float* Wh, const float* hprev, const float* gates, float* dgi,
                      float* dgh, int32_t n_seq, int32_t T, int32_t n_inner, void* stream);
int32_t dgppo_gru_bwd_dhn(const float* dhs, const float* Wh, const float* hprev, const float* gates, float* dgi,
                          float* dhn, int32_t n_seq, int32_t T, int32_t n_inner, void* stream);
int64_t dgppo_gru_bwd_w_workspace_bytes(void);
int32_t dgppo_gru_bwd_w(const float* x, int32_t ldx, const float* hprev, int32_t ldh, const float* dgi, const float* dhn,
                        float* dWi, int32_t ldwi, float* dbi, float* dWh, int32_t ldwh, float* dbhn, int32_t M,
                        float* workspace, int64_t workspace_bytes, dgppo_reduce_desc* pending, void* stream);

int32_t dgppo_lstm_fwd(const float* zi, const float* Wh, const float* bh, const float* c0, const float* h0, float* cs,
                       float* hs, float* cprev, float* hprev, float* gates, int32_t n_seq, int32_t T, int32_t n_inner,
                       void* stream);
int32_t dgppo_lstm_bwd(const float* dhs, const float* Wh, const float* cprev, const float* gates, float* dz,
                       int32_t n_seq, int32_t T, int32_t n_inner, void* stream);

int32_t dgppo_policy_head(const float* ms, const float* eps, const float* action_in, float* action, float* log_pi,
                          float* entropy, int32_t rows, int32_t n_agents, int32_t mode, const float* log_pi_old,
                          const float* adv, float* dms, float* stats, float clip_eps, float coef_ent, void* stream);

int32_t dgppo_value_loss(const float* v, const float* target, float* dv, float* stats, int32_t count, void* stream);
int32_t dgppo_mean_agents(const float* x, float* y, int32_t G, int32_t n, int32_t D, int32_t backward,
                          const float* relu_mask, void* stream);
int32_t dgppo_relu_bwd(float* dy, const float* y, int64_t count, void* stream);


int32_t dgppo_gae(const float* costs, const float* rewards, const float* Vh, const float* Vl, const float* lam_pow,
                  float gamma, float one_minus_gamma, float one_minus_lam, float* Qh, float* Ql, int32_t B, int32_t T,
                  int32_t n, int32_t nh, void* stream);
int32_t dgppo_advantage(const float* Ql, const float* Vl, const float* Vh, float dt, float alpha, float cbf_eps,
                        float cbf_weight, float* adv, float* stats, int32_t B, int32_t T, int32_t n, int32_t nh,
                        void* stream);
int32_t dgppo_advantage_lagr(const float* Ql, const float* Vl, const float* Qh, const float* Vh, const float* lagr,
                             float* adv, float* Ah, int32_t B, int32_t T, int32_t n, int32_t nh, void* stream);
int32_t dgppo_lagr_update(const float* lp_new, const float* lp_old, const float* Vh, int64_t vh_env_stride,
                          const float* Ah, float* lagr, float* sums, int32_t n_env, int32_t T, int32_t n, int32_t nh,
                          float one_minus_gamma, float lr, void* stream);
int32_t dgppo_lagr_sums(const float* lp_new, const float* lp_old, const float* Vh, int64_t vh_env_stride, const float* Ah,
                        float* sums, int32_t n_env, int32_t T, int32_t n, int32_t nh, float one_minus_gamma, void* stream);
int32_t dgppo_lagr_apply(float* lagr, float* sums, int32_t count, int64_t rows_total, float lr, void* stream);
int32_t dgppo_relu_fwd(const float* x, float* out, int64_t count, void* stream);
int32_t dgppo_shaped_reward(const float* reward, const float* cost, float cost_weight, float* out, int64_t rows,
                            int32_t n, int32_t nh, void* stream);
#define DGPPO_OPT_PARTIALS 256
#define DGPPO_OPT_STATE_FLOATS (8 + 2 * DGPPO_OPT_PARTIALS)
int32_t dgppo_clip_adam_step(float* params, const float* grads, float* m, float* v, int64_t n, float* state, float lr,
                             float b1, float b2, float eps, float max_norm, float grad_scale, void* stream);

#define DGPPO_COMM_ID_BYTES 128
int32_t dgppo_comm_unique_id(uint8_t* id_out);
int32_t dgppo_comm_version(int32_t* version_out);
int32_t dgppo_comm_init(const uint8_t* id, int32_t rank, int32_t world, void** comm_out);
int32_t dgppo_comm_allreduce_sum_f32(void* comm, float* buf, int64_t count, void* stream);
int32_t dgppo_comm_destroy(void* comm);

#ifdef __cplusplus
}
#endif
#endif
```

Baseline: 4.168 million.

## Fuse GRU input projection into the recurrent GRU forward kernel

```diff
diff --git a/dgppo_amd/_native.py b/dgppo_amd/_native.py
--- a/dgppo_amd/_native.py
+++ b/dgppo_amd/_native.py
@@ -155,6 +155,10 @@
     l = C.CDLL(LIB_PATH)
     l.dgppo_abi_version.restype = C.c_int32
     l.dgppo_last_error.restype = C.c_char_p
+    l.dgppo_gru_fwd_x.restype = C.c_int32
+    l.dgppo_gru_fwd_x.argtypes = [C.c_void_p, C.c_int32] + [C.c_void_p] * 8 + [C.c_int32] * 3 + [C.c_void_p]
+    l.dgppo_gru_fwd_x_preferred.restype = C.c_int32
+    l.dgppo_gru_fwd_x_preferred.argtypes = [C.c_int32] * 4
     v = l.dgppo_abi_version()
     if v != ABI_VERSION:
         raise RuntimeError(f"dgppo_amd: ABI mismatch: library {v}, python {ABI_VERSION}")
diff --git a/dgppo_amd/csrc/nn_elem.hip b/dgppo_amd/csrc/nn_elem.hip
--- a/dgppo_amd/csrc/nn_elem.hip
+++ b/dgppo_amd/csrc/nn_elem.hip
@@ -137,6 +137,10 @@
 
 struct GruArgs {
   const float* gi;
+  const float* x;
+  const float* Wi;
+  const float* bi;
+  int ldx;
   const float* Wh;
   const float* bhn;
   const float* h0;
@@ -161,8 +165,8 @@
 
 #define GRU_LDS_BARRIER() asm volatile("s_waitcnt lgkmcnt(0)\n\ts_barrier" ::: "memory")
 
-template <int RTW>
-__global__ void __launch_bounds__(256) gru_fwd_kernel(GruArgs a) {
+template <int RTW, bool XIN>
+__device__ __forceinline__ void gru_fwd_body(const GruArgs& a) {
   extern __shared__ float sm[];
   constexpr int RB = 16 * RTW;
   constexpr int HSLOT = RB * 16 / 256 > 0 ? RB * 16 / 256 : 1;
@@ -174,6 +178,16 @@
 #pragma unroll
     for (int t = 0; t < 3; ++t) breg[kk][t] = a.Wh[(size_t)(kk * 4 + lq) * 192 + t * 64 + c];
   const float bn = a.bhn[c];
+  float wireg[16][3];
+  float bi3[3] = {0.f, 0.f, 0.f};
+  if constexpr (XIN) {
+#pragma unroll
+    for (int j = 0; j < 16; ++j)
+#pragma unroll
+      for (int t = 0; t < 3; ++t) wireg[j][t] = a.Wi[(size_t)(lq * 16 + j) * 192 + t * 64 + c];
+#pragma unroll
+    for (int t = 0; t < 3; ++t) bi3[t] = a.bi[t * 64 + c];
+  }
   const int n_tiles = (a.n_seq + RB - 1) / RB;
   const float4 z4 = make_float4(0.f, 0.f, 0.f, 0.f);
   float hpf[HSLOT][4];
@@ -205,6 +219,12 @@
     const int s0 = tile * RB;
     const int nxt = tile + gridDim.x;
     if (nxt < n_tiles) fetch_h0(nxt);
+    auto seq_row0 = [&](int s) {
+      int rw = s;
+      if (a.T != 1 && a.n_inner != 1) { const int grp = s / a.n_inner; rw = grp * a.T * a.n_inner + (s - grp * a.n_inner); }
+      else if (a.T != 1) rw = s * a.T;
+      return rw;
+    };
     int row0[RTW][4];
     bool ok[RTW][4];
 #pragma unroll
@@ -214,10 +234,7 @@
         int s = s0 + rt * 16 + lq * 4 + r;
         ok[rt][r] = s < a.n_seq;
         s = ok[rt][r] ? s : a.n_seq - 1;
-        int rw = s;
-        if (a.T != 1 && a.n_inner != 1) { const int grp = s / a.n_inner; rw = grp * a.T * a.n_inner + (s - grp * a.n_inner); }
-        else if (a.T != 1) rw = s * a.T;
-        row0[rt][r] = rw;
+        row0[rt][r] = seq_row0(s);
       }
     float gn[RTW][4][3];
     auto fetch_gi = [&](int tau) {
@@ -229,16 +246,37 @@
           gn[rt][r][0] = gp[0]; gn[rt][r][1] = gp[64]; gn[rt][r][2] = gp[128];
         }
     };
-    fetch_gi(0);
+    int xrow0[RTW];
+    float xr[RTW][16];
+    auto fetch_x = [&](int tau) {
+#pragma unroll
+      for (int rt = 0; rt < RTW; ++rt) {
+        const float4* p = reinterpret_cast<const float4*>(a.x + (size_t)(xrow0[rt] + tau * a.n_inner) * a.ldx + lq * 16);
+#pragma unroll
+        for (int j = 0; j < 4; ++j) { const float4 v = p[j]; xr[rt][4 * j] = v.x; xr[rt][4 * j + 1] = v.y; xr[rt][4 * j + 2] = v.z; xr[rt][4 * j + 3] = v.w; }
+      }
+    };
+    if constexpr (XIN) {
+#pragma unroll
+      for (int rt = 0; rt < RTW; ++rt) {
+        const int s = s0 + rt * 16 + li;
+        xrow0[rt] = seq_row0(s < a.n_seq ? s : a.n_seq - 1);
+      }
+      fetch_x(0);
+    } else {
+      fetch_gi(0);
+    }
     for (int tau = 0; tau < a.T; ++tau) {
       const float* hs_cur = sm + cur * (RB * GRU_HL);
       float* hs_nxt = sm + (cur ^ 1) * (RB * GRU_HL);
       float g[RTW][4][3];
-#pragma unroll
-      for (int rt = 0; rt < RTW; ++rt)
-#pragma unroll
-        for (int r = 0; r < 4; ++r) { g[rt][r][0] = gn[rt][r][0]; g[rt][r][1] = gn[rt][r][1]; g[rt][r][2] = gn[rt][r][2]; }
-      if (tau + 1 < a.T) fetch_gi(tau + 1);
+      if constexpr (!XIN) {
+#pragma unroll
+        for (int rt = 0; rt < RTW; ++rt)
+#pragma unroll
+          for (int r = 0; r < 4; ++r) { g[rt][r][0] = gn[rt][r][0]; g[rt][r][1] = gn[rt][r][1]; g[rt][r][2] = gn[rt][r][2]; }
+        if (tau + 1 < a.T) fetch_gi(tau + 1);
+      }
       __builtin_amdgcn_sched_barrier(0);
       float areg[RTW][16];
 #pragma unroll
@@ -257,6 +295,29 @@
         for (int rt = 0; rt < RTW; ++rt)
 #pragma unroll
           for (int t = 0; t < 3; ++t) acc[rt][t] = __builtin_amdgcn_mfma_f32_16x16x4f32(areg[rt][kk], breg[kk][t], acc[rt][t], 0, 0, 0);
+      if constexpr (XIN) {
+        __builtin_amdgcn_sched_barrier(0);
+        f32x4 agi[RTW][3];
+#pragma unroll
+        for (int rt = 0; rt < RTW; ++rt)
+#pragma unroll
+          for (int t = 0; t < 3; ++t) agi[rt][t] = f32x4{0.f, 0.f, 0.f, 0.f};
+#pragma unroll
+        for (int j = 0; j < 16; ++j)
+#pragma unroll
+          for (int rt = 0; rt < RTW; ++rt)
+#pragma unroll
+            for (int t = 0; t < 3; ++t) agi[rt][t] = __builtin_amdgcn_mfma_f32_16x16x4f32(xr[rt][j], wireg[j][t], agi[rt][t], 0, 0, 0);
+        __builtin_amdgcn_sched_barrier(0);
+        if (tau + 1 < a.T) fetch_x(tau + 1);
+        __builtin_amdgcn_sched_barrier(0);
+#pragma unroll
+        for (int rt = 0; rt < RTW; ++rt)
+#pragma unroll
+          for (int r = 0; r < 4; ++r)
+#pragma unroll
+            for (int t = 0; t < 3; ++t) g[rt][r][t] = agi[rt][t][r] + bi3[t];
+      }
 #pragma unroll
       for (int rt = 0; rt < RTW; ++rt)
 #pragma unroll
@@ -267,7 +328,7 @@
           const float zg = gate_sigmoid(g[rt][r][1] + acc[rt][1][r]);
           const float hn = acc[rt][2][r] + bn;
           const float ng = gate_tanh(g[rt][r][2] + rg * hn);
-          const float hnew = (1.0f - zg) * ng + zg * hp;
+          const float hnew = (RTW == 1 && r != 0) ? fmaf(1.0f - zg, ng, zg * hp) : fmaf(zg, hp, (1.0f - zg) * ng);
           hs_nxt[rl * GRU_HL + c] = hnew;
           if (ok[rt][r]) {
             const size_t row = (size_t)(row0[rt][r] + tau * a.n_inner);
@@ -288,6 +349,11 @@
     }
   }
 }
+
+template <int RTW>
+__global__ void __launch_bounds__(256) gru_fwd_kernel(GruArgs a) { gru_fwd_body<RTW, false>(a); }
+template <int RTW>
+__global__ void __launch_bounds__(256) __attribute__((amdgpu_waves_per_eu(2, 8))) gru_fwd_x_kernel(GruArgs a) { gru_fwd_body<RTW, true>(a); }
 
 template <int RTW, bool DHN_ONLY>
 __global__ void __launch_bounds__(256) gru_bwd_kernel(GruArgs a) {
@@ -407,6 +473,27 @@
   return 0;
 }
 
+template <bool XIN>
+static int32_t gru_fwd_launch(const GruArgs& a, hipStream_t stream) {
+  if (cdiv(a.n_seq, 32) >= 512) {
+    void (*const fn)(GruArgs) = XIN ? &gru_fwd_x_kernel<2> : &gru_fwd_kernel<2>;
+    const size_t smem = sizeof(float) * 2 * 32 * GRU_HL;
+    static thread_local int cap = 0;
+    if (cap == 0) cap = gru_resident(reinterpret_cast<const void*>(fn), smem);
+    const int tiles = cdiv(a.n_seq, 32);
+    hipLaunchKernelGGL(fn, dim3(tiles < cap ? tiles : cap), dim3(256), smem, stream, a);
+  } else {
+    void (*const fn)(GruArgs) = XIN ? &gru_fwd_x_kernel<1> : &gru_fwd_kernel<1>;
+    const size_t smem = sizeof(float) * 2 * 16 * GRU_HL;
+    static thread_local int cap = 0;
+    if (cap == 0) cap = gru_resident(reinterpret_cast<const void*>(fn), smem);
+    const int tiles = cdiv(a.n_seq, 16);
+    hipLaunchKernelGGL(fn, dim3(tiles < cap ? tiles : cap), dim3(256), smem, stream, a);
+  }
+  DGPPO_LAUNCH_CHECK();
+  return 0;
+}
+
 extern "C" int32_t dgppo_gru_fwd(const float* gi, const float* Wh, const float* bhn, const float* h0, float* hs,
                                  float* hprev, float* gates, int32_t n_seq, int32_t T, int32_t n_inner, void* stream) {
   GruArgs a{};
@@ -416,21 +503,30 @@
   if (rc) return rc;
   if (n_seq == 0) return 0;
   DGPPO_REQUIRE(gi && Wh && bhn && hs, "gru_fwd: NULL operand");
-  if (cdiv(n_seq, 32) >= 512) {
-    const size_t smem = sizeof(float) * 2 * 32 * GRU_HL;
-    static thread_local int cap = 0;
-    if (cap == 0) cap = gru_resident(reinterpret_cast<const void*>(&gru_fwd_kernel<2>), smem);
-    const int tiles = cdiv(n_seq, 32);
-    hipLaunchKernelGGL(gru_fwd_kernel<2>, dim3(tiles < cap ? tiles : cap), dim3(256), smem, (hipStream_t)stream, a);
-  } else {
-    const size_t smem = sizeof(float) * 2 * 16 * GRU_HL;
-    static thread_local int cap = 0;
-    if (cap == 0) cap = gru_resident(reinterpret_cast<const void*>(&gru_fwd_kernel<1>), smem);
-    const int tiles = cdiv(n_seq, 16);
-    hipLaunchKernelGGL(gru_fwd_kernel<1>, dim3(tiles < cap ? tiles : cap), dim3(256), smem, (hipStream_t)stream, a);
-  }
-  DGPPO_LAUNCH_CHECK();
-  return 0;
+  return gru_fwd_launch<false>(a, (hipStream_t)stream);
+}
+
+extern "C" int32_t dgppo_gru_fwd_x(const float* x, int32_t ldx, const float* Wi, const float* bi, const float* Wh,
+                                   const float* bhn, const float* h0, float* hs, float* hprev, float* gates, int32_t n_seq,
+                                   int32_t T, int32_t n_inner, void* stream) {
+  GruArgs a{};
+  a.x = x; a.ldx = ldx; a.Wi = Wi; a.bi = bi; a.Wh = Wh; a.bhn = bhn; a.h0 = h0; a.hs = hs; a.hprev = hprev; a.gates = gates;
+  a.n_seq = n_seq; a.T = T; a.n_inner = n_inner;
+  int32_t rc = gru_check(a);
+  if (rc) return rc;
+  if (n_seq == 0) return 0;
+  DGPPO_REQUIRE(x && Wi && bi && Wh && bhn && hs, "gru_fwd_x: NULL operand");
+  DGPPO_REQUIRE(ldx >= GRU_H && (ldx & 3) == 0 && (reinterpret_cast<uintptr_t>(x) & 15) == 0,
+                "gru_fwd_x: the rows of x must be 16-byte addressable (x %p, ldx %d): form gi with dgppo_mlp_gi_fwd and call "
+                "dgppo_gru_fwd", (const void*)x, ldx);
+  return gru_fwd_launch<true>(a, (hipStream_t)stream);
+}
+
+#define GRU_X_MIN_SEQ 4096
+extern "C" int32_t dgppo_gru_fwd_x_preferred(int32_t n_seq, int32_t T, int32_t n_inner, int32_t train) {
+  (void)n_inner; (void)train;
+  if (n_seq <= 0 || T < 1) return 0;
+  return (T == 1 || n_seq >= GRU_X_MIN_SEQ) ? 1 : 0;
 }
 
 template <bool DHN_ONLY>
diff --git a/dgppo_amd/csrc/nn_fused.hip b/dgppo_amd/csrc/nn_fused.hip
--- a/dgppo_amd/csrc/nn_fused.hip
+++ b/dgppo_amd/csrc/nn_fused.hip
@@ -21,6 +21,7 @@
   float* gi;
 };
 
+template <bool GI>
 __global__ void __launch_bounds__(256) __attribute__((amdgpu_waves_per_eu(2, 8))) mlp_gi_fwd_kernel(MlpGiArgs a) {
   extern __shared__ float sm[];
   float* s_x = sm;
@@ -35,11 +36,14 @@
     const int k = kk * 4 + lq;
     w1[kk] = a.W1[k * FZ_H + c];
     w2[kk] = a.W2[k * FZ_H + c];
-#pragma unroll
-    for (int t = 0; t < 3; ++t) wi[kk][t] = a.Wi[k * 192 + t * 64 + c];
+    if constexpr (GI) {
+#pragma unroll
+      for (int t = 0; t < 3; ++t) wi[kk][t] = a.Wi[k * 192 + t * 64 + c];
+    }
   }
   const float b1 = a.b1[c], g1 = a.g1[c], e1 = a.be1[c], b2 = a.b2[c], g2 = a.g2[c], e2 = a.be2[c];
-  const float bi0 = a.bi[c], bi1 = a.bi[64 + c], bi2 = a.bi[128 + c];
+  float bi0 = 0.f, bi1 = 0.f, bi2 = 0.f;
+  if constexpr (GI) { bi0 = a.bi[c]; bi1 = a.bi[64 + c]; bi2 = a.bi[128 + c]; }
   const int n_tiles = (a.M + FZ_RB - 1) / FZ_RB;
   const bool vec = ((a.ldx & 3) == 0) && ((reinterpret_cast<uintptr_t>(a.X) & 15) == 0);
   float xpf[2][4];
@@ -96,7 +100,7 @@
         const int row = row0 + rl;
         if (y_out != nullptr && row < a.M) {
           y_out[(size_t)row * FZ_H + c] = y;
-          if (c == 0) { st_out[(size_t)row * 2] = mean; st_out[(size_t)row * 2 + 1] = rstd; }
+          if (c == 0 && st_out != nullptr) { st_out[(size_t)row * 2] = mean; st_out[(size_t)row * 2 + 1] = rstd; }
         }
       }
     FZ_LDS_BARRIER();
@@ -152,32 +156,34 @@
         if (a.p2 != nullptr && row < a.M) a.p2[(size_t)row * FZ_H + c] = v[rt][r];
       }
     ln_relu(v, g2, e2, s_y2, a.y2, a.st2, row0);
-#pragma unroll
-    for (int rt = 0; rt < 2; ++rt)
-#pragma unroll
-      for (int kk = 0; kk < 16; ++kk) areg[rt][kk] = s_y2[(rt * 16 + li) * FZ_HL + kk * 4 + lq];
-    __builtin_amdgcn_sched_barrier(0);
-    f32x4 ag[2][3];
-#pragma unroll
-    for (int rt = 0; rt < 2; ++rt)
-#pragma unroll
-      for (int t = 0; t < 3; ++t) ag[rt][t] = f32x4{0.f, 0.f, 0.f, 0.f};
-#pragma unroll
-    for (int kk = 0; kk < 16; ++kk)
+    if constexpr (GI) {
 #pragma unroll
       for (int rt = 0; rt < 2; ++rt)
 #pragma unroll
-        for (int t = 0; t < 3; ++t) ag[rt][t] = __builtin_amdgcn_mfma_f32_16x16x4f32(areg[rt][kk], wi[kk][t], ag[rt][t], 0, 0, 0);
-#pragma unroll
-    for (int rt = 0; rt < 2; ++rt)
-#pragma unroll
-      for (int r = 0; r < 4; ++r) {
-        const int row = row0 + rt * 16 + lq * 4 + r;
-        if (row < a.M) {
-          float* o = a.gi + (size_t)row * 192 + c;
-          o[0] = ag[rt][0][r] + bi0; o[64] = ag[rt][1][r] + bi1; o[128] = ag[rt][2][r] + bi2;
+        for (int kk = 0; kk < 16; ++kk) areg[rt][kk] = s_y2[(rt * 16 + li) * FZ_HL + kk * 4 + lq];
+      __builtin_amdgcn_sched_barrier(0);
+      f32x4 ag[2][3];
+#pragma unroll
+      for (int rt = 0; rt < 2; ++rt)
+#pragma unroll
+        for (int t = 0; t < 3; ++t) ag[rt][t] = f32x4{0.f, 0.f, 0.f, 0.f};
+#pragma unroll
+      for (int kk = 0; kk < 16; ++kk)
+#pragma unroll
+        for (int rt = 0; rt < 2; ++rt)
+#pragma unroll
+          for (int t = 0; t < 3; ++t) ag[rt][t] = __builtin_amdgcn_mfma_f32_16x16x4f32(areg[rt][kk], wi[kk][t], ag[rt][t], 0, 0, 0);
+#pragma unroll
+      for (int rt = 0; rt < 2; ++rt)
+#pragma unroll
+        for (int r = 0; r < 4; ++r) {
+          const int row = row0 + rt * 16 + lq * 4 + r;
+          if (row < a.M) {
+            float* o = a.gi + (size_t)row * 192 + c;
+            o[0] = ag[rt][0][r] + bi0; o[64] = ag[rt][1][r] + bi1; o[128] = ag[rt][2][r] + bi2;
+          }
         }
-      }
+    }
   }
 }
 
@@ -185,38 +191,43 @@
 #define RW_WIL 193
 #define RW_YL 68
 #define RW_WAVES 16
+template <bool GI>
 __global__ void __launch_bounds__(64 * RW_WAVES) mlp_gi_fwd_rw_kernel(MlpGiArgs a) {
   extern __shared__ float sm[];
   float* sW1 = sm;
   float* sW2 = sW1 + 64 * RW_WL;
   float* sWi = sW2 + 64 * RW_WL;
-  float* sP = sWi + 64 * RW_WIL;
+  float* sP = sWi + (GI ? 64 * RW_WIL : 0);
   const int tid = threadIdx.x, lane = tid & 63, w = tid >> 6, li = lane & 15, lq = lane >> 4;
   float* sY = sP + 576 + w * (16 * RW_YL);
   {
     static_assert(RW_WAVES == 16, "the staging below assumes 1024 threads");
     const float4 v1 = reinterpret_cast<const float4*>(a.W1)[tid], v2 = reinterpret_cast<const float4*>(a.W2)[tid];
     float4 vi[3];
-#pragma unroll
-    for (int j = 0; j < 3; ++j) vi[j] = reinterpret_cast<const float4*>(a.Wi)[j * 1024 + tid];
+    if constexpr (GI) {
+#pragma unroll
+      for (int j = 0; j < 3; ++j) vi[j] = reinterpret_cast<const float4*>(a.Wi)[j * 1024 + tid];
+    }
     {
       const int k = tid >> 4, c = (tid & 15) * 4;
       float* d1 = sW1 + k * RW_WL + c; float* d2 = sW2 + k * RW_WL + c;
       d1[0] = v1.x; d1[1] = v1.y; d1[2] = v1.z; d1[3] = v1.w;
       d2[0] = v2.x; d2[1] = v2.y; d2[2] = v2.z; d2[3] = v2.w;
     }
-#pragma unroll
-    for (int j = 0; j < 3; ++j) {
-      const int q = j * 1024 + tid, k = q / 48, c = (q - k * 48) * 4;
-      float* d = sWi + k * RW_WIL + c;
-      d[0] = vi[j].x; d[1] = vi[j].y; d[2] = vi[j].z; d[3] = vi[j].w;
+    if constexpr (GI) {
+#pragma unroll
+      for (int j = 0; j < 3; ++j) {
+        const int q = j * 1024 + tid, k = q / 48, c = (q - k * 48) * 4;
+        float* d = sWi + k * RW_WIL + c;
+        d[0] = vi[j].x; d[1] = vi[j].y; d[2] = vi[j].z; d[3] = vi[j].w;
+      }
     }
   }
   if (tid < 64) {
     sP[tid] = a.b1[tid]; sP[64 + tid] = a.g1[tid]; sP[128 + tid] = a.be1[tid];
     sP[192 + tid] = a.b2[tid]; sP[256 + tid] = a.g2[tid]; sP[320 + tid] = a.be2[tid];
   }
-  if (tid < 192) sP[384 + tid] = a.bi[tid];
+  if (GI && tid < 192) sP[384 + tid] = a.bi[tid];
   __syncthreads();
   const int n_tiles = (a.M + 15) >> 4;
   const bool save = a.p1 != nullptr;
@@ -282,7 +293,7 @@
         const float y = fmaxf((acc[ct][r] - mean[r]) * rstd[r] * g + e, 0.0f);
         sY[(lq * 4 + r) * RW_YL + ct * 16 + li] = y;
         const int row = row0 + lq * 4 + r;
-        if (save && row < a.M) y_out[(size_t)row * FZ_H + ct * 16 + li] = y;
+        if (y_out != nullptr && row < a.M) y_out[(size_t)row * FZ_H + ct * 16 + li] = y;
       }
     }
 #pragma unroll
@@ -296,39 +307,41 @@
     fetch(tile);
     layer(sW1, sP, a.p1, a.y1, a.st1, row0);
     layer(sW2, sP + 192, a.p2, a.y2, a.st2, row0);
-#pragma unroll
-    for (int half = 0; half < 2; ++half) {
-      f32x4 ag[6];
-#pragma unroll
-      for (int t = 0; t < 6; ++t) ag[t] = f32x4{0.f, 0.f, 0.f, 0.f};
-      float bg[2][2][6];
-      auto ldg = [&](int buf, int g) {
-#pragma unroll
-        for (int kk = 0; kk < 2; ++kk) {
-          const float* wr = sWi + (lq * 16 + g * 2 + kk) * RW_WIL + half * 96 + li;
-#pragma unroll
-          for (int t = 0; t < 6; ++t) bg[buf][kk][t] = wr[t * 16];
+    if constexpr (GI) {
+#pragma unroll
+      for (int half = 0; half < 2; ++half) {
+        f32x4 ag[6];
+#pragma unroll
+        for (int t = 0; t < 6; ++t) ag[t] = f32x4{0.f, 0.f, 0.f, 0.f};
+        float bg[2][2][6];
+        auto ldg = [&](int buf, int g) {
+#pragma unroll
+          for (int kk = 0; kk < 2; ++kk) {
+            const float* wr = sWi + (lq * 16 + g * 2 + kk) * RW_WIL + half * 96 + li;
+#pragma unroll
+            for (int t = 0; t < 6; ++t) bg[buf][kk][t] = wr[t * 16];
+          }
+        };
+        ldg(0, 0);
+#pragma unroll
+        for (int g = 0; g < 8; ++g) {
+          if (g + 1 < 8) ldg((g + 1) & 1, g + 1);
+          __builtin_amdgcn_sched_barrier(0);
+#pragma unroll
+          for (int kk = 0; kk < 2; ++kk)
+#pragma unroll
+            for (int t = 0; t < 6; ++t) ag[t] = __builtin_amdgcn_mfma_f32_16x16x4f32(A[g * 2 + kk], bg[g & 1][kk][t], ag[t], 0, 0, 0);
+          __builtin_amdgcn_sched_barrier(0);
         }
-      };
-      ldg(0, 0);
-#pragma unroll
-      for (int g = 0; g < 8; ++g) {
-        if (g + 1 < 8) ldg((g + 1) & 1, g + 1);
-        __builtin_amdgcn_sched_barrier(0);
-#pragma unroll
-        for (int kk = 0; kk < 2; ++kk)
-#pragma unroll
-          for (int t = 0; t < 6; ++t) ag[t] = __builtin_amdgcn_mfma_f32_16x16x4f32(A[g * 2 + kk], bg[g & 1][kk][t], ag[t], 0, 0, 0);
-        __builtin_amdgcn_sched_barrier(0);
-      }
-#pragma unroll
-      for (int t = 0; t < 6; ++t) {
-        const int col = half * 96 + t * 16 + li;
-        const float b = sP[384 + col];
-#pragma unroll
-        for (int r = 0; r < 4; ++r) {
-          const int row = row0 + lq * 4 + r;
-          if (row < a.M) a.gi[(size_t)row * 192 + col] = ag[t][r] + b;
+#pragma unroll
+        for (int t = 0; t < 6; ++t) {
+          const int col = half * 96 + t * 16 + li;
+          const float b = sP[384 + col];
+#pragma unroll
+          for (int r = 0; r < 4; ++r) {
+            const int row = row0 + lq * 4 + r;
+            if (row < a.M) a.gi[(size_t)row * 192 + col] = ag[t][r] + b;
+          }
         }
       }
     }
@@ -566,51 +579,58 @@
   return 0;
 }
 
+template <bool GI>
+static int32_t mlp_gi_fwd_launch(const MlpGiArgs& a, hipStream_t stream) {
+  const int M = a.M;
+  if ((a.ldx & 3) == 0 && ((reinterpret_cast<uintptr_t>(a.X) | reinterpret_cast<uintptr_t>(a.W1) | reinterpret_cast<uintptr_t>(a.W2) |
+                            (GI ? reinterpret_cast<uintptr_t>(a.Wi) : 0)) & 15) == 0) {
+    static thread_local int cus = 0;
+    if (cus == 0) {
+      int dev = 0;
+      if (hipGetDevice(&dev) != hipSuccess ||
+          hipDeviceGetAttribute(&cus, hipDeviceAttributeMultiprocessorCount, dev) != hipSuccess || cus < 1) cus = 256;
+    }
+    const size_t smem_rw = sizeof(float) * (2 * 64 * RW_WL + (GI ? 64 * RW_WIL : 0) + 576 + RW_WAVES * 16 * RW_YL);
+    static thread_local bool attr = false;
+    if (!attr) {
+      const hipError_t e = hipFuncSetAttribute(reinterpret_cast<const void*>(&mlp_gi_fwd_rw_kernel<GI>),
+                                               hipFuncAttributeMaxDynamicSharedMemorySize, (int)smem_rw);
+      DGPPO_REQUIRE(e == hipSuccess, "mlp_gi_fwd: cannot reserve %zu bytes of LDS per workgroup: %s", smem_rw, hipGetErrorString(e));
+      attr = true;
+    }
+    const int tiles16 = (M + 15) / 16;
+    hipLaunchKernelGGL(mlp_gi_fwd_rw_kernel<GI>, dim3(tiles16 < cus ? tiles16 : cus), dim3(64 * RW_WAVES), smem_rw, stream, a);
+    DGPPO_LAUNCH_CHECK();
+    return 0;
+  }
+  const size_t smem = sizeof(float) * (3 * FZ_RB * FZ_HL + FZ_RB * 8);
+  static thread_local int cap = 0;
+  if (cap == 0) {
+    int per_cu = 0, dev = 0, cus = 256;
+    if (hipOccupancyMaxActiveBlocksPerMultiprocessor(&per_cu, reinterpret_cast<const void*>(&mlp_gi_fwd_kernel<GI>), 256, smem) !=
+            hipSuccess || per_cu < 1) per_cu = 1;
+    if (hipGetDevice(&dev) != hipSuccess ||
+        hipDeviceGetAttribute(&cus, hipDeviceAttributeMultiprocessorCount, dev) != hipSuccess || cus < 1) cus = 256;
+    cap = per_cu * cus;
+  }
+  const int tiles = (M + FZ_RB - 1) / FZ_RB;
+  hipLaunchKernelGGL(mlp_gi_fwd_kernel<GI>, dim3(tiles < cap ? tiles : cap), dim3(256), smem, stream, a);
+  DGPPO_LAUNCH_CHECK();
+  return 0;
+}
+
 extern "C" int32_t dgppo_mlp_gi_fwd(const float* X, int32_t ldx, const float* W1, const float* b1, const float* g1,
                                     const float* be1, const float* W2, const float* b2, const float* g2, const float* be2,
                                     const float* Wi, const float* bi, float* p1, float* y1, float* st1, float* p2, float* y2,
                                     float* st2, float* gi, int32_t M, void* stream) {
   DGPPO_REQUIRE(M >= 0 && ldx >= FZ_H, "mlp_gi_fwd: bad shape M=%d ldx=%d", M, ldx);
-  DGPPO_REQUIRE(X && W1 && b1 && g1 && be1 && W2 && b2 && g2 && be2 && Wi && bi && gi, "mlp_gi_fwd: NULL operand");
-  const bool save = p1 || y1 || st1 || p2 || y2 || st2;
+  DGPPO_REQUIRE(X && W1 && b1 && g1 && be1 && W2 && b2 && g2 && be2 && (!gi || (Wi && bi)), "mlp_gi_fwd: NULL operand");
+  DGPPO_REQUIRE(gi || y2, "mlp_gi_fwd: without gi the chain ends at y2, which must be given");
+  const bool save = p1 || y1 || st1 || p2 || st2 || (gi && y2);
   DGPPO_REQUIRE(!save || (p1 && y1 && st1 && p2 && y2 && st2), "mlp_gi_fwd: the saved activations are all-or-none");
   if (M == 0) return 0;
   MlpGiArgs a{X, ldx, M, W1, b1, g1, be1, W2, b2, g2, be2, Wi, bi, p1, y1, st1, p2, y2, st2, gi};
-  if ((ldx & 3) == 0 && ((reinterpret_cast<uintptr_t>(X) | reinterpret_cast<uintptr_t>(W1) | reinterpret_cast<uintptr_t>(W2) |
-                          reinterpret_cast<uintptr_t>(Wi)) & 15) == 0) {
-    static thread_local int cus = 0;
-    if (cus == 0) {
-      int dev = 0;
-      if (hipGetDevice(&dev) != hipSuccess ||
-          hipDeviceGetAttribute(&cus, hipDeviceAttributeMultiprocessorCount, dev) != hipSuccess || cus < 1) cus = 256;
-    }
-    const size_t smem_rw = sizeof(float) * (2 * 64 * RW_WL + 64 * RW_WIL + 576 + RW_WAVES * 16 * RW_YL);
-    static thread_local bool attr = false;
-    if (!attr) {
-      const hipError_t e = hipFuncSetAttribute(reinterpret_cast<const void*>(&mlp_gi_fwd_rw_kernel),
-                                               hipFuncAttributeMaxDynamicSharedMemorySize, (int)smem_rw);
-      DGPPO_REQUIRE(e == hipSuccess, "mlp_gi_fwd: cannot reserve %zu bytes of LDS per workgroup: %s", smem_rw, hipGetErrorString(e));
-      attr = true;
-    }
-    const int tiles16 = (M + 15) / 16;
-    hipLaunchKernelGGL(mlp_gi_fwd_rw_kernel, dim3(tiles16 < cus ? tiles16 : cus), dim3(64 * RW_WAVES), smem_rw, (hipStream_t)stream, a);
-    DGPPO_LAUNCH_CHECK();
-    return 0;
-  }
-  const size_t smem = sizeof(float) * (3 * FZ_RB * FZ_HL + FZ_RB * 8);
-  static thread_local int cap = 0;
-  if (cap == 0) {
-    int per_cu = 0, dev = 0, cus = 256;
-    if (hipOccupancyMaxActiveBlocksPerMultiprocessor(&per_cu, reinterpret_cast<const void*>(&mlp_gi_fwd_kernel), 256, smem) !=
-            hipSuccess || per_cu < 1) per_cu = 1;
-    if (hipGetDevice(&dev) != hipSuccess ||
-        hipDeviceGetAttribute(&cus, hipDeviceAttributeMultiprocessorCount, dev) != hipSuccess || cus < 1) cus = 256;
-    cap = per_cu * cus;
-  }
-  const int tiles = (M + FZ_RB - 1) / FZ_RB;
-  hipLaunchKernelGGL(mlp_gi_fwd_kernel, dim3(tiles < cap ? tiles : cap), dim3(256), smem, (hipStream_t)stream, a);
-  DGPPO_LAUNCH_CHECK();
-  return 0;
+  return gi ? mlp_gi_fwd_launch<true>(a, (hipStream_t)stream) : mlp_gi_fwd_launch<false>(a, (hipStream_t)stream);
 }
 
 struct GruHeadArgs {
diff --git a/dgppo_amd/nets.py b/dgppo_amd/nets.py
--- a/dgppo_amd/nets.py
+++ b/dgppo_amd/nets.py
@@ -140,6 +140,7 @@
         self.kind, self.cfg, self.gnn_layers, self.n_out, self.device = kind, cfg, gnn_layers, n_out, device
         self.rnn, self.rnn_layers = rnn, (rnn_layers if rnn != "none" else 0)
         self.carry_dim = HID * max(self.rnn_layers, 1) * (2 if rnn == "lstm" else 1)
+        self.gru_from_x: Optional[bool] = None
         self.layout = make_layout(kind, cfg.node_dim, gnn_layers, n_out, rnn, rnn_layers)
         self.params = torch.zeros(self.layout.size, device=device)
         if grads is None:
@@ -250,7 +251,12 @@
             xcat.view(G, n, 2 * OUT_DIM)[:, :, OUT_DIM:].copy_(pooled.view(G, 1, OUT_DIM).expand(G, n, OUT_DIM))
             x = xcat
         act["Rh"], act["n_inner"], act["mlp_in"] = Rh, n_inner, x
-        gi = A.get(f"{tag}.gi", Rh, 3 * HID)
+        simple = (self.rnn == "gru" and self.rnn_layers == 1)
+        fused_tail = (simple and T == 1 and self.kind == "policy")
+        from_x = (self.gru_from_x is not False and simple and not fused_tail and self.kind != "Vhg" and x.is_cuda
+                  and x.data_ptr() % 16 == 0 and x.stride(0) % 4 == 0
+                  and (self.gru_from_x or K.gru_fwd_x_preferred(n_seq, T, n_inner, train)))
+        gi = None if from_x else A.get(f"{tag}.gi", Rh, 3 * HID)
         if self.kind == "Vhg" or self.rnn != "gru":
             sv = {nm: A.get(f"{tag}.{nm}", Rh, w) for nm, w in (("p1", HID), ("y1", HID), ("st1", 2), ("p2", HID), ("y2", HID), ("st2", 2))}
             K.dense_fwd(x, self.p("mlp.W1"), self.p("mlp.b1"), sv["p1"])
@@ -261,13 +267,15 @@
                 K.dense_fwd(sv["y2"], self.p("gru.Wi"), self.p("gru.bi"), gi)
             act.update(sv)
         else:
-            saves = None
+            saves = y2 = None
             if train:
                 saves = tuple(A.get(f"{tag}.{nm}{i}", Rh, w) for i in (1, 2) for nm, w in (("p", HID), ("y", HID), ("st", 2)))
                 for i in (1, 2):
                     act[f"p{i}"], act[f"y{i}"], act[f"st{i}"] = saves[3 * (i - 1):3 * i]
+            elif from_x:
+                y2 = act["y2"] = A.get(f"{tag}.y2", Rh, HID)
             K.mlp_gi_fwd(x, self.p("mlp.W1"), self.p("mlp.b1"), self.p("mlp.g1"), self.p("mlp.be1"), self.p("mlp.W2"),
-                         self.p("mlp.b2"), self.p("mlp.g2"), self.p("mlp.be2"), self.p("gru.Wi"), self.p("gru.bi"), gi, saves)
+                         self.p("mlp.b2"), self.p("mlp.g2"), self.p("mlp.be2"), self.p("gru.Wi"), self.p("gru.bi"), gi, saves, y2)
         assert n_seq * T == Rh, (n_seq, T, Rh)
         L, CD = self.rnn_layers, self.carry_dim
         if h0 is not None:
@@ -275,7 +283,6 @@
         if hs_out is not None:
             assert tuple(hs_out.shape) == (Rh, CD), (tuple(hs_out.shape), Rh, CD)
         act["gi"] = gi
-        simple = (self.rnn == "gru" and L == 1)
         if simple:
             hs = hs_out if hs_out is not None else A.get(f"{tag}.hs", Rh, HID)
             hprev_is_h0 = train and T == 1 and h0 is not None and self.kind != "policy"
@@ -283,9 +290,12 @@
             gates = A.get(f"{tag}.gates", Rh, 4 * HID) if train else None
             feat = hs
             act["hs"], act["hprev"], act["gates"] = hs, hprev, gates
-        fused_tail = (simple and T == 1 and self.kind == "policy")
+        if from_x:
+            K.gru_fwd_x(act["y2"], self.p("gru.Wi"), self.p("gru.bi"), self.p("gru.Wh"), self.p("gru.bhn"), h0, hs, hprev, gates,
+                        n_seq, T, n_inner)
+        elif simple and not fused_tail:
+            K.gru_fwd(gi, self.p("gru.Wh"), self.p("gru.bhn"), h0, hs, hprev, gates, n_seq, T, n_inner)
         if simple and not fused_tail:
-            K.gru_fwd(gi, self.p("gru.Wh"), self.p("gru.bhn"), h0, hs, hprev, gates, n_seq, T, n_inner)
             if hprev_is_h0:
                 act["hprev"] = h0
         if self.rnn == "none":
@@ -418,7 +428,7 @@
                 dhs = dx
             dy = dhs
         else:
-            stack = act.get("stack") or [dict(x=None, gi=act["gi"], hs=act["hs"], hprev=act["hprev"], gates=act["gates"])]
+            stack = act.get("stack") or [dict(x=None, hs=act["hs"], hprev=act["hprev"], gates=act["gates"])]
             if act.get("stack") is None and dout.is_cuda:
                 st = stack[0]
                 dgi = A.get(f"{tag}.dgi0", Rh, 3 * HID)
diff --git a/dgppo_amd/ops_nn.py b/dgppo_amd/ops_nn.py
--- a/dgppo_amd/ops_nn.py
+++ b/dgppo_amd/ops_nn.py
@@ -47,21 +47,29 @@
     N.check(rc, "dgppo_dense_fwd")
 
 
-def mlp_gi_fwd(X, W1, b1, g1, be1, W2, b2, g2, be2, Wi, bi, gi, saves=None):
+def mlp_gi_fwd(X, W1, b1, g1, be1, W2, b2, g2, be2, Wi, bi, gi=None, saves=None, y2=None):
     xp, ldx, M, K = _mat(X, "X")
     if K != 64:
         raise ValueError(f"mlp_gi_fwd: X must be [M, 64], got {tuple(X.shape)}")
-    for t, shp, nm in ((W1, (64, 64), "W1"), (W2, (64, 64), "W2"), (Wi, (64, 192), "Wi"), (b1, (64,), "b1"), (g1, (64,), "g1"),
-                       (be1, (64,), "be1"), (b2, (64,), "b2"), (g2, (64,), "g2"), (be2, (64,), "be2"), (bi, (192,), "bi"),
-                       (gi, (M, 192), "gi")):
+    for t, shp, nm in ((W1, (64, 64), "W1"), (W2, (64, 64), "W2"), (b1, (64,), "b1"), (g1, (64,), "g1"),
+                       (be1, (64,), "be1"), (b2, (64,), "b2"), (g2, (64,), "g2"), (be2, (64,), "be2")):
         N.expect_shape(t, shp, nm)
+    if gi is not None:
+        for t, shp, nm in ((Wi, (64, 192), "Wi"), (bi, (192,), "bi"), (gi, (M, 192), "gi")):
+            N.expect_shape(t, shp, nm)
     sv = [None] * 6
     if saves is not None:
         for t, shp, nm in zip(saves, ((M, 64), (M, 64), (M, 2), (M, 64), (M, 64), (M, 2)), ("p1", "y1", "st1", "p2", "y2", "st2")):
             N.expect_shape(t, shp, nm)
         sv = list(saves)
-    FLOPS[0] += 2.0 * M * (64 * 64 * 2 + 64 * 192)
-    rc = N.lib().dgppo_mlp_gi_fwd(xp, ldx, _p(W1), _p(b1), _p(g1), _p(be1), _p(W2), _p(b2), _p(g2), _p(be2), _p(Wi), _p(bi),
+    if y2 is not None:
+        if saves is not None or gi is not None:
+            raise ValueError("mlp_gi_fwd: y2 alone is the output of the call without gi and without saves")
+        N.expect_shape(y2, (M, 64), "y2")
+        sv[4] = y2
+    FLOPS[0] += 2.0 * M * (64 * 64 * 2 + (64 * 192 if gi is not None else 0))
+    rc = N.lib().dgppo_mlp_gi_fwd(xp, ldx, _p(W1), _p(b1), _p(g1), _p(be1), _p(W2), _p(b2), _p(g2), _p(be2),
+                                  _p(Wi if gi is not None else None), _p(bi if gi is not None else None),
                                   *[_p(t) for t in sv], _p(gi), M, N.stream_ptr())
     N.check(rc, "dgppo_mlp_gi_fwd")
 
@@ -379,6 +387,27 @@
     rc = N.lib().dgppo_gru_fwd(_p(gi), _p(Wh), _p(bhn), _p(h0), _p(hs), _p(hprev), _p(gates), n_seq, T, n_inner,
                                N.stream_ptr())
     N.check(rc, "dgppo_gru_fwd")
+
+
+def gru_fwd_x_preferred(n_seq, T, n_inner, train) -> bool:
+    return bool(N.lib().dgppo_gru_fwd_x_preferred(int(n_seq), int(T), int(n_inner), int(bool(train))))
+
+
+def gru_fwd_x(x, Wi, bi, Wh, bhn, h0, hs, hprev, gates, n_seq, T, n_inner):
+    rows = n_seq * T
+    xp, ldx, Mx, Kx = _mat(x, "x")
+    if (Mx, Kx) != (rows, 64):
+        raise ValueError(f"gru_fwd_x: x must be [{rows}, 64], got {tuple(x.shape)}")
+    N.expect_shape(Wi, (64, 192), "Wi")
+    N.expect_shape(bi, (192,), "bi")
+    N.expect_shape(hs, (rows, 64), "hs")
+    N.expect_shape(Wh, (64, 192), "Wh")
+    if h0 is not None:
+        N.expect_shape(h0, (n_seq, 64), "h0")
+    FLOPS[0] += 2.0 * rows * 64 * 192 * 2
+    rc = N.lib().dgppo_gru_fwd_x(xp, ldx, _p(Wi), _p(bi), _p(Wh), _p(bhn), _p(h0), _p(hs), _p(hprev), _p(gates), n_seq, T,
+                                 n_inner, N.stream_ptr())
+    N.check(rc, "dgppo_gru_fwd_x")
 
 
 def gru_bwd(dhs, Wh, hprev, gates, dgi, dgh, n_seq, T, n_inner):
diff --git a/include/dgppo_hip.h b/include/dgppo_hip.h
--- a/include/dgppo_hip.h
+++ b/include/dgppo_hip.h
@@ -185,6 +185,10 @@
 
 int32_t dgppo_gru_fwd(const float* gi, const float* Wh, const float* bhn, const float* h0, float* hs, float* hprev,
                       float* gates, int32_t n_seq, int32_t T, int32_t n_inner, void* stream);
+int32_t dgppo_gru_fwd_x(const float* x, int32_t ldx, const float* Wi, const float* bi, const float* Wh, const float* bhn,
+                        const float* h0, float* hs, float* hprev, float* gates, int32_t n_seq, int32_t T, int32_t n_inner,
+                        void* stream);
+int32_t dgppo_gru_fwd_x_preferred(int32_t n_seq, int32_t T, int32_t n_inner, int32_t train);
 int32_t dgppo_gru_bwd(const float* dhs, const float* Wh, const float* hprev, const float* gates, float* dgi,
                       float* dgh, int32_t n_seq, int32_t T, int32_t n_inner, void* stream);
 int32_t dgppo_gru_bwd_dhn(const float* dhs, const float* Wh, const float* hprev, const float* gates, float* dgi,
```

Result: no change. 4.202 million, median of 6 (+0.8%).
